# AliaksandrSiarohin/wc-gan

Hardware: AMD Instinct MI355X
Metric: images/sec G+D step, CIFAR-10 ResNet-SN+WC, batch 64 (higher is better)
Workload: dtype f32; 1 GPU; CIFAR-10 ResNet SN uncond + WC (scripts/cifar10_resnet_sn_uncond.sh), batch 64/GPU, training_ratio 5, generator_batch_multiple 2; parallelism=dp1, wc_statistics=per-replica, launch=hipgraph

## Files before the change

### include/wc_hip.h

```cpp
#ifndef WC_HIP_H
#define WC_HIP_H

#include <stddef.h>
#include <stdint.h>

#ifdef __cplusplus
extern "C" {
#endif

#define WC_ABI_VERSION 8

#define WC_OK                 0
#define WC_ERR_NULL          -1
#define WC_ERR_SHAPE         -2
#define WC_ERR_CHANNELS      -3
#define WC_ERR_WORKSPACE     -4
#define WC_ERR_ARG           -5

typedef void* wc_stream_t;

int         wc_abi_version(void);
const char* wc_error_string(int code);

#define WC_CORE_API "wc_stats_f32 wc_factor_f64 wc_color_f32 wc_group_bias_f32 wc_apply_f32 wc_apply_act_f32 " \
                    "wc_bwd_reduce_f32 wc_bwd_factor_f64 wc_bwd_apply_f32 " \
                    "wc_stats_workspace_bytes wc_factor_workspace_bytes wc_color_workspace_bytes wc_apply_workspace_bytes " \
                    "wc_bwd_reduce_workspace_bytes wc_bwd_factor_workspace_bytes wc_bwd_apply_workspace_bytes"

size_t wc_whiten_workspace_bytes(int64_t M, int C, int groups);
size_t wc_factor_error_offset(int C, int groups);
int    wc_factor_route(int C, int groups);
size_t wc_whiten_error_offset(int64_t M, int C, int groups);
int    wc_whiten_f32(const float* x, int64_t M, int C, int groups, double eps, double momentum, int ddof,
                     float* moving_mean , float* moving_cov ,
                     float* mu , float* chan_scale , double* L , double* W ,
                     void* ws, size_t ws_bytes, wc_stream_t stream);

size_t wc_stats_workspace_bytes(int64_t M, int C, int groups);
size_t wc_factor_workspace_bytes(int C, int groups);
size_t wc_color_workspace_bytes(int C, int Kc);
size_t wc_bwd_reduce_workspace_bytes(int64_t N, int64_t HW, int C, int Kc, int has_slot);
size_t wc_bwd_factor_workspace_bytes(int C, int Kc);
size_t wc_apply_workspace_bytes(int64_t N, int64_t HW, int C, int Kc);
size_t wc_apply_plan_bytes(int C, int Kc);
size_t wc_bwd_apply_workspace_bytes(int64_t N, int64_t HW, int C, int Kc);

int wc_stats_f32(const float* x, int64_t M, int C, int groups,
                 double* sum , double* xtx ,
                 void* ws, size_t ws_bytes, wc_stream_t stream);

int wc_factor_f64(const double* sum, const double* xtx, int64_t M , int C, int groups,
                  double eps, double momentum, int ddof, int training,
                  float* moving_mean , float* moving_cov ,
                  float* mu , float* chan_scale ,
                  double* L , double* W ,
                  void* ws, size_t ws_bytes, wc_stream_t stream);

int wc_color_f32(const double* W , const float* gamma ,
                 int Kc, int C, int groups, int per_group,
                 float* A , float* At ,
                 const float* chan_scale , void* plan ,
                 void* ws, size_t ws_bytes, wc_stream_t stream);

int wc_group_bias_f32(const float* mu , const float* A ,
                      const float* beta ,
                      int groups, int Kc, int C, int per_group, float* center , float* bias ,
                      wc_stream_t stream);

int wc_apply_f32(const float* x, const float* mu, const float* A, const float* bias,
                 const int32_t* slot, int64_t N, int64_t HW, int C, int Kc,
                 float* y, const void* plan ,
                 void* ws, size_t ws_bytes, wc_stream_t stream);

int wc_apply_act_f32(const float* x, const float* mu, const float* A, const float* bias,
                     const int32_t* slot, int64_t N, int64_t HW, int C, int Kc, int relu,
                     float* y, const void* plan ,
                     void* ws, size_t ws_bytes, wc_stream_t stream);

size_t wc_split_bytes(int64_t M, int C);
#define WC_SPLIT_FLAG_WORDS (64 + 2 * 1024)
int wc_split_scales_f32(const float* x, int64_t M, int C, float* center , float* scale ,
                        int* flag , wc_stream_t stream);
int wc_split_f32(const float* x, const float* center , const float* scale, int64_t M, int C, int relu,
                 void* xs , int* flag , wc_stream_t stream);
int wc_unsplit_f32(const void* xs, const float* center , const float* scale, int64_t M, int C, float* x ,
                   wc_stream_t stream);

int    wc_stats_split_supported(int64_t M, int C, int groups);
size_t wc_stats_split_workspace_bytes(int64_t M, int C, int groups);
int wc_stats_split_f16x2(const void* xs, const float* xs_center, const float* xs_scale, int64_t M, int C, int groups,
                         double* sum , double* xtx , void* ws, size_t ws_bytes, wc_stream_t stream);

int    wc_split_bias_f32(const float* A , const float* bias, const float* xs_center, const float* mu, int Kc, int C,
                         float* bias_eff , wc_stream_t stream);
int    wc_apply_split_supported(int64_t N, int64_t HW, int C);
size_t wc_apply_split_workspace_bytes(int C, int Kc);
int wc_apply_split_f16x2(const void* xs, const float* xs_center , const float* xs_scale,
                         const float* mu , const float* A, const float* bias ,
                         const int32_t* slot, int64_t N, int64_t HW, int C, int Kc, int relu,
                         float* y, const void* plan , void* ws, size_t ws_bytes, wc_stream_t stream);

int wc_resadd_split_supported(int64_t N, int64_t H, int64_t W, int C);
int wc_resadd_f32(const float* h, const float* s , int64_t N, int64_t H, int64_t W, int C, int up, float* out,
                  wc_stream_t stream);
int wc_resadd_split_f32(const float* h, const float* s , int64_t N, int64_t H, int64_t W, int C, int up,
                        void* xs , float* center , float* scale ,
                        int* flag , float* x32 ,
                        wc_stream_t stream);
int wc_patch_sum_f32(const float* g , int64_t N, int64_t Hs, int64_t Ws, int C, float* out ,
                     wc_stream_t stream);
int    wc_resadd_stats_supported(int64_t N, int64_t H, int64_t W, int C, int up, int groups);
size_t wc_resadd_stats_workspace_bytes(int64_t N, int64_t H, int64_t W, int C, int groups);
int    wc_resadd_stats_split_f32(const float* h, const float* s , int64_t N, int64_t H, int64_t W, int C, int up, int groups,
                                 void* xs , float* center , float* scale , int* flag ,
                                 float* x32 , void* ws , size_t ws_bytes, wc_stream_t stream);
size_t wc_whiten_presummed_error_offset(int64_t M, int C, int groups);
int    wc_whiten_presummed_f16x2(const float* xs_center, int64_t M, int C, int groups, double eps, double momentum, int ddof,
                                 float* moving_mean , float* moving_cov , float* mu ,
                                 double* L , double* W , void* ws ,
                                 size_t ws_bytes, wc_stream_t stream);
int    wc_stats_presummed_f16x2(const float* xs_center, int64_t M, int C, int groups, double* sum ,
                                double* xtx , void* ws , size_t ws_bytes, wc_stream_t stream);
int wc_fold_channel_scale_f32(const float* w, int64_t stride_o, int64_t stride_c, int Cout, int Cin, const float* bias ,
                              const float* scale, const float* center, float* wf , float* bf , wc_stream_t stream);
int wc_unfold_channel_scale_f32(const float* D, const float* db, int64_t stride_o, int64_t stride_c, int Cout, int Cin,
                                const float* scale, const float* center, float* dW , wc_stream_t stream);

size_t wc_whiten_split_workspace_bytes(int64_t M, int C, int groups);
size_t wc_whiten_split_error_offset(int64_t M, int C, int groups);
int    wc_whiten_split_f16x2(const void* xs, const float* xs_center, const float* xs_scale, int64_t M, int C, int groups,
                             double eps, double momentum, int ddof, float* moving_mean , float* moving_cov ,
                             float* mu , double* L , double* W ,
                             void* ws, size_t ws_bytes, wc_stream_t stream);

int wc_color_split_f32(const double* W , const float* gamma , int Kc, int C, float* A ,
                       float* At , const float* xs_scale, const float* xs_center, const float* mu ,
                       const float* beta , void* plan , float* bias_eff ,
                       void* ws, size_t ws_bytes, wc_stream_t stream);
int wc_group_bias_centered_f32(const float* mu , const float* A , const float* beta ,
                               const float* center , int groups, int Kc, int C, int per_group, float* bias ,
                               wc_stream_t stream);

int    wc_factor_mix_supported(int E, int C);
int    wc_factor_mix_f32(const float* dict, const float* alpha, const int32_t* idx , const float* base ,
                         int E, int C, int K, int Kc, float* out , wc_stream_t stream);
size_t wc_factor_mix_bwd_workspace_bytes(int E, int Kc);
int    wc_factor_mix_bwd_f32(const float* dict, const float* alpha, const int32_t* idx , const float* dout ,
                             int E, int C, int K, int Kc, float* ddict , float* dalpha , float* dbase ,
                             void* ws, size_t ws_bytes, wc_stream_t stream);

int wc_apply_split_ex_f16x2(const void* xs, const float* xs_center , const float* xs_scale,
                            const float* mu , const float* A, const float* bias ,
                            const int32_t* slot, int64_t N, int64_t HW, int C, int Kc, int relu,
                            float* y , void* relu_mask , void* planes , float* oscale,
                            const void* plan , void* ws, size_t ws_bytes, wc_stream_t stream);

size_t wc_relu_mask_bytes(int64_t M, int C);
int wc_relu_mask_apply_f32(const float* gy, const void* relu_mask, int64_t M, int C, float* out, wc_stream_t stream);
int wc_apply_mask_f32(const float* x, const float* mu, const float* A, const float* bias,
                      const int32_t* slot, int64_t N, int64_t HW, int C, int Kc,
                      float* y, void* relu_mask , const void* plan ,
                      void* ws, size_t ws_bytes, wc_stream_t stream);

int    wc_apply_planes_supported(int64_t N, int64_t HW, int C);
size_t wc_apply_planes_scale_floats(void);
int    wc_out_scale_f32(const float* gamma , const float* beta , int K, int C,
                        float* oscale, wc_stream_t stream);
int    wc_apply_planes_f32(const float* x, const float* mu, const float* A, const float* bias, const int32_t* slot,
                           int64_t N, int64_t HW, int C, int Kc, int relu, void* planes , float* oscale,
                           void* relu_mask , const void* plan, wc_stream_t stream);

int wc_bwd_reduce_f32(const float* x, const float* mu, const float* gy, const int32_t* slot,
                      int64_t N, int64_t HW, int C, int Kc,
                      double* R , double* gsum ,
                      void* ws, size_t ws_bytes, wc_stream_t stream);

int wc_bwd_reduce_scaled_f32(const float* x, const float* mu, const float* gy, const int32_t* slot,
                             int64_t N, int64_t HW, int C, int Kc,
                             double* R , double* gsum , float* scales_out ,
                             void* ws, size_t ws_bytes, wc_stream_t stream);
int wc_bwd_reduce_relu_f32(const float* x, const float* mu, const float* gy, const float* relu_y , const int32_t* slot,
                           int64_t N, int64_t HW, int C, int Kc,
                           double* R , double* gsum , float* gy_masked ,
                           float* scales_out , void* ws, size_t ws_bytes, wc_stream_t stream);
int wc_bwd_reduce_mask_f32(const float* x, const float* mu, const float* gy, const void* relu_mask, const int32_t* slot,
                           int64_t N, int64_t HW, int C, int Kc,
                           double* R , double* gsum , float* gy_masked ,
                           float* scales_out , void* ws, size_t ws_bytes, wc_stream_t stream);

int wc_bwd_bits_supported(int64_t N, int64_t HW, int C, int has_slot);
int wc_bwd_reduce_bits_f32(const float* x, const float* mu, const float* gy, const void* relu_mask, const int32_t* slot,
                           int64_t N, int64_t HW, int C, int Kc, double* R , double* gsum ,
                           float* scales_out , void* ws, size_t ws_bytes, wc_stream_t stream);
int wc_bwd_apply_bits_f32(const float* gy, const void* relu_mask, const float* x, const float* mu, const float* At, const float* S,
                          const float* gmean, const int32_t* slot, int64_t N, int64_t HW, int C, int Kc,
                          const float* scales , float* dx, void* ws, size_t ws_bytes, wc_stream_t stream);
int wc_bwd_apply_scaled_f32(const float* gy, const float* x, const float* mu, const float* At,
                            const float* S, const float* gmean, const int32_t* slot,
                            int64_t N, int64_t HW, int C, int Kc, const float* scales , float* dx,
                            void* ws, size_t ws_bytes, wc_stream_t stream);

int    wc_bwd_xsplit_supported(int64_t N, int64_t HW, int C, int has_slot);
int    wc_bwd_reduce_xsplit_f32(const void* xs, const float* xs_center, const float* xs_scale, const float* mu, const float* gy,
                                const void* relu_mask , const int32_t* slot, int64_t N, int64_t HW, int C, int Kc,
                                double* R , double* gsum , float* scales_out ,
                                void* ws , size_t ws_bytes, wc_stream_t stream);
size_t wc_bwd_apply_xsplit_workspace_bytes(int C, int Kc);
int    wc_bwd_apply_xsplit_f32(const float* gy, const void* relu_mask , const void* xs, const float* xs_center,
                               const float* xs_scale, const float* mu, const float* At, const float* S, const float* gmean,
                               const int32_t* slot, int64_t N, int64_t HW, int C, int Kc, const float* scales ,
                               float* dx, void* ws, size_t ws_bytes, wc_stream_t stream);

int wc_bwd_factor_f64(const double* R, const double* gsum, const double* W, const double* L,
                      const float* gamma, const float* A, int Kc, int C, int64_t M,
                      double eps, int ddof, int training,
                      float* dgamma , float* dbeta ,
                      float* S , float* gmean ,
                      void* ws, size_t ws_bytes, wc_stream_t stream);

int wc_bwd_apply_f32(const float* gy, const float* x, const float* mu, const float* At,
                     const float* S, const float* gmean, const int32_t* slot,
                     int64_t N, int64_t HW, int C, int Kc, float* dx,
                     void* ws, size_t ws_bytes, wc_stream_t stream);

size_t wc_spectral_norm_workspace_bytes(int rows, int cols);
size_t wc_spectral_norm_amax_offset(int rows, int cols);
size_t wc_spectral_norm_error_offset(int rows, int cols);
int wc_spectral_norm_f32(const float* W, int rows, int cols, float* u, float* v, int iterations, float eps,
                         float* w_sn , float* sigma ,
                         float* u_used , float* v_used ,
                         void* ws, size_t ws_bytes, wc_stream_t stream);

int wc_spectral_norm_bwd_f32(const float* g, const float* w_sn, const float* u, const float* v, const float* sigma,
                             int rows, int cols, int fully_diff, float* dW,
                             void* ws, size_t ws_bytes, wc_stream_t stream);

typedef struct {
    const float* W; float* u; float* v; float* w_sn; float* sigma; float* u_used; float* v_used; void* ws;
    int rows, cols;
} wc_sn_item;
typedef struct {
    const float* g; const float* w_sn; const float* u; const float* v; const float* sigma; float* dW; void* ws;
    int rows, cols;
} wc_sn_bwd_item;
int wc_spectral_norm_batched_f32(const wc_sn_item* items, int count, int iterations, float eps, wc_stream_t stream);
int wc_spectral_norm_bwd_batched_f32(const wc_sn_bwd_item* items, int count, int fully_diff, wc_stream_t stream);

typedef struct {
    int N, H, W;
    int Hin, Win, Cin;
    int Hout, Wout, Cout;
    int in_stride, out_stride;
    int ntaps, nphase;
    signed char dy[4][16], dx[4][16];
    signed char off_y[4], off_x[4];
    signed char nsrc[4][16];
    signed char wr[4][16][4], ws[4][16][4];
    float wcoef;
} wc_conv_geom;

#define WC_CONV_SCRATCH_BYTES 2048

int wc_conv_supported(const wc_conv_geom* g);

int wc_conv_split_f32(const float* x, int64_t n, int relu, void* hi, void* lo, float* scale, void* amax_scratch,
                      wc_stream_t stream);

#define WC_CONV_COLSUM_ROWS 512
int wc_conv_split_colsum_f32(const float* x, int64_t n, int relu, void* hi, void* lo, float* scale, void* amax_scratch,
                             float* colsum_partials, int C, wc_stream_t stream);

#define WC_CONV_HIST_FLOATS (4 * 512 + 16)
#define WC_CONV_HIST_REDO (4 * 512)
int wc_conv_split_hist_f32(const float* x, int64_t n, int relu, void* hi, void* lo, float* scale, float* colsum_partials , int C,
                           float* hist, int bootstrap, wc_stream_t stream);

int wc_conv_split_leaky_f32(const float* x, int64_t n, float negative_slope, void* hi, void* lo, float* scale, void* amax_scratch,
                            float* colsum_partials , int C, wc_stream_t stream);
int wc_conv_split_hist_leaky_f32(const float* x, int64_t n, float negative_slope, void* hi, void* lo, float* scale,
                                 float* colsum_partials , int C, float* hist, int bootstrap, wc_stream_t stream);
int wc_conv_leaky_bwd_f32(float* dx, const float* x, int64_t n, float negative_slope, wc_stream_t stream);

size_t wc_conv_weights_bytes(const wc_conv_geom* g);
int wc_conv_weights_f32(const float* w, int64_t stride_k, int64_t stride_n, int64_t stride_r, int64_t stride_s,
                        int64_t n_elems, const wc_conv_geom* g, void* image, float* scale, void* amax_scratch,
                        const float* known_amax, int known_count, wc_stream_t stream);

int wc_conv_weights_pair_f32(const float* w, int64_t stride_r, int64_t stride_s, int64_t n_elems,
                             int64_t a_stride_k, int64_t a_stride_n, const wc_conv_geom* ga, void* image_a,
                             int64_t b_stride_k, int64_t b_stride_n, const wc_conv_geom* gb, void* image_b,
                             float* scale, void* amax_scratch, const float* known_amax, int known_count,
                             wc_stream_t stream);

size_t wc_conv_workspace_bytes(const wc_conv_geom* g);
int wc_conv_f16x3(const void* xhi, const void* xlo, const float* xscale, const void* wimage, const float* wscale,
                  const float* bias, const void* zero_line, const wc_conv_geom* g, int relu, float* y,
                  void* ws, size_t ws_bytes, wc_stream_t stream);

size_t wc_conv_wrw_workspace_bytes(const wc_conv_geom* g);
int wc_conv_wrw_f16x3(const void* xhi, const void* xlo, const float* xscale, const void* ghi, const void* glo,
                      const float* gscale, const void* zero_line, const wc_conv_geom* g, float* dw, int64_t stride_k,
                      int64_t stride_n, int64_t stride_r, int64_t stride_s, void* ws, size_t ws_bytes,
                      wc_stream_t stream);

int    wc_conv_wrw_narrow_supported(int64_t N, int64_t H, int64_t W, int Cin, int Cout, int ksize);
size_t wc_conv_wrw_narrow_workspace_bytes(int64_t N, int64_t H, int64_t W, int Cin, int Cout, int ksize);
int    wc_conv_wrw_narrow_f32(const float* x, const float* gy, int64_t N, int64_t H, int64_t W, int Cin, int Cout, int ksize,
                              float* dw, int64_t stride_k, int64_t stride_n, int64_t stride_r, int64_t stride_s, float* db ,
                              void* ws, size_t ws_bytes, wc_stream_t stream);

int    wc_conv_narrow64_supported(int64_t N, int64_t H, int64_t W, int Cin, int Cout, int ksize);
size_t wc_conv_wrw_narrow64_workspace_bytes(int64_t N, int64_t H, int64_t W, int Cin, int Cout, int ksize);
int    wc_conv_wrw_narrow64_f32(const float* x, const float* gy, int64_t N, int64_t H, int64_t W, int Cin, int Cout, int ksize,
                                float* dw, int64_t stride_k, int64_t stride_n, int64_t stride_r, int64_t stride_s, float* db ,
                                void* ws, size_t ws_bytes, wc_stream_t stream);

int    wc_conv_fwd_narrow_f32(const float* x, const float* w, int64_t stride_k, int64_t stride_n, int64_t stride_r, int64_t stride_s,
                              const float* bias , int64_t N, int64_t H, int64_t W, int Cin, int Cout, int ksize, int relu,
                              float* y, wc_stream_t stream);

int wc_conv_wrw_bias_f16x3(const void* xhi, const void* xlo, const float* xscale, const void* ghi, const void* glo,
                           const float* gscale, const void* zero_line, const wc_conv_geom* g, float* dw, int64_t stride_k,
                           int64_t stride_n, int64_t stride_r, int64_t stride_s, const float* colsum_partials, float* db,
                           void* ws, size_t ws_bytes, wc_stream_t stream);

int    wc_conv_bwd_pair_supported(const wc_conv_geom* gd, const wc_conv_geom* gf);
size_t wc_conv_bwd_pair_workspace_bytes(const wc_conv_geom* gd, const wc_conv_geom* gf);
int    wc_conv_bwd_pair_f16x3(const void* ghi, const void* glo, const float* gscale, const void* wimage, const float* wscale,
                              const void* zero_line, const wc_conv_geom* gd, float* dx, void* ws_dx, size_t ws_dx_bytes,
                              const void* xhi, const void* xlo, const float* xscale, const wc_conv_geom* gf, float* dw,
                              int64_t stride_k, int64_t stride_n, int64_t stride_r, int64_t stride_s,
                              const float* colsum_partials, float* db, void* ws_dw, size_t ws_dw_bytes, wc_stream_t stream);

int wc_stream_copy_f32(const float* src, float* dst, int64_t n, wc_stream_t stream);


size_t wc_std_stats_workspace_bytes(int64_t M, int C, int groups);
int    wc_std_stats_f32(const float* x, int64_t M, int C, int groups, double* sum , double* sqsum ,
                        void* ws, size_t ws_bytes, wc_stream_t stream);

int    wc_std_factor_f64(const double* sum, const double* sqsum, int64_t M, int C, int groups, double eps, double momentum, int ddof,
                         int training, float* moving_mean , float* moving_variance ,
                         const float* gamma , const float* beta , int Kc,
                         float* mu , float* w , float* a , float* b ,
                         wc_stream_t stream);

int    wc_std_apply_f32(const float* x, const float* a, const float* b, const int32_t* slot , int64_t N, int64_t HW,
                        int C, int Kt, int relu, float* y, wc_stream_t stream);

size_t wc_std_bwd_reduce_workspace_bytes(int64_t N, int64_t HW, int C, int Kc);
int    wc_std_bwd_reduce_f32(const float* x, const float* gy, const float* a, const float* b, const int32_t* slot, int64_t N, int64_t HW,
                             int C, int Kc, int relu, double* gsum , double* gxsum ,
                             void* ws, size_t ws_bytes, wc_stream_t stream);

int    wc_std_bwd_factor_f64(const double* gsum, const double* gxsum, const float* mu , const float* w ,
                             const float* gamma , int64_t M, int C, int Kc, int training,
                             float* dgamma , float* dbeta , float* q , float* r , wc_stream_t stream);

int    wc_std_bwd_apply_f32(const float* x, const float* gy, const float* a, const float* b, const float* q, const float* r,
                            const int32_t* slot, int64_t N, int64_t HW, int C, int Kc, int relu, float* dx, wc_stream_t stream);


int    wc_zca_supported(int C);
size_t wc_zca_workspace_bytes(int C, int groups);
size_t wc_zca_status_offset(int C, int groups);
int    wc_zca_f64(const double* L , int C, int groups, double eps,
                  double* U , double* lam , double* W ,
                  void* ws, size_t ws_bytes, wc_stream_t stream);

size_t wc_bwd_factor_zca_workspace_bytes(int C, int Kc);
int    wc_bwd_factor_zca_f64(const double* R, const double* gsum, const double* W, const double* U, const double* lam,
                             const float* gamma, const float* A, int Kc, int C, int64_t M,
                             double eps, int ddof, int training,
                             float* dgamma , float* dbeta ,
                             float* S , float* gmean ,
                             void* ws, size_t ws_bytes, wc_stream_t stream);


int    wc_renorm_supported(int C);
size_t wc_renorm_workspace_bytes(int C);
int    wc_renorm_f64(const float* moving_cov , const double* L , int C, double eps,
                     double* Wm , double* C0 ,
                     void* ws, size_t ws_bytes, wc_stream_t stream);

size_t wc_bwd_factor_renorm_workspace_bytes(int C, int Kc);
int    wc_bwd_factor_renorm_f64(const double* R, const double* gsum, const double* W, const double* Wm, const double* C0,
                                const float* gamma, const float* A, int Kc, int C, int64_t M,
                                double eps, int ddof, int training,
                                float* dgamma , float* dbeta ,
                                float* S , float* gmean ,
                                void* ws, size_t ws_bytes, wc_stream_t stream);


int wc_conv_split_masked_f32(const float* t, const float* a, int64_t n, float slope, void* hi, void* lo, float* scale, void* amax_scratch,
                             wc_stream_t stream);
int wc_conv_split_hist_masked_f32(const float* t, const float* a, int64_t n, float slope, void* hi, void* lo, float* scale, float* hist,
                                  int bootstrap, wc_stream_t stream);

int wc_gp_interp_f32(const float* real, const float* fake, const float* eps, int64_t N, int64_t L, float* x_hat, wc_stream_t stream);

size_t wc_gp_rows_workspace_bytes(int64_t N);
int wc_gp_rows_f32(const float* g, int64_t N, int64_t L, double lambda, double inv_n, float* norms , float* v ,
                   float* penalty , void* ws, size_t ws_bytes, wc_stream_t stream);

#ifdef __cplusplus
}
#endif
#endif
```

### wc_gan_amd/_lib.py

```python
from __future__ import annotations

import ctypes
import os
from ctypes import c_float, c_char_p, c_double, c_int, c_int64, c_size_t, c_void_p

_HERE = os.path.dirname(os.path.abspath(__file__))
LIB_PATH = os.path.join(_HERE, "libwc_hip.so")

WC_OK = 0
ABI_VERSION = 8
ERRORS = {-1: "WC_ERR_NULL", -2: "WC_ERR_SHAPE", -3: "WC_ERR_CHANNELS", -4: "WC_ERR_WORKSPACE", -5: "WC_ERR_ARG"}

SIGNATURES = {
    "wc_abi_version": (c_int, []),
    "wc_error_string": (c_char_p, [c_int]),
    "wc_stats_workspace_bytes": (c_size_t, [c_int64, c_int, c_int]),
    "wc_factor_workspace_bytes": (c_size_t, [c_int, c_int]),
    "wc_color_workspace_bytes": (c_size_t, [c_int, c_int]),
    "wc_bwd_reduce_workspace_bytes": (c_size_t, [c_int64, c_int64, c_int, c_int, c_int]),
    "wc_bwd_factor_workspace_bytes": (c_size_t, [c_int, c_int]),
    "wc_apply_workspace_bytes": (c_size_t, [c_int64, c_int64, c_int, c_int]),
    "wc_apply_plan_bytes": (c_size_t, [c_int, c_int]),
    "wc_bwd_apply_workspace_bytes": (c_size_t, [c_int64, c_int64, c_int, c_int]),
    "wc_stats_f32": (c_int, [c_void_p, c_int64, c_int, c_int, c_void_p, c_void_p, c_void_p, c_size_t, c_void_p]),
    "wc_group_bias_f32": (c_int, [c_void_p, c_void_p, c_void_p, c_int, c_int, c_int, c_int, c_void_p, c_void_p, c_void_p]),
    "wc_factor_f64": (c_int, [c_void_p, c_void_p, c_int64, c_int, c_int, c_double, c_double, c_int, c_int,
                              c_void_p, c_void_p, c_void_p, c_void_p, c_void_p, c_void_p, c_void_p, c_size_t, c_void_p]),
    "wc_color_f32": (c_int, [c_void_p, c_void_p, c_int, c_int, c_int, c_int, c_void_p, c_void_p, c_void_p, c_void_p,
                             c_void_p, c_size_t, c_void_p]),
    "wc_apply_f32": (c_int, [c_void_p, c_void_p, c_void_p, c_void_p, c_void_p, c_int64, c_int64, c_int, c_int,
                             c_void_p, c_void_p, c_void_p, c_size_t, c_void_p]),
    "wc_apply_act_f32": (c_int, [c_void_p, c_void_p, c_void_p, c_void_p, c_void_p, c_int64, c_int64, c_int, c_int, c_int,
                                 c_void_p, c_void_p, c_void_p, c_size_t, c_void_p]),
    "wc_bwd_reduce_f32": (c_int, [c_void_p, c_void_p, c_void_p, c_void_p, c_int64, c_int64, c_int, c_int,
                                  c_void_p, c_void_p, c_void_p, c_size_t, c_void_p]),
    "wc_bwd_reduce_scaled_f32": (c_int, [c_void_p, c_void_p, c_void_p, c_void_p, c_int64, c_int64, c_int, c_int,
                                         c_void_p, c_void_p, c_void_p, c_void_p, c_size_t, c_void_p]),
    "wc_bwd_reduce_relu_f32": (c_int, [c_void_p, c_void_p, c_void_p, c_void_p, c_void_p, c_int64, c_int64, c_int, c_int,
                                       c_void_p, c_void_p, c_void_p, c_void_p, c_void_p, c_size_t, c_void_p]),
    "wc_relu_mask_bytes": (c_size_t, [c_int64, c_int]),
    "wc_relu_mask_apply_f32": (c_int, [c_void_p, c_void_p, c_int64, c_int, c_void_p, c_void_p]),
    "wc_apply_mask_f32": (c_int, [c_void_p, c_void_p, c_void_p, c_void_p, c_void_p, c_int64, c_int64, c_int, c_int,
                                  c_void_p, c_void_p, c_void_p, c_void_p, c_size_t, c_void_p]),
    "wc_whiten_workspace_bytes": (c_size_t, [c_int64, c_int, c_int]),
    "wc_factor_error_offset": (c_size_t, [c_int, c_int]),
    "wc_factor_route": (c_int, [c_int, c_int]),
    "wc_whiten_error_offset": (c_size_t, [c_int64, c_int, c_int]),
    "wc_whiten_f32": (c_int, [c_void_p, c_int64, c_int, c_int, c_double, c_double, c_int, c_void_p, c_void_p, c_void_p, c_void_p,
                              c_void_p, c_void_p, c_void_p, c_size_t, c_void_p]),
    "wc_apply_planes_supported": (c_int, [c_int64, c_int64, c_int]),
    "wc_apply_planes_scale_floats": (c_size_t, []),
    "wc_out_scale_f32": (c_int, [c_void_p, c_void_p, c_int, c_int, c_void_p, c_void_p]),
    "wc_apply_planes_f32": (c_int, [c_void_p, c_void_p, c_void_p, c_void_p, c_void_p, c_int64, c_int64, c_int, c_int, c_int,
                                    c_void_p, c_void_p, c_void_p, c_void_p, c_void_p]),
    "wc_bwd_reduce_mask_f32": (c_int, [c_void_p, c_void_p, c_void_p, c_void_p, c_void_p, c_int64, c_int64, c_int, c_int,
                                       c_void_p, c_void_p, c_void_p, c_void_p, c_void_p, c_size_t, c_void_p]),
    "wc_bwd_bits_supported": (c_int, [c_int64, c_int64, c_int, c_int]),
    "wc_bwd_reduce_bits_f32": (c_int, [c_void_p, c_void_p, c_void_p, c_void_p, c_void_p, c_int64, c_int64, c_int, c_int,
                                       c_void_p, c_void_p, c_void_p, c_void_p, c_size_t, c_void_p]),
    "wc_bwd_apply_bits_f32": (c_int, [c_void_p, c_void_p, c_void_p, c_void_p, c_void_p, c_void_p, c_void_p, c_void_p,
                                      c_int64, c_int64, c_int, c_int, c_void_p, c_void_p, c_void_p, c_size_t, c_void_p]),
    "wc_bwd_apply_scaled_f32": (c_int, [c_void_p, c_void_p, c_void_p, c_void_p, c_void_p, c_void_p, c_void_p,
                                        c_int64, c_int64, c_int, c_int, c_void_p, c_void_p, c_void_p, c_size_t, c_void_p]),
    "wc_bwd_factor_f64": (c_int, [c_void_p, c_void_p, c_void_p, c_void_p, c_void_p, c_void_p, c_int, c_int, c_int64,
                                  c_double, c_int, c_int, c_void_p, c_void_p, c_void_p, c_void_p,
                                  c_void_p, c_size_t, c_void_p]),
    "wc_bwd_apply_f32": (c_int, [c_void_p, c_void_p, c_void_p, c_void_p, c_void_p, c_void_p, c_void_p,
                                 c_int64, c_int64, c_int, c_int, c_void_p, c_void_p, c_size_t, c_void_p]),
    "wc_split_bytes": (c_size_t, [c_int64, c_int]),
    "wc_split_scales_f32": (c_int, [c_void_p, c_int64, c_int, c_void_p, c_void_p, c_void_p, c_void_p]),
    "wc_split_f32": (c_int, [c_void_p, c_void_p, c_void_p, c_int64, c_int, c_int, c_void_p, c_void_p, c_void_p]),
    "wc_unsplit_f32": (c_int, [c_void_p, c_void_p, c_void_p, c_int64, c_int, c_void_p, c_void_p]),
    "wc_stats_split_supported": (c_int, [c_int64, c_int, c_int]),
    "wc_stats_split_workspace_bytes": (c_size_t, [c_int64, c_int, c_int]),
    "wc_stats_split_f16x2": (c_int, [c_void_p, c_void_p, c_void_p, c_int64, c_int, c_int, c_void_p, c_void_p, c_void_p, c_size_t, c_void_p]),
    "wc_split_bias_f32": (c_int, [c_void_p, c_void_p, c_void_p, c_void_p, c_int, c_int, c_void_p, c_void_p]),
    "wc_apply_split_supported": (c_int, [c_int64, c_int64, c_int]),
    "wc_apply_split_workspace_bytes": (c_size_t, [c_int, c_int]),
    "wc_apply_split_f16x2": (c_int, [c_void_p, c_void_p, c_void_p, c_void_p, c_void_p, c_void_p, c_void_p, c_int64, c_int64,
                                     c_int, c_int, c_int, c_void_p, c_void_p, c_void_p, c_size_t, c_void_p]),
    "wc_apply_split_ex_f16x2": (c_int, [c_void_p, c_void_p, c_void_p, c_void_p, c_void_p, c_void_p, c_void_p, c_int64, c_int64,
                                        c_int, c_int, c_int, c_void_p, c_void_p, c_void_p, c_void_p, c_void_p, c_void_p, c_size_t, c_void_p]),
    "wc_whiten_split_workspace_bytes": (c_size_t, [c_int64, c_int, c_int]),
    "wc_whiten_split_error_offset": (c_size_t, [c_int64, c_int, c_int]),
    "wc_whiten_split_f16x2": (c_int, [c_void_p, c_void_p, c_void_p, c_int64, c_int, c_int, c_double, c_double, c_int, c_void_p, c_void_p,
                                      c_void_p, c_void_p, c_void_p, c_void_p, c_size_t, c_void_p]),
    "wc_resadd_split_supported": (c_int, [c_int64, c_int64, c_int64, c_int]),
    "wc_resadd_f32": (c_int, [c_void_p, c_void_p, c_int64, c_int64, c_int64, c_int, c_int, c_void_p, c_void_p]),
    "wc_resadd_stats_supported": (c_int, [c_int64, c_int64, c_int64, c_int, c_int, c_int]),
    "wc_resadd_stats_workspace_bytes": (c_size_t, [c_int64, c_int64, c_int64, c_int, c_int]),
    "wc_resadd_stats_split_f32": (c_int, [c_void_p, c_void_p, c_int64, c_int64, c_int64, c_int, c_int, c_int, c_void_p, c_void_p, c_void_p, c_void_p,
                                          c_void_p, c_void_p, c_size_t, c_void_p]),
    "wc_whiten_presummed_error_offset": (c_size_t, [c_int64, c_int, c_int]),
    "wc_whiten_presummed_f16x2": (c_int, [c_void_p, c_int64, c_int, c_int, c_double, c_double, c_int, c_void_p, c_void_p, c_void_p, c_void_p,
                                          c_void_p, c_void_p, c_size_t, c_void_p]),
    "wc_stats_presummed_f16x2": (c_int, [c_void_p, c_int64, c_int, c_int, c_void_p, c_void_p, c_void_p, c_size_t, c_void_p]),
    "wc_resadd_split_f32": (c_int, [c_void_p, c_void_p, c_int64, c_int64, c_int64, c_int, c_int, c_void_p, c_void_p, c_void_p, c_void_p,
                                    c_void_p, c_void_p]),
    "wc_patch_sum_f32": (c_int, [c_void_p, c_int64, c_int64, c_int64, c_int, c_void_p, c_void_p]),
    "wc_fold_channel_scale_f32": (c_int, [c_void_p, c_int64, c_int64, c_int, c_int, c_void_p, c_void_p, c_void_p, c_void_p, c_void_p, c_void_p]),
    "wc_unfold_channel_scale_f32": (c_int, [c_void_p, c_void_p, c_int64, c_int64, c_int, c_int, c_void_p, c_void_p, c_void_p, c_void_p]),
    "wc_color_split_f32": (c_int, [c_void_p, c_void_p, c_int, c_int, c_void_p, c_void_p, c_void_p, c_void_p, c_void_p, c_void_p, c_void_p,
                                   c_void_p, c_void_p, c_size_t, c_void_p]),
    "wc_factor_mix_supported": (c_int, [c_int, c_int]),
    "wc_factor_mix_f32": (c_int, [c_void_p, c_void_p, c_void_p, c_void_p, c_int, c_int, c_int, c_int, c_void_p, c_void_p]),
    "wc_factor_mix_bwd_workspace_bytes": (c_size_t, [c_int, c_int]),
    "wc_factor_mix_bwd_f32": (c_int, [c_void_p, c_void_p, c_void_p, c_void_p, c_int, c_int, c_int, c_int, c_void_p, c_void_p, c_void_p,
                                      c_void_p, c_size_t, c_void_p]),
    "wc_group_bias_centered_f32": (c_int, [c_void_p, c_void_p, c_void_p, c_void_p, c_int, c_int, c_int, c_int, c_void_p, c_void_p]),
    "wc_bwd_xsplit_supported": (c_int, [c_int64, c_int64, c_int, c_int]),
    "wc_bwd_reduce_xsplit_f32": (c_int, [c_void_p, c_void_p, c_void_p, c_void_p, c_void_p, c_void_p, c_void_p, c_int64, c_int64, c_int, c_int,
                                         c_void_p, c_void_p, c_void_p, c_void_p, c_size_t, c_void_p]),
    "wc_bwd_apply_xsplit_workspace_bytes": (c_size_t, [c_int, c_int]),
    "wc_bwd_apply_xsplit_f32": (c_int, [c_void_p, c_void_p, c_void_p, c_void_p, c_void_p, c_void_p, c_void_p, c_void_p, c_void_p, c_void_p,
                                        c_int64, c_int64, c_int, c_int, c_void_p, c_void_p, c_void_p, c_size_t, c_void_p]),
    "wc_stream_copy_f32": (c_int, [c_void_p, c_void_p, c_int64, c_void_p]),
    "wc_spectral_norm_workspace_bytes": (c_size_t, [c_int, c_int]),
    "wc_spectral_norm_batched_f32": (c_int, [c_void_p, c_int, c_int, c_float, c_void_p]),
    "wc_spectral_norm_bwd_batched_f32": (c_int, [c_void_p, c_int, c_int, c_void_p]),
    "wc_spectral_norm_f32": (c_int, [c_void_p, c_int, c_int, c_void_p, c_void_p, c_int, c_float, c_void_p, c_void_p,
                                     c_void_p, c_void_p, c_void_p, c_size_t, c_void_p]),
    "wc_spectral_norm_bwd_f32": (c_int, [c_void_p, c_void_p, c_void_p, c_void_p, c_void_p, c_int, c_int, c_int, c_void_p,
                                         c_void_p, c_size_t, c_void_p]),
    "wc_conv_supported": (c_int, [c_void_p]),
    "wc_conv_split_f32": (c_int, [c_void_p, c_int64, c_int, c_void_p, c_void_p, c_void_p, c_void_p, c_void_p]),
    "wc_conv_weights_bytes": (c_size_t, [c_void_p]),
    "wc_conv_weights_f32": (c_int, [c_void_p, c_int64, c_int64, c_int64, c_int64, c_int64, c_void_p, c_void_p, c_void_p,
                                    c_void_p, c_void_p, c_int, c_void_p]),
    "wc_spectral_norm_amax_offset": (c_size_t, [c_int, c_int]),
    "wc_spectral_norm_error_offset": (c_size_t, [c_int, c_int]),
    "wc_conv_split_hist_f32": (c_int, [c_void_p, c_int64, c_int, c_void_p, c_void_p, c_void_p, c_void_p, c_int, c_void_p, c_int, c_void_p]),
    "wc_conv_split_leaky_f32": (c_int, [c_void_p, c_int64, c_float, c_void_p, c_void_p, c_void_p, c_void_p, c_void_p, c_int, c_void_p]),
    "wc_conv_split_hist_leaky_f32": (c_int, [c_void_p, c_int64, c_float, c_void_p, c_void_p, c_void_p, c_void_p, c_int, c_void_p, c_int, c_void_p]),
    "wc_conv_leaky_bwd_f32": (c_int, [c_void_p, c_void_p, c_int64, c_float, c_void_p]),
    "wc_conv_narrow64_supported": (c_int, [c_int64, c_int64, c_int64, c_int, c_int, c_int]),
    "wc_conv_wrw_narrow64_workspace_bytes": (c_size_t, [c_int64, c_int64, c_int64, c_int, c_int, c_int]),
    "wc_conv_wrw_narrow64_f32": (c_int, [c_void_p, c_void_p, c_int64, c_int64, c_int64, c_int, c_int, c_int, c_void_p, c_int64, c_int64, c_int64,
                                         c_int64, c_void_p, c_void_p, c_size_t, c_void_p]),
    "wc_conv_fwd_narrow_f32": (c_int, [c_void_p, c_void_p, c_int64, c_int64, c_int64, c_int64, c_void_p, c_int64, c_int64, c_int64, c_int, c_int, c_int,
                                       c_int, c_void_p, c_void_p]),
    "wc_conv_wrw_narrow_supported": (c_int, [c_int64, c_int64, c_int64, c_int, c_int, c_int]),
    "wc_conv_wrw_narrow_workspace_bytes": (c_size_t, [c_int64, c_int64, c_int64, c_int, c_int, c_int]),
    "wc_conv_wrw_narrow_f32": (c_int, [c_void_p, c_void_p, c_int64, c_int64, c_int64, c_int, c_int, c_int, c_void_p, c_int64, c_int64, c_int64,
                                       c_int64, c_void_p, c_void_p, c_size_t, c_void_p]),
    "wc_conv_split_colsum_f32": (c_int, [c_void_p, c_int64, c_int, c_void_p, c_void_p, c_void_p, c_void_p, c_void_p, c_int, c_void_p]),
    "wc_conv_wrw_bias_f16x3": (c_int, [c_void_p, c_void_p, c_void_p, c_void_p, c_void_p, c_void_p, c_void_p, c_void_p, c_void_p,
                                       c_int64, c_int64, c_int64, c_int64, c_void_p, c_void_p, c_void_p, c_size_t, c_void_p]),
    "wc_conv_weights_pair_f32": (c_int, [c_void_p, c_int64, c_int64, c_int64, c_int64, c_int64, c_void_p, c_void_p,
                                         c_int64, c_int64, c_void_p, c_void_p, c_void_p, c_void_p, c_void_p, c_int, c_void_p]),
    "wc_conv_wrw_workspace_bytes": (c_size_t, [c_void_p]),
    "wc_conv_wrw_f16x3": (c_int, [c_void_p, c_void_p, c_void_p, c_void_p, c_void_p, c_void_p, c_void_p, c_void_p, c_void_p,
                                  c_int64, c_int64, c_int64, c_int64, c_void_p, c_size_t, c_void_p]),
    "wc_conv_workspace_bytes": (c_size_t, [c_void_p]),
    "wc_conv_f16x3": (c_int, [c_void_p, c_void_p, c_void_p, c_void_p, c_void_p, c_void_p, c_void_p, c_void_p, c_int,
                              c_void_p, c_void_p, c_size_t, c_void_p]),
    "wc_conv_bwd_pair_supported": (c_int, [c_void_p, c_void_p]),
    "wc_conv_bwd_pair_workspace_bytes": (c_size_t, [c_void_p, c_void_p]),
    "wc_conv_bwd_pair_f16x3": (c_int, [c_void_p, c_void_p, c_void_p, c_void_p, c_void_p, c_void_p, c_void_p, c_void_p, c_void_p, c_size_t,
                                       c_void_p, c_void_p, c_void_p, c_void_p, c_void_p, c_int64, c_int64, c_int64, c_int64,
                                       c_void_p, c_void_p, c_void_p, c_size_t, c_void_p]),
    "wc_std_stats_workspace_bytes": (c_size_t, [c_int64, c_int, c_int]),
    "wc_std_stats_f32": (c_int, [c_void_p, c_int64, c_int, c_int, c_void_p, c_void_p, c_void_p, c_size_t, c_void_p]),
    "wc_std_factor_f64": (c_int, [c_void_p, c_void_p, c_int64, c_int, c_int, c_double, c_double, c_int, c_int, c_void_p, c_void_p,
                                  c_void_p, c_void_p, c_int, c_void_p, c_void_p, c_void_p, c_void_p, c_void_p]),
    "wc_std_apply_f32": (c_int, [c_void_p, c_void_p, c_void_p, c_void_p, c_int64, c_int64, c_int, c_int, c_int, c_void_p, c_void_p]),
    "wc_std_bwd_reduce_workspace_bytes": (c_size_t, [c_int64, c_int64, c_int, c_int]),
    "wc_std_bwd_reduce_f32": (c_int, [c_void_p, c_void_p, c_void_p, c_void_p, c_void_p, c_int64, c_int64, c_int, c_int, c_int,
                                      c_void_p, c_void_p, c_void_p, c_size_t, c_void_p]),
    "wc_std_bwd_factor_f64": (c_int, [c_void_p, c_void_p, c_void_p, c_void_p, c_void_p, c_int64, c_int, c_int, c_int,
                                      c_void_p, c_void_p, c_void_p, c_void_p, c_void_p]),
    "wc_std_bwd_apply_f32": (c_int, [c_void_p, c_void_p, c_void_p, c_void_p, c_void_p, c_void_p, c_void_p, c_int64, c_int64, c_int, c_int,
                                     c_int, c_void_p, c_void_p]),
    "wc_zca_supported": (c_int, [c_int]),
    "wc_zca_workspace_bytes": (c_size_t, [c_int, c_int]),
    "wc_zca_status_offset": (c_size_t, [c_int, c_int]),
    "wc_zca_f64": (c_int, [c_void_p, c_int, c_int, c_double, c_void_p, c_void_p, c_void_p, c_void_p, c_size_t, c_void_p]),
    "wc_bwd_factor_zca_workspace_bytes": (c_size_t, [c_int, c_int]),
    "wc_bwd_factor_zca_f64": (c_int, [c_void_p, c_void_p, c_void_p, c_void_p, c_void_p, c_void_p, c_void_p, c_int, c_int, c_int64,
                                      c_double, c_int, c_int, c_void_p, c_void_p, c_void_p, c_void_p,
                                      c_void_p, c_size_t, c_void_p]),
    "wc_renorm_supported": (c_int, [c_int]),
    "wc_renorm_workspace_bytes": (c_size_t, [c_int]),
    "wc_renorm_f64": (c_int, [c_void_p, c_void_p, c_int, c_double, c_void_p, c_void_p, c_void_p, c_size_t, c_void_p]),
    "wc_bwd_factor_renorm_workspace_bytes": (c_size_t, [c_int, c_int]),
    "wc_bwd_factor_renorm_f64": (c_int, [c_void_p, c_void_p, c_void_p, c_void_p, c_void_p, c_void_p, c_void_p, c_int, c_int, c_int64,
                                         c_double, c_int, c_int, c_void_p, c_void_p, c_void_p, c_void_p,
                                         c_void_p, c_size_t, c_void_p]),
    "wc_conv_split_masked_f32": (c_int, [c_void_p, c_void_p, c_int64, c_float, c_void_p, c_void_p, c_void_p, c_void_p, c_void_p]),
    "wc_conv_split_hist_masked_f32": (c_int, [c_void_p, c_void_p, c_int64, c_float, c_void_p, c_void_p, c_void_p, c_void_p, c_int, c_void_p]),
    "wc_gp_interp_f32": (c_int, [c_void_p, c_void_p, c_void_p, c_int64, c_int64, c_void_p, c_void_p]),
    "wc_gp_rows_workspace_bytes": (c_size_t, [c_int64]),
    "wc_gp_rows_f32": (c_int, [c_void_p, c_int64, c_int64, c_double, c_double, c_void_p, c_void_p, c_void_p, c_void_p, c_size_t, c_void_p]),
}


class SnItem(ctypes.Structure):
    _fields_ = [("W", c_void_p), ("u", c_void_p), ("v", c_void_p), ("w_sn", c_void_p), ("sigma", c_void_p),
                ("u_used", c_void_p), ("v_used", c_void_p), ("ws", c_void_p), ("rows", c_int), ("cols", c_int)]


class SnBwdItem(ctypes.Structure):
    _fields_ = [("g", c_void_p), ("w_sn", c_void_p), ("u", c_void_p), ("v", c_void_p), ("sigma", c_void_p),
                ("dW", c_void_p), ("ws", c_void_p), ("rows", c_int), ("cols", c_int)]


class ConvGeom(ctypes.Structure):
    _fields_ = [("N", c_int), ("H", c_int), ("W", c_int), ("Hin", c_int), ("Win", c_int), ("Cin", c_int),
                ("Hout", c_int), ("Wout", c_int), ("Cout", c_int), ("in_stride", c_int), ("out_stride", c_int),
                ("ntaps", c_int), ("nphase", c_int),
                ("dy", (ctypes.c_byte * 16) * 4), ("dx", (ctypes.c_byte * 16) * 4),
                ("off_y", ctypes.c_byte * 4), ("off_x", ctypes.c_byte * 4),
                ("nsrc", (ctypes.c_byte * 16) * 4),
                ("wr", ((ctypes.c_byte * 4) * 16) * 4), ("ws", ((ctypes.c_byte * 4) * 16) * 4),
                ("wcoef", c_float)]


_lib = None


class WcHipError(RuntimeError):
    pass


def shared_gpu_guard(device_count=None) -> bool:
    if "WC_K2_TWO_LAUNCH" in os.environ:
        if os.environ["WC_K2_TWO_LAUNCH"] == "0":
            del os.environ["WC_K2_TWO_LAUNCH"]
        return False
    try:
        ranks = int(os.environ.get("LOCAL_WORLD_SIZE", "1") or 1)
    except ValueError:
        ranks = 1
    if ranks <= 1:
        return False
    if any(os.environ.get(k) for k in ("HIP_VISIBLE_DEVICES", "CUDA_VISIBLE_DEVICES", "ROCR_VISIBLE_DEVICES")):
        return False
    if device_count is None:
        try:
            import torch
            device_count = torch.cuda.device_count()
        except Exception:
            device_count = 0
    if device_count and ranks > device_count:
        os.environ["WC_K2_TWO_LAUNCH"] = "1"
        return True
    return False


def load() -> ctypes.CDLL:
    global _lib
    if _lib is not None:
        return _lib
    import torch
    shared_gpu_guard()
    if not os.path.exists(LIB_PATH):
        raise WcHipError(
            f"{LIB_PATH} is missing: build it with `python -m wc_gan_amd.build` "
            "(or __graft_entry__.build()); the WC path has no non-HIP fallback")
    lib = ctypes.CDLL(LIB_PATH)
    for name, (res, args) in SIGNATURES.items():
        fn = getattr(lib, name)
        fn.restype = res
        fn.argtypes = args
    if lib.wc_abi_version() != ABI_VERSION:
        raise WcHipError(f"libwc_hip.so ABI version {lib.wc_abi_version()} != {ABI_VERSION}: rebuild it "
                         "(python -m wc_gan_amd.build)")
    _lib = lib
    return lib


def check(code: int, what: str) -> None:
    if code == WC_OK:
        return
    lib = load()
    msg = lib.wc_error_string(code)
    raise WcHipError(f"{what} failed: {ERRORS.get(code, code)} ({msg.decode() if msg else '?'})")
```

### wc_gan_amd/conv.py

```python
from __future__ import annotations

import ctypes
import os

import torch
import torch.nn.functional as F

from . import _lib, _state
from .ops import _ptr, _stream

_zero_lines = {}


def _zero_line(device):
    z = _zero_lines.get(device)
    if z is None:
        z = _zero_lines[device] = torch.zeros(64, dtype=torch.uint8, device=device)
    return z


def _plain(r, s):
    return [(r, s)], 1.0


def _pooled3(r, s):
    return [(r - a, s - b) for a in (0, 1) for b in (0, 1) if 0 <= r - a <= 2 and 0 <= s - b <= 2], 0.25


_UP_ROWS = ((2,), (1, 2), (0, 1), (0,))


def _upsampled3(r, s):
    return [(r3, s3) for r3 in _UP_ROWS[r] for s3 in _UP_ROWS[s]], 1.0


def _set_sources(g, p, t, r, s, source):
    taps, coef = source(r, s)
    g.nsrc[p][t] = len(taps)
    for m, (r3, s3) in enumerate(taps):
        g.wr[p][t][m], g.ws[p][t][m] = r3, s3
    g.wcoef = coef


def _dense_geom(N, Hin, Win, Cin, Cout, k, stride, source=_plain):
    pad = k // 2 if stride == 1 else 1
    g = _lib.ConvGeom()
    g.N, g.Hin, g.Win, g.Cin, g.Cout = N, Hin, Win, Cin, Cout
    g.H, g.W = Hin // stride, Win // stride
    g.Hout, g.Wout = g.H, g.W
    g.in_stride, g.out_stride, g.ntaps, g.nphase = stride, 1, k * k, 1
    for r in range(k):
        for s in range(k):
            t = r * k + s
            g.dy[0][t], g.dx[0][t] = r - pad, s - pad
            _set_sources(g, 0, t, r, s, source)
    return g


def _phase_geom(N, Hin, Win, Cin, Cout, source=_plain):
    g = _lib.ConvGeom()
    g.N, g.Hin, g.Win, g.Cin, g.Cout = N, Hin, Win, Cin, Cout
    g.H, g.W, g.Hout, g.Wout = Hin, Win, 2 * Hin, 2 * Win
    g.in_stride, g.out_stride, g.ntaps, g.nphase = 1, 2, 4, 4
    for py in range(2):
        for px in range(2):
            p = py * 2 + px
            g.off_y[p], g.off_x[p] = py, px
            t = 0
            for dy in ((-1, 0) if py == 0 else (0, 1)):
                for dx in ((-1, 0) if px == 0 else (0, 1)):
                    g.dy[p][t], g.dx[p][t] = dy, dx
                    _set_sources(g, p, t, py + 1 - 2 * dy, px + 1 - 2 * dx, source)
                    t += 1
    return g


def _supported(g):
    return bool(_lib.load().wc_conv_supported(ctypes.addressof(g)))


def supported(x, w, kind):
    handed = getattr(x, '_wc_planes', None) is not None
    if not (x.is_cuda and x.dtype == torch.float32 and x.dim() == 4 and (handed or x.is_contiguous()) and w.dtype == torch.float32):
        return False
    p = _plan(kind, x, w)
    return bool(p) and p.ok


class _Plan:
    __slots__ = ('ok', 'fwd', 'bwd', 'fwd_ws', 'bwd_ws', 'wrw_ws', 'fwd_ptr', 'bwd_ptr', 'pair')

    def __init__(self, kind, N, H, W, wshape):
        class _W:
            shape = wshape
        lib = _lib.load()
        (gf, kf, nf), (gb, kb, nb) = _geoms(kind, N, H, W, _W)
        self.fwd, self.bwd = (gf, kf, nf), (gb, kb, nb)
        self.fwd_ptr, self.bwd_ptr = ctypes.addressof(gf), ctypes.addressof(gb)
        self.ok = bool(lib.wc_conv_supported(self.fwd_ptr)) and bool(lib.wc_conv_supported(self.bwd_ptr))
        self.fwd_ws = lib.wc_conv_workspace_bytes(self.fwd_ptr) if self.ok else 0
        self.bwd_ws = lib.wc_conv_workspace_bytes(self.bwd_ptr) if self.ok else 0
        self.wrw_ws = lib.wc_conv_wrw_workspace_bytes(self.fwd_ptr) if self.ok else 0
        self.pair = self.ok and bool(lib.wc_conv_bwd_pair_supported(self.bwd_ptr, self.fwd_ptr))


_plans = {}


def _plan(kind, x, w):
    key = (kind, tuple(x.shape), tuple(w.shape))
    p = _plans.get(key)
    if p is None:
        N, H, W, C = x.shape
        good = (kind == 'same' and w.shape[1] == C and w.shape[2] == w.shape[3] and w.shape[2] in (1, 3)) or \
               (kind == 'down' and w.shape[1] == C and tuple(w.shape[2:]) == (4, 4) and H % 2 == 0 and W % 2 == 0) or \
               (kind == 'down3' and w.shape[1] == C and tuple(w.shape[2:]) == (3, 3) and H % 2 == 0 and W % 2 == 0) or \
               (kind == 'up3' and w.shape[1] == C and tuple(w.shape[2:]) == (3, 3)) or \
               (kind == 'up' and w.shape[0] == C and tuple(w.shape[2:]) == (4, 4))
        if kind not in ('same', 'down', 'up', 'down3', 'up3'):
            raise ValueError(kind)
        if good and kind != 'down' and (C % 128 or w.shape[0] % 128 or w.shape[1] % 128):
            good = False
        p = _plans[key] = _Plan(kind, N, H, W, tuple(w.shape)) if good else False
    return p


def _colsum_ok(C):
    return C % 4 == 0 and 256 % (C // 4) == 0


SPLIT_HIST = os.environ.get('WC_SPLIT_HIST', '1') != '0'
HIST_FLOATS = 4 * 512 + 16
HIST_REDO = 4 * 512


_REDO_MODE = os.environ.get('WC_SPLIT_HIST_REDO', '1')


def _guarded(role):
    return _REDO_MODE == '2' or (_REDO_MODE != '0' and role in ('g', 't', 'd'))


def _site_hist(site, role, device):
    if not getattr(site, 'training', True):
        return None
    book = site.__dict__.setdefault('_wc_split_hist', {})
    h = book.get(role)
    if h is not None and h[0].device != device:
        h = None
    if h is None:
        if torch.cuda.is_current_stream_capturing():
            return None
        h = book[role] = [torch.zeros(HIST_FLOATS, dtype=torch.float32, device=device), False]
    return h


def split_planes(x, relu=False, colsum=False, site=None, role='x', leaky=None):
    lib = _lib.load()
    if leaky is not None:
        if relu:
            raise ValueError("relu and leaky are two activations")
        return _split_planes_leaky(lib, x, float(leaky), colsum, site, role)
    both = torch.empty((2,) + tuple(x.shape), dtype=torch.float16, device=x.device)
    hi, lo = both[0], both[1]
    scale = torch.empty(1 + 512, dtype=torch.float32, device=x.device)
    h = _site_hist(site, role, x.device) if (SPLIT_HIST and site is not None) else None
    if h is not None:
        C = x.shape[-1]
        part = torch.empty((512, C), dtype=torch.float32, device=x.device) if colsum else None
        _lib.check(lib.wc_conv_split_hist_f32(_ptr(x), x.numel(), 1 if relu else 0, _ptr(hi), _ptr(lo), _ptr(scale), _ptr(part), C if colsum else 0,
                                              _ptr(h[0]), (0 if h[1] else 1) | (0 if _guarded(role) else 2), _stream()), "wc_conv_split_hist_f32")
        h[1] = True
        return (hi, lo, scale, part) if colsum else (hi, lo, scale)
    if not colsum:
        _lib.check(lib.wc_conv_split_f32(_ptr(x), x.numel(), 1 if relu else 0, _ptr(hi), _ptr(lo), _ptr(scale),
                                         scale.data_ptr() + 4, _stream()), "wc_conv_split_f32")
        return hi, lo, scale
    C = x.shape[-1]
    part = torch.empty((512, C), dtype=torch.float32, device=x.device)
    _lib.check(lib.wc_conv_split_colsum_f32(_ptr(x), x.numel(), 1 if relu else 0, _ptr(hi), _ptr(lo), _ptr(scale),
                                            scale.data_ptr() + 4, _ptr(part), C, _stream()), "wc_conv_split_colsum_f32")
    return hi, lo, scale, part


def _split_planes_leaky(lib, x, slope, colsum, site, role):
    both = torch.empty((2,) + tuple(x.shape), dtype=torch.float16, device=x.device)
    hi, lo = both[0], both[1]
    scale = torch.empty(1 + 512, dtype=torch.float32, device=x.device)
    C = x.shape[-1]
    part = torch.empty((512, C), dtype=torch.float32, device=x.device) if colsum else None
    h = _site_hist(site, role, x.device) if (SPLIT_HIST and site is not None) else None
    if h is not None:
        _lib.check(lib.wc_conv_split_hist_leaky_f32(_ptr(x), x.numel(), slope, _ptr(hi), _ptr(lo), _ptr(scale), _ptr(part), C if colsum else 0,
                                                    _ptr(h[0]), (0 if h[1] else 1) | (0 if _guarded(role) else 2), _stream()),
                   "wc_conv_split_hist_leaky_f32")
        h[1] = True
    else:
        _lib.check(lib.wc_conv_split_leaky_f32(_ptr(x), x.numel(), slope, _ptr(hi), _ptr(lo), _ptr(scale), scale.data_ptr() + 4,
                                               _ptr(part), C if colsum else 0, _stream()), "wc_conv_split_leaky_f32")
    return (hi, lo, scale, part) if colsum else (hi, lo, scale)


def split_planes_masked(t, a, slope=0.0, site=None, role='t'):
    if not (t.is_contiguous() and a.is_contiguous() and t.shape == a.shape and t.dtype == a.dtype == torch.float32):
        raise ValueError("split_planes_masked: dense fp32 tensors of one shape")
    lib = _lib.load()
    both = torch.empty((2,) + tuple(t.shape), dtype=torch.float16, device=t.device)
    hi, lo = both[0], both[1]
    scale = torch.empty(1 + 512, dtype=torch.float32, device=t.device)
    h = _site_hist(site, role, t.device) if (SPLIT_HIST and site is not None) else None
    if h is not None:
        _lib.check(lib.wc_conv_split_hist_masked_f32(_ptr(t), _ptr(a), t.numel(), float(slope), _ptr(hi), _ptr(lo), _ptr(scale), _ptr(h[0]),
                                                     (0 if h[1] else 1) | (0 if _guarded(role) else 2), _stream()),
                   "wc_conv_split_hist_masked_f32")
        h[1] = True
    else:
        _lib.check(lib.wc_conv_split_masked_f32(_ptr(t), _ptr(a), t.numel(), float(slope), _ptr(hi), _ptr(lo), _ptr(scale),
                                                scale.data_ptr() + 4, _stream()), "wc_conv_split_masked_f32")
    return hi, lo, scale


def leaky_backward_(dx, x, slope):
    if not (dx.is_contiguous() and x.is_contiguous() and dx.shape == x.shape and dx.dtype == x.dtype == torch.float32):
        raise ValueError("leaky_backward_: dense fp32 tensors of one shape")
    _lib.check(_lib.load().wc_conv_leaky_bwd_f32(_ptr(dx), _ptr(x), dx.numel(), float(slope), _stream()), "wc_conv_leaky_bwd_f32")
    return dx


def _storage_extent(w):
    return 1 + sum((n - 1) * s for n, s in zip(w.shape, w.stride()))


def weight_image(w, geom, k_axis, n_axis):
    lib = _lib.load()
    nbytes = lib.wc_conv_weights_bytes(ctypes.addressof(geom))
    img = torch.empty(nbytes, dtype=torch.uint8, device=w.device)
    scale = torch.empty(1 + 512, dtype=torch.float32, device=w.device)
    ext = _storage_extent(w)
    if ext != w.numel():
        raise ValueError("weight must be dense")
    known = getattr(w, '_wc_amax', None)
    _lib.check(lib.wc_conv_weights_f32(_ptr(w), w.stride(k_axis), w.stride(n_axis), w.stride(2), w.stride(3), ext,
                                       ctypes.addressof(geom), _ptr(img), _ptr(scale), scale.data_ptr() + 4,
                                       _ptr(known), 0 if known is None else known.numel(), _stream()),
               "wc_conv_weights_f32")
    return img, scale


def weight_image_pair(w, fwd, bwd):
    lib = _lib.load()
    (ga, ka, na), (gb, kb, nb) = fwd, bwd
    img_a = torch.empty(lib.wc_conv_weights_bytes(ctypes.addressof(ga)), dtype=torch.uint8, device=w.device)
    img_b = torch.empty(lib.wc_conv_weights_bytes(ctypes.addressof(gb)), dtype=torch.uint8, device=w.device)
    scale = torch.empty(2 + 512, dtype=torch.float32, device=w.device)
    ext = _storage_extent(w)
    if ext != w.numel():
        raise ValueError("weight must be dense")
    known = getattr(w, '_wc_amax', None)
    _lib.check(lib.wc_conv_weights_pair_f32(_ptr(w), w.stride(2), w.stride(3), ext,
                                            w.stride(ka), w.stride(na), ctypes.addressof(ga), _ptr(img_a),
                                            w.stride(kb), w.stride(nb), ctypes.addressof(gb), _ptr(img_b),
                                            _ptr(scale), scale.data_ptr() + 8, _ptr(known), 0 if known is None else known.numel(),
                                            _stream()), "wc_conv_weights_pair_f32")
    return (img_a, scale[0:1]), (img_b, scale[1:2])


def _cached_image(w, key, geom, k_axis, n_axis):
    return weight_image(w, geom, k_axis, n_axis)


def run(planes, image, geom, bias=None, relu=False, nbytes=None):
    hi, lo, xs = planes
    img, ws = image
    lib = _lib.load()
    y = torch.empty((geom.N, geom.Hout, geom.Wout, geom.Cout), dtype=torch.float32, device=hi.device)
    if nbytes is None:
        nbytes = lib.wc_conv_workspace_bytes(ctypes.addressof(geom))
    work = torch.empty(nbytes, dtype=torch.uint8, device=hi.device) if nbytes else None
    _lib.check(lib.wc_conv_f16x3(_ptr(hi), _ptr(lo), _ptr(xs), _ptr(img), _ptr(ws), _ptr(bias) if bias is not None else None,
                                 _ptr(_zero_line(hi.device)), ctypes.addressof(geom), 1 if relu else 0, _ptr(y),
                                 _ptr(work), nbytes, _stream()), "wc_conv_f16x3")
    return y


def _geoms(kind, N, H, W, w):
    if kind == 'same':
        co, ci, k = w.shape[0], w.shape[1], w.shape[2]
        fwd = _dense_geom(N, H, W, ci, co, k, 1)
        bwd = _dense_geom(N, H, W, co, ci, k, 1)
        for t in range(k * k):
            bwd.dy[0][t], bwd.dx[0][t] = -bwd.dy[0][t], -bwd.dx[0][t]
        return (fwd, 1, 0), (bwd, 0, 1)
    if kind in ('down', 'down3'):
        co, ci = w.shape[0], w.shape[1]
        src = _pooled3 if kind == 'down3' else _plain
        return (_dense_geom(N, H, W, ci, co, 4, 2, src), 1, 0), (_phase_geom(N, H // 2, W // 2, co, ci, src), 0, 1)
    if kind == 'up3':
        co, ci = w.shape[0], w.shape[1]
        return (_phase_geom(N, H, W, ci, co, _upsampled3), 1, 0), (_dense_geom(N, 2 * H, 2 * W, co, ci, 4, 2, _upsampled3), 0, 1)
    ci, co = w.shape[0], w.shape[1]
    return (_phase_geom(N, H, W, ci, co), 0, 1), (_dense_geom(N, 2 * H, 2 * W, co, ci, 4, 2), 1, 0)


def weight_gradient(x_planes, g_planes, geom, w, k_axis, n_axis, nbytes=None, colsum=None):
    lib = _lib.load()
    xh, xl, xs = x_planes
    gh, gl, gs = g_planes[:3]
    dw = torch.empty_like(w)
    if dw.stride() != w.stride():
        raise ValueError("weight must be dense")
    if nbytes is None:
        nbytes = lib.wc_conv_wrw_workspace_bytes(ctypes.addressof(geom))
    ws = torch.empty(nbytes, dtype=torch.uint8, device=w.device)
    if colsum is not None:
        db = torch.empty(geom.Cout, dtype=torch.float32, device=w.device)
        _lib.check(lib.wc_conv_wrw_bias_f16x3(_ptr(xh), _ptr(xl), _ptr(xs), _ptr(gh), _ptr(gl), _ptr(gs), _ptr(_zero_line(w.device)),
                                              ctypes.addressof(geom), _ptr(dw), w.stride(k_axis), w.stride(n_axis), w.stride(2),
                                              w.stride(3), _ptr(colsum), _ptr(db), _ptr(ws), nbytes, _stream()),
                   "wc_conv_wrw_bias_f16x3")
        return dw, db
    _lib.check(lib.wc_conv_wrw_f16x3(_ptr(xh), _ptr(xl), _ptr(xs), _ptr(gh), _ptr(gl), _ptr(gs), _ptr(_zero_line(w.device)),
                                     ctypes.addressof(geom), _ptr(dw), w.stride(k_axis), w.stride(n_axis), w.stride(2),
                                     w.stride(3), _ptr(ws), nbytes, _stream()), "wc_conv_wrw_f16x3")
    return dw


def backward_pair(g_planes, image, x_planes, plan, w, colsum=None):
    lib = _lib.load()
    gh, gl, gs = g_planes[:3]
    xh, xl, xs = x_planes
    img, ws = image
    gf, kf, nf = plan.fwd
    gb = plan.bwd[0]
    dx = torch.empty((gb.N, gb.Hout, gb.Wout, gb.Cout), dtype=torch.float32, device=gh.device)
    dw = torch.empty_like(w)
    if dw.stride() != w.stride():
        raise ValueError("weight must be dense")
    work_dx = torch.empty(plan.bwd_ws, dtype=torch.uint8, device=gh.device) if plan.bwd_ws else None
    work_dw = torch.empty(plan.wrw_ws, dtype=torch.uint8, device=gh.device)
    db = torch.empty(gf.Cout, dtype=torch.float32, device=w.device) if colsum is not None else None
    zero = _zero_line(gh.device)
    _lib.check(lib.wc_conv_bwd_pair_f16x3(_ptr(gh), _ptr(gl), _ptr(gs), _ptr(img), _ptr(ws), _ptr(zero), plan.bwd_ptr, _ptr(dx),
                                          _ptr(work_dx), plan.bwd_ws,
                                          _ptr(xh), _ptr(xl), _ptr(xs), plan.fwd_ptr, _ptr(dw), w.stride(kf), w.stride(nf), w.stride(2),
                                          w.stride(3), _ptr(colsum), _ptr(db), _ptr(work_dw), plan.wrw_ws, _stream()),
               "wc_conv_bwd_pair_f16x3")
    return dx, dw, db


def takes_planes(shape, wshape, kind):
    class _S:
        pass
    xs, ws = _S(), _S()
    xs.shape, ws.shape = tuple(shape), tuple(wshape)
    p = _plan(kind, xs, ws)
    return bool(p) and p.ok


class _FastConv(torch.autograd.Function):
    @staticmethod
    def forward(ctx, x, w, bias, kind, plan, relu_input=False, handed=None, site=None, leaky=None):
        gf, kf, nf = plan.fwd
        planes = handed if handed is not None else split_planes(x, relu=relu_input, site=site, role='x', leaky=leaky)
        ctx.site, ctx.leaky = site, leaky
        if ctx.needs_input_grad[0]:
            img, ctx.bwd_image = weight_image_pair(w, plan.fwd, plan.bwd)
        else:
            img, ctx.bwd_image = weight_image(w, gf, kf, nf), None
        y = run(planes, img, gf, bias, nbytes=plan.fwd_ws)
        ctx.save_for_backward(w, *planes, *((x,) if (relu_input or leaky is not None) else ()))
        ctx.kind, ctx.has_bias, ctx.plan, ctx.relu_input = kind, bias is not None, plan, relu_input
        return y

    @staticmethod
    def backward(ctx, gy):
        w, xh, xl, xs = ctx.saved_tensors[:4]
        kind, plan = ctx.kind, ctx.plan
        gy = gy.contiguous()
        want_db = ctx.has_bias and ctx.needs_input_grad[2]
        fused_db = want_db and ctx.needs_input_grad[1] and _colsum_ok(gy.shape[-1])
        g_planes = split_planes(gy, colsum=fused_db, site=ctx.site, role='g')
        dx = dw = db = None
        paired = ctx.needs_input_grad[0] and ctx.needs_input_grad[1] and ctx.bwd_image is not None and plan.pair
        if paired:
            dx, dw, pdb = backward_pair(g_planes, ctx.bwd_image, (xh, xl, xs), plan, w, colsum=g_planes[3] if fused_db else None)
            if fused_db:
                db = pdb
        if ctx.needs_input_grad[0]:
            if not paired:
                gb, kb, nb = plan.bwd
                image = ctx.bwd_image if ctx.bwd_image is not None else weight_image(w, gb, kb, nb)
                dx = run(g_planes[:3], image, gb, nbytes=plan.bwd_ws)
            if ctx.relu_input:
                dx = torch.ops.aten.threshold_backward(dx, ctx.saved_tensors[4], 0)
            elif ctx.leaky is not None:
                dx = leaky_backward_(dx, ctx.saved_tensors[4], ctx.leaky)
        if ctx.needs_input_grad[1] and not paired:
            gf, kf, nf = plan.fwd
            if fused_db:
                dw, db = weight_gradient((xh, xl, xs), g_planes, gf, w, kf, nf, nbytes=plan.wrw_ws, colsum=g_planes[3])
            else:
                dw = weight_gradient((xh, xl, xs), g_planes, gf, w, kf, nf, nbytes=plan.wrw_ws)
        if want_db and not fused_db:
            db = gy.sum((0, 1, 2))
        return dx, dw, db, None, None, None, None, None, None


_ones = {}


def _one(device):
    t = _ones.get(device)
    if t is None:
        t = torch.ones(1, dtype=torch.float32, device=device)
        if not torch.cuda.is_current_stream_capturing():
            _ones[device] = t
    return t


class _SplitConv(torch.autograd.Function):

    @staticmethod
    def forward(ctx, x, w, bias, plan, st, site=None):
        from . import ops
        ctx.site = site
        gf, kf, nf = plan.fwd
        wf, bf = ops.fold_channel_scale(w, bias, st.scale, st.center)
        img = weight_image(wf, gf, kf, nf)
        ctx.bwd_image = None
        if ctx.needs_input_grad[0]:
            gb, kb, nb = plan.bwd
            ctx.bwd_image = weight_image(w, gb, kb, nb)
        hi, lo = st.planes[0].view(st.shape), st.planes[1].view(st.shape)
        one = _one(hi.device)
        y = run((hi, lo, one), img, gf, bf, nbytes=plan.fwd_ws)
        ctx.save_for_backward(w, hi, lo, one, st.scale, st.center)
        ctx.plan, ctx.has_bias = plan, bias is not None
        return y

    @staticmethod
    def backward(ctx, gy):
        from . import ops
        w, xh, xl, one, scale, center = ctx.saved_tensors
        plan = ctx.plan
        gy = gy.contiguous()
        need_w = ctx.needs_input_grad[1]
        need_b = ctx.has_bias and ctx.needs_input_grad[2]
        fused_db = need_w and _colsum_ok(gy.shape[-1])
        g_planes = split_planes(gy, colsum=fused_db, site=ctx.site, role='g')
        dx = dw = db = None
        paired = ctx.needs_input_grad[0] and need_w and ctx.bwd_image is not None and plan.pair
        if paired:
            dx, D, db = backward_pair(g_planes, ctx.bwd_image, (xh, xl, one), plan, w, colsum=g_planes[3] if fused_db else None)
            if not fused_db:
                db = gy.sum((0, 1, 2))
            dw = ops.unfold_channel_scale(D, db, scale, center)
        elif ctx.needs_input_grad[0]:
            gb, kb, nb = plan.bwd
            image = ctx.bwd_image if ctx.bwd_image is not None else weight_image(w, gb, kb, nb)
            dx = run(g_planes[:3], image, gb, nbytes=plan.bwd_ws)
        if need_w:
            if not paired:
                gf, kf, nf = plan.fwd
                if fused_db:
                    D, db = weight_gradient((xh, xl, one), g_planes, gf, w, kf, nf, nbytes=plan.wrw_ws, colsum=g_planes[3])
                else:
                    D = weight_gradient((xh, xl, one), g_planes, gf, w, kf, nf, nbytes=plan.wrw_ws)
                    db = gy.sum((0, 1, 2))
                dw = ops.unfold_channel_scale(D, db, scale, center)
        elif need_b:
            db = gy.sum((0, 1, 2))
        return dx, dw, (db if need_b else None), None, None, None


def split_conv(x, st, w, bias=None, site=None):
    p = _plan('same', x, w)
    if not (p and p.ok and tuple(w.shape[2:]) == (1, 1) and w.dtype == torch.float32):
        raise _lib.WcHipError(f"split_conv: a pre-split handle reached a convolution without a planes path {tuple(x.shape)} x {tuple(w.shape)}")
    return _SplitConv.apply(x, w, bias, p, st, site)


def fast_conv_or_none(x, w, bias=None, kind='same', relu_input=False, site=None, leaky_input=None):
    if leaky_input is not None and relu_input:
        raise ValueError("relu_input and leaky_input are two activations")
    handed = getattr(x, '_wc_planes', None)
    if not supported(x, w, kind):
        if handed is not None:
            raise _lib.WcHipError(f"fast_conv: a K3 handle reached a convolution that cannot take planes {tuple(x.shape)} x {tuple(w.shape)} ({kind})")
        return None
    if handed is not None:
        if relu_input or leaky_input is not None:
            raise ValueError("a K3 handle is already ReLU'd")
        return _FastConv.apply(x, w, bias, kind, _plan(kind, x, w), False, handed, site)
    return _FastConv.apply(x, w, bias, kind, _plan(kind, x, w), relu_input, None, site,
                           None if leaky_input is None else float(leaky_input))


NARROW_WRW = os.environ.get('WC_NARROW_WRW', '1') != '0'


def narrow_wrw_supported(x, w):
    if not (NARROW_WRW and x.is_cuda and x.dtype == torch.float32 and w.dtype == torch.float32 and x.dim() == 4 and w.dim() == 4):
        return False
    k = w.shape[2]
    if w.shape[3] != k or k not in (1, 3) or w.shape[1] != x.shape[3]:
        return False
    N, H, W, C = x.shape
    return bool(_lib.load().wc_conv_narrow64_supported(N, H, W, C, w.shape[0], k))


def narrow_forward(x, w, bias=None, relu=False, mirrored=False):
    lib = _lib.load()
    N, H, W, C = x.shape
    k = w.shape[2]
    if mirrored:
        O = w.shape[1]
        ptr = ctypes.c_void_p(w.data_ptr() + 4 * ((k - 1) * w.stride(2) + (k - 1) * w.stride(3)))
        strides = (w.stride(0), w.stride(1), -w.stride(2), -w.stride(3))
    else:
        O = w.shape[0]
        ptr = _ptr(w)
        strides = (w.stride(1), w.stride(0), w.stride(2), w.stride(3))
    y = torch.empty((N, H, W, O), dtype=torch.float32, device=x.device)
    xc = x if x.is_contiguous() else x.contiguous()
    _lib.check(lib.wc_conv_fwd_narrow_f32(_ptr(xc), ptr, *strides, _ptr(bias), N, H, W, C, O, k, 1 if relu else 0, _ptr(y), _stream()),
               "wc_conv_fwd_narrow_f32")
    return y


class _NarrowInConv(torch.autograd.Function):

    @staticmethod
    def forward(ctx, x, w, bias):
        ctx.save_for_backward(x, w)
        ctx.has_bias = bias is not None
        return narrow_forward(x, w, bias)

    @staticmethod
    def backward(ctx, gy):
        x, w = ctx.saved_tensors
        N, H, W, C = x.shape
        O, k = w.shape[0], w.shape[2]
        lib = _lib.load()
        dx = dw = db = None
        g = gy if gy.is_contiguous() else gy.contiguous()
        if ctx.needs_input_grad[0]:
            dx = torch.ops.aten.convolution_backward(g.permute(0, 3, 1, 2), x.permute(0, 3, 1, 2), w, None, [1, 1], [k // 2, k // 2], [1, 1],
                                                     False, [0, 0], 1, [True, False, False])[0].permute(0, 2, 3, 1)
        if ctx.needs_input_grad[1] or (ctx.has_bias and ctx.needs_input_grad[2]):
            dw = torch.empty_strided(w.shape, w.stride(), dtype=torch.float32, device=w.device)
            if _storage_extent(dw) != dw.numel():
                raise ValueError("weight must be dense")
            db = torch.empty(O, dtype=torch.float32, device=w.device) if ctx.has_bias else None
            nb = lib.wc_conv_wrw_narrow64_workspace_bytes(N, H, W, C, O, k)
            ws = torch.empty(nb, dtype=torch.uint8, device=x.device)
            xc = x if x.is_contiguous() else x.contiguous()
            _lib.check(lib.wc_conv_wrw_narrow64_f32(_ptr(xc), _ptr(g), N, H, W, C, O, k, _ptr(dw), dw.stride(1), dw.stride(0), dw.stride(2),
                                                    dw.stride(3), _ptr(db), _ptr(ws), nb, _stream()), "wc_conv_wrw_narrow64_f32")
        return dx, dw, db


def narrow_weight_gradient(x, gy, w):
    N, H, W, C = x.shape
    O, k = w.shape[0], w.shape[2]
    lib = _lib.load()
    dw = torch.empty_strided(w.shape, w.stride(), dtype=torch.float32, device=w.device)
    if _storage_extent(dw) != dw.numel():
        raise ValueError("weight must be dense")
    nb = lib.wc_conv_wrw_narrow64_workspace_bytes(N, H, W, C, O, k)
    ws = torch.empty(nb, dtype=torch.uint8, device=x.device)
    xc = x if x.is_contiguous() else x.contiguous()
    g = gy if gy.is_contiguous() else gy.contiguous()
    _lib.check(lib.wc_conv_wrw_narrow64_f32(_ptr(xc), _ptr(g), N, H, W, C, O, k, _ptr(dw), dw.stride(1), dw.stride(0), dw.stride(2),
                                            dw.stride(3), None, _ptr(ws), nb, _stream()), "wc_conv_wrw_narrow64_f32")
    return dw


def narrow_in_conv(x, w, bias=None):
    if _storage_extent(w) != w.numel():
        w = w.contiguous()
    return _NarrowInConv.apply(x, w, bias)


def narrow_out_weight_gradient(x, gy, w):
    lib = _lib.load()
    N, H, W, C = x.shape
    O, k = w.shape[0], w.shape[2]
    dw = torch.empty_strided(w.shape, w.stride(), dtype=torch.float32, device=w.device)
    if _storage_extent(dw) != dw.numel():
        raise ValueError("weight must be dense")
    nb = lib.wc_conv_wrw_narrow_workspace_bytes(N, H, W, O, C, k)
    ws = torch.empty(nb, dtype=torch.uint8, device=x.device)
    last = dw.data_ptr() + 4 * ((k - 1) * dw.stride(2) + (k - 1) * dw.stride(3))
    _lib.check(lib.wc_conv_wrw_narrow_f32(_ptr(gy), _ptr(x), N, H, W, O, C, k, ctypes.c_void_p(last), dw.stride(0), dw.stride(1), -dw.stride(2),
                                          -dw.stride(3), None, _ptr(ws), nb, _stream()), "wc_conv_wrw_narrow_f32")
    return dw


def narrow_out_wrw_supported(x, w):
    if not (NARROW_WRW and x.is_cuda and x.dtype == torch.float32 and w.dtype == torch.float32 and x.dim() == 4 and w.dim() == 4):
        return False
    k = w.shape[2]
    if w.shape[3] != k or k not in (1, 3) or w.shape[1] != x.shape[3]:
        return False
    N, H, W, C = x.shape
    return bool(_lib.load().wc_conv_wrw_narrow_supported(N, H, W, w.shape[0], C, k))


def fast_conv(x, w, bias=None, kind='same'):
    if not supported(x, w, kind):
        raise _lib.WcHipError(f"fast_conv: unsupported call {tuple(x.shape)} x {tuple(w.shape)} ({kind})")
    return _FastConv.apply(x, w, bias, kind, _plan(kind, x, w))
```

### wc_gan_amd/csrc/wc_conv.hip

```cpp
#include "wc_common.h"
#include "../../include/wc_hip.h"
#include <stdlib.h>


namespace {

constexpr int kMaxTaps = 16, kMaxPhase = 4;

struct ConvArgs {
    const _Float16* xhi; const _Float16* xlo;
    const _Float16* zero;
    const char* wimg;
    const float* xscale; const float* wscale;
    const float* bias;
    float* y;
    int N, H, W, Hin, Win, Cin, Cout, in_stride, ntaps, nphase, Hout, Wout, out_stride, relu;
    unsigned magHW, shHW, magW, shW;
    int ksplit; float* partial;
    signed char dy[kMaxPhase][kMaxTaps], dx[kMaxPhase][kMaxTaps];
    signed char offy[kMaxPhase], offx[kMaxPhase];
};

__device__ __forceinline__ void lds_dma16(const void* g, unsigned lds)
{
    unsigned keep;
    asm volatile("s_mov_b32 %0, m0\n\ts_mov_b32 m0, %2\n\ts_nop 0\n\tglobal_load_lds_dwordx4 %1, off\n\ts_mov_b32 m0, %0"
                 : "=&s"(keep) : "v"(g), "s"(lds) : "memory");
}

template <int MB, int NB, bool KS>
__device__ __forceinline__ void conv_f16x3_body(const ConvArgs& a, const unsigned bx, const unsigned by, const unsigned bz)
{
    extern __shared__ __attribute__((aligned(16))) char smem[];
    constexpr int TM = 64 * MB, TN = 64 * NB;
    constexpr int A_BYTES = 2 * MB * 4 * 1024, B_BYTES = 2 * NB * 4 * 1024, STAGE = A_BYTES + B_BYTES;
    constexpr int AQ = (2 * MB) / 4;
    static_assert(AQ >= 1, "MB >= 2");

    const int tid = threadIdx.x, lane = tid & 63;
    const int wave = __builtin_amdgcn_readfirstlane(tid >> 6);
    const int wm = wave >> 1, wn = wave & 1;
    const int ntn = a.Cout / TN;
    const int phase = by / ntn, nt = by - phase * ntn;
    const unsigned m0 = bx * TM;
    const unsigned HW = a.H * a.W;
    const int koff = (lane >> 5) * 8;

    int gy[AQ], gx[AQ];
    unsigned gpix[AQ];
    #pragma unroll
    for (int q = 0; q < AQ; ++q) {
        const unsigned m = m0 + (wave * AQ + q) * 32 + (lane & 31);
        const unsigned n = __umulhi(m, a.magHW) >> a.shHW, rem = m - n * HW;
        const unsigned yy = __umulhi(rem, a.magW) >> a.shW, xx = rem - yy * a.W;
        gy[q] = yy * a.in_stride; gx[q] = xx * a.in_stride; gpix[q] = n * (a.Hin * a.Win);
    }
    const unsigned lds0 = (unsigned)(size_t)((__attribute__((address_space(3))) char*)smem);
    const int nchunk = a.Cin >> 5;
    const int iters = a.ntaps * nchunk;
    const int nblk_all = a.Cout >> 5;

    auto issue = [&](int it, int stage) {
        const int tap = it / nchunk, ch = it - tap * nchunk;
        const int dy = a.dy[phase][tap], dx = a.dx[phase][tap];
        const unsigned sbase = __builtin_amdgcn_readfirstlane(lds0 + stage * STAGE);
        #pragma unroll
        for (int q = 0; q < AQ; ++q) {
            const int iy = gy[q] + dy, ix = gx[q] + dx;
            const bool ok = (unsigned)iy < (unsigned)a.Hin && (unsigned)ix < (unsigned)a.Win;
            const int64_t e = ((int64_t)(gpix[q] + iy * a.Win + ix)) * a.Cin + ch * 32 + koff;
            #pragma unroll
            for (int s = 0; s < 2; ++s) {
                const _Float16* ph = ok ? a.xhi + e + s * 16 : a.zero + koff;
                const _Float16* pl = ok ? a.xlo + e + s * 16 : a.zero + koff;
                const unsigned l = sbase + (((wave * AQ + q) * 2 + s) * 2) * 1024;
                lds_dma16(ph, l);
                lds_dma16(pl, l + 1024);
            }
        }
        const char* wsrc = a.wimg + ((((int64_t)(phase * a.ntaps + tap) * nchunk + ch) * nblk_all + nt * 2 * NB) << 12);
        #pragma unroll
        for (int c = 0; c < 2 * NB; ++c) {
            const int idx = wave * 2 * NB + c;
            lds_dma16(wsrc + idx * 1024 + lane * 16, sbase + A_BYTES + idx * 1024);
        }
    };

    f32x16 acc[MB][NB];
    #pragma unroll
    for (int i = 0; i < MB; ++i)
        #pragma unroll
        for (int j = 0; j < NB; ++j)
            #pragma unroll
            for (int r = 0; r < 16; ++r) acc[i][j][r] = 0.f;

    const int it0 = KS ? (int)bz * iters / a.ksplit : 0, it1 = KS ? ((int)bz + 1) * iters / a.ksplit : iters;
    constexpr int NA = AQ * 4, ND = NA + 2 * NB, HALF = ND / 2, PER = 3 * MB * NB, GAP = PER / HALF;
    static_assert(PER % HALF == 0, "DMAs spread evenly");
    int tabv = 0;
    if (lane < a.ntaps) tabv = (a.dy[phase][lane] & 0xff) | ((a.dx[phase][lane] & 0xff) << 8);
    const char* pa[AQ][2];
    int pstep[AQ];
    const char* pw;
    unsigned sb_next = 0;
    auto prep = [&](int it, int stage) {
        const int tap = it / nchunk, ch = it - tap * nchunk;
        const int p = __builtin_amdgcn_readlane(tabv, tap);
        const int dy = (signed char)(p & 0xff), dx = (signed char)((p >> 8) & 0xff);
        #pragma unroll
        for (int q = 0; q < AQ; ++q) {
            const int iy = gy[q] + dy, ix = gx[q] + dx;
            const bool ok = (unsigned)iy < (unsigned)a.Hin && (unsigned)ix < (unsigned)a.Win;
            const int64_t e = ((int64_t)(gpix[q] + iy * a.Win + ix)) * a.Cin + ch * 32 + koff;
            pa[q][0] = reinterpret_cast<const char*>(ok ? a.xhi + e : a.zero + koff);
            pa[q][1] = reinterpret_cast<const char*>(ok ? a.xlo + e : a.zero + koff);
            pstep[q] = ok ? 32 : 0;
        }
        pw = a.wimg + ((((int64_t)(phase * a.ntaps + tap) * nchunk + ch) * nblk_all + nt * 2 * NB) << 12) + wave * (2 * NB * 1024) + lane * 16;
        sb_next = __builtin_amdgcn_readfirstlane(lds0 + stage * STAGE);
    };
    auto dma = [&](int d) {
        if (d < NA) {
            const int q = d >> 2, ks = (d >> 1) & 1, pl = d & 1;
            lds_dma16(pa[q][pl] + ks * pstep[q], sb_next + (((wave * AQ + q) * 2 + ks) * 2 + pl) * 1024);
        } else {
            const int c = d - NA;
            lds_dma16(pw + c * 1024, sb_next + A_BYTES + (wave * 2 * NB + c) * 1024);
        }
    };
    f16x8 fa[2][MB][2], fb[2][NB][2];
    auto frags = [&](int stage, int ks) {
        const char* sa = smem + stage * STAGE;
        const char* sb = sa + A_BYTES;
        #pragma unroll
        for (int i = 0; i < MB; ++i) {
            const char* p = sa + (((wm * MB + i) * 2 + ks) * 2) * 1024 + lane * 16;
            fa[ks][i][0] = *reinterpret_cast<const f16x8*>(p);
            fa[ks][i][1] = *reinterpret_cast<const f16x8*>(p + 1024);
        }
        #pragma unroll
        for (int j = 0; j < NB; ++j) {
            const char* p = sb + (((wn * NB + j) * 2 + ks) * 2) * 1024 + lane * 16;
            fb[ks][j][0] = *reinterpret_cast<const f16x8*>(p);
            fb[ks][j][1] = *reinterpret_cast<const f16x8*>(p + 1024);
        }
    };
    prep(it0, 0);
    #pragma unroll
    for (int d = 0; d < ND; ++d) dma(d);
    for (int it = it0; it < it1; ++it) {
        const int stage = (it - it0) & 1;
        __builtin_amdgcn_s_waitcnt(0x0F70);
        __syncthreads();
        frags(stage, 0);
        prep(it + 1 < it1 ? it + 1 : it, stage ^ 1);
        __builtin_amdgcn_sched_barrier(0);
        #pragma unroll
        for (int ks = 0; ks < 2; ++ks) {
            #pragma unroll
            for (int g = 0; g < PER; ++g) {
                const int prod = g / (MB * NB), i = (g / NB) % MB, j = g % NB;
                acc[i][j] = __builtin_amdgcn_mfma_f32_32x32x16_f16(fa[ks][i][prod == 0 ? 1 : 0], fb[ks][j][prod == 1 ? 1 : 0], acc[i][j], 0, 0, 0);
                if ((g + 1) % GAP == 0) {
                    dma(ks * HALF + g / GAP);
                    __builtin_amdgcn_sched_barrier(0);
                }
                if (ks == 0 && g == PER / 2) {
                    frags(stage, 1);
                    __builtin_amdgcn_sched_barrier(0);
                }
            }
        }
    }
    __builtin_amdgcn_s_waitcnt(0x0F70);
    const float inv = 1.0f / (a.xscale[0] * a.wscale[0]);
    const int oy0 = a.offy[phase], ox0 = a.offx[phase];
    float bj[NB];
    #pragma unroll
    for (int j = 0; j < NB; ++j) bj[j] = a.bias ? a.bias[nt * TN + (wn * NB + j) * 32 + (lane & 31)] : 0.f;
    #pragma unroll
    for (int i = 0; i < MB; ++i) {
        #pragma unroll
        for (int r = 0; r < 16; ++r) {
            const unsigned row = (r & 3) + 8 * (r >> 2) + 4 * (lane >> 5);
            const unsigned m = m0 + (wm * MB + i) * 32 + row;
            const unsigned n = __umulhi(m, a.magHW) >> a.shHW, rem = m - n * HW;
            const unsigned yy = __umulhi(rem, a.magW) >> a.shW, xx = rem - yy * a.W;
            const int64_t opix = ((int64_t)n * a.Hout + (yy * a.out_stride + oy0)) * a.Wout + (xx * a.out_stride + ox0);
            const int64_t oe = opix * a.Cout + nt * TN + wn * NB * 32 + (lane & 31);
            if (KS) {
                float* o = a.partial + (int64_t)bz * ((int64_t)a.N * a.Hout * a.Wout * a.Cout) + oe;
                #pragma unroll
                for (int j = 0; j < NB; ++j) o[j * 32] = acc[i][j][r];
            } else {
                float* o = a.y + oe;
                #pragma unroll
                for (int j = 0; j < NB; ++j) {
                    float v = acc[i][j][r] * inv + bj[j];
                    if (a.relu) v = fmaxf(v, 0.f);
                    o[j * 32] = v;
                }
            }
        }
    }
}

template <int MB, int NB, bool KS>
__global__ __launch_bounds__(256) void conv_f16x3_kernel(ConvArgs a) { conv_f16x3_body<MB, NB, KS>(a, blockIdx.x, blockIdx.y, blockIdx.z); }

struct KsplitReduceArgs {
    const float* partial; int ksplit; int64_t n4; int cout;
    const float* xscale; const float* wscale; const float* bias; int relu; float* y;
};

__device__ __forceinline__ void conv_ksplit_reduce_body(const float* __restrict__ partial, int ksplit, int64_t n4, int cout,
                                                        const float* __restrict__ xscale, const float* __restrict__ wscale,
                                                        const float* __restrict__ bias, int relu, float* __restrict__ y,
                                                        const unsigned bid, const unsigned nblocks)
{
    const float inv = 1.0f / (xscale[0] * wscale[0]);
    for (int64_t i = (int64_t)bid * 256 + threadIdx.x; i < n4; i += (int64_t)nblocks * 256) {
        f32x4 v = *reinterpret_cast<const f32x4*>(partial + 4 * i);
        int z = 1;
        for (; z + 3 < ksplit; z += 4) {
            f32x4 t[4];
            #pragma unroll
            for (int u = 0; u < 4; ++u) t[u] = *reinterpret_cast<const f32x4*>(partial + 4 * ((z + u) * n4 + i));
            #pragma unroll
            for (int u = 0; u < 4; ++u) v += t[u];
        }
        for (; z < ksplit; ++z) v += *reinterpret_cast<const f32x4*>(partial + 4 * (z * n4 + i));
        v = v * inv;
        if (bias) v += *reinterpret_cast<const f32x4*>(bias + (4 * i) % cout);
        if (relu) { v[0] = fmaxf(v[0], 0.f); v[1] = fmaxf(v[1], 0.f); v[2] = fmaxf(v[2], 0.f); v[3] = fmaxf(v[3], 0.f); }
        *reinterpret_cast<f32x4*>(y + 4 * i) = v;
    }
}

__global__ __launch_bounds__(256) void conv_ksplit_reduce_kernel(const float* __restrict__ partial, int ksplit, int64_t n4, int cout,
                                                                 const float* __restrict__ xscale, const float* __restrict__ wscale,
                                                                 const float* __restrict__ bias, int relu, float* __restrict__ y)
{
    conv_ksplit_reduce_body(partial, ksplit, n4, cout, xscale, wscale, bias, relu, y, blockIdx.x, gridDim.x);
}

__device__ __forceinline__ f32x4 split_act(f32x4 v, int relu, float slope)
{
    if (relu == 1) { v[0] = fmaxf(v[0], 0.f); v[1] = fmaxf(v[1], 0.f); v[2] = fmaxf(v[2], 0.f); v[3] = fmaxf(v[3], 0.f); }
    else if (relu == 2) {
        #pragma unroll
        for (int j = 0; j < 4; ++j) v[j] = v[j] > 0.f ? v[j] : slope * v[j];
    }
    return v;
}

constexpr int kAmaxBlocks = 512;

__global__ __launch_bounds__(256) void conv_absmax_kernel(const float* __restrict__ x, int64_t n4, int64_t n, float* __restrict__ partial,
                                                          float* __restrict__ colsum = nullptr, int c4n = 0, float leaky = -1.f)
{
    __shared__ float red[4];
    __shared__ f32x4 red4[256];
    float m = 0.f;
    f32x4 cs = {0.f, 0.f, 0.f, 0.f};
    for (int64_t i = blockIdx.x * 256 + threadIdx.x; i < n4; i += (int64_t)gridDim.x * 256) {
        const f32x4 v = *reinterpret_cast<const f32x4*>(x + 4 * i);
        const f32x4 u = leaky >= 0.f ? split_act(v, 2, leaky) : v;
        m = fmaxf(fmaxf(m, fabsf(u[0])), fmaxf(fabsf(u[1]), fmaxf(fabsf(u[2]), fabsf(u[3]))));
        cs += v;
    }
    if (blockIdx.x == 0 && threadIdx.x == 0) for (int64_t i = 4 * n4; i < n; ++i) m = fmaxf(m, fabsf(x[i]));
    #pragma unroll
    for (int o = 32; o > 0; o >>= 1) m = fmaxf(m, __shfl_xor(m, o));
    if ((threadIdx.x & 63) == 0) red[threadIdx.x >> 6] = m;
    if (colsum) red4[threadIdx.x] = cs;
    __syncthreads();
    if (threadIdx.x == 0) partial[blockIdx.x] = fmaxf(fmaxf(red[0], red[1]), fmaxf(red[2], red[3]));
    if (colsum && (int)threadIdx.x < c4n) {
        f32x4 t = red4[threadIdx.x];
        for (int p = threadIdx.x + c4n; p < 256; p += c4n) t += red4[p];
        *reinterpret_cast<f32x4*>(colsum + (int64_t)blockIdx.x * 4 * c4n + 4 * threadIdx.x) = t;
    }
}

__device__ __forceinline__ float scale_of(const float* __restrict__ partial, float mul = 1.0f, int count = kAmaxBlocks)
{
    float amax = 0.f;
    for (int i = threadIdx.x & 63; i < count; i += 64) amax = fmaxf(amax, partial[i]);
    #pragma unroll
    for (int o = 32; o > 0; o >>= 1) amax = fmaxf(amax, __shfl_xor(amax, o));
    amax *= mul;
    if (!(amax > 0.f) || !(amax < 3.0e38f)) return 1.0f;
    int e;
    (void)frexpf(amax, &e);
    return ldexpf(1.0f, 14 - e);
}

__global__ __launch_bounds__(256) void conv_leaky_bwd_kernel(float* __restrict__ dx, const float* __restrict__ x, int64_t n4, float slope)
{
    for (int64_t i = blockIdx.x * 256 + threadIdx.x; i < n4; i += (int64_t)gridDim.x * 256) {
        f32x4 g = *reinterpret_cast<const f32x4*>(dx + 4 * i);
        const f32x4 v = *reinterpret_cast<const f32x4*>(x + 4 * i);
        #pragma unroll
        for (int j = 0; j < 4; ++j) g[j] = v[j] > 0.f ? g[j] : slope * g[j];
        *reinterpret_cast<f32x4*>(dx + 4 * i) = g;
    }
}

__global__ __launch_bounds__(256) void conv_split_kernel(const float* __restrict__ x, int64_t n4, const float* __restrict__ amax,
                                                         int relu, _Float16* __restrict__ hi, _Float16* __restrict__ lo,
                                                         float* __restrict__ scale_out, float slope = 0.f)
{
    const float s = scale_of(amax);
    if (blockIdx.x == 0 && threadIdx.x == 0) scale_out[0] = s;
    for (int64_t i = blockIdx.x * 256 + threadIdx.x; i < n4; i += (int64_t)gridDim.x * 256) {
        f32x4 v = *reinterpret_cast<const f32x4*>(x + 4 * i);
        v = split_act(v, relu, slope);
        v = v * s;
        f16x4 h, l;
        #pragma unroll
        for (int j = 0; j < 4; ++j) { h[j] = (_Float16)v[j]; l[j] = (_Float16)(v[j] - (float)h[j]); }
        *reinterpret_cast<f16x4*>(hi + 4 * i) = h;
        *reinterpret_cast<f16x4*>(lo + 4 * i) = l;
    }
}

constexpr float kHistMargin = 64.0f;
constexpr int kHistArray = 2 * kAmaxBlocks;

__device__ __forceinline__ float scale_for(float amax)
{
    if (!(amax > 0.f) || !(amax < 3.0e38f)) return 1.0f;
    int e;
    (void)frexpf(amax, &e);
    return ldexpf(1.0f, 14 - e);
}

__global__ __launch_bounds__(kAmaxBlocks) void conv_hist_seed_kernel(float* __restrict__ hist)
{
    const float m = hist[threadIdx.x];
    __syncthreads();
    typedef float f32x2h __attribute__((ext_vector_type(2)));
    f32x2h a = {m, __builtin_bit_cast(float, 1u)}, b = {0.f, __builtin_bit_cast(float, 0u)};
    *reinterpret_cast<f32x2h*>(hist + 2 * threadIdx.x) = a;
    *reinterpret_cast<f32x2h*>(hist + kHistArray + 2 * threadIdx.x) = b;
    __shared__ float red[kAmaxBlocks / 64];
    float mm = m;
    #pragma unroll
    for (int o = 32; o > 0; o >>= 1) mm = fmaxf(mm, __shfl_xor(mm, o));
    if ((threadIdx.x & 63) == 0) red[threadIdx.x >> 6] = mm;
    __syncthreads();
    if (threadIdx.x == 0) {
        float t = 0.f;
        for (int i = 0; i < kAmaxBlocks / 64; ++i) t = fmaxf(t, red[i]);
        hist[2 * kHistArray + 2] = t; hist[2 * kHistArray + 3] = t;
    }
}

__global__ __launch_bounds__(256) void conv_split_hist_kernel(const float* __restrict__ x, int64_t n4, int relu, _Float16* __restrict__ hi,
                                                              _Float16* __restrict__ lo, float* __restrict__ scale_out,
                                                              float* __restrict__ hist, float* __restrict__ colsum, int c4n,
                                                              float slope = 0.f)
{
    __shared__ float red[4];
    __shared__ f32x4 red4[256];
    typedef float f32x2h __attribute__((ext_vector_type(2)));
    typedef int i32x2h __attribute__((ext_vector_type(2)));
    float mx[2] = {0.f, 0.f};
    int tlo[2] = {0x7fffffff, 0x7fffffff}, thi[2] = {0, 0};
    #pragma unroll
    for (int arr = 0; arr < 2; ++arr)
        #pragma unroll
        for (int i = 0; i < kAmaxBlocks / 64; ++i) {
            const i32x2h p = *reinterpret_cast<const i32x2h*>(hist + arr * kHistArray + 2 * ((threadIdx.x & 63) + 64 * i));
            mx[arr] = fmaxf(mx[arr], __builtin_bit_cast(float, p[0]));
            tlo[arr] = min(tlo[arr], p[1]);
            thi[arr] = max(thi[arr], p[1]);
        }
    #pragma unroll
    for (int o = 32; o > 0; o >>= 1)
        #pragma unroll
        for (int arr = 0; arr < 2; ++arr) {
            mx[arr] = fmaxf(mx[arr], __shfl_xor(mx[arr], o));
            tlo[arr] = min(tlo[arr], __shfl_xor(tlo[arr], o));
            thi[arr] = max(thi[arr], __shfl_xor(thi[arr], o));
        }
    const bool ok0 = tlo[0] == thi[0], ok1 = tlo[1] == thi[1];
    const int src = (ok1 && (!ok0 || thi[1] > thi[0])) ? 1 : 0;
    const int tag = (src ? thi[1] : thi[0]) + 1;
    const float prev = src ? mx[1] : mx[0];
    const float assumed = prev > 0.f ? prev : hist[2 * kHistArray + 2 + src];
    const float s = scale_for(assumed * kHistMargin);
    if (blockIdx.x == 0 && threadIdx.x == 0) { scale_out[0] = s; hist[2 * kHistArray + 2 + (1 - src)] = assumed; }
    float m = 0.f;
    f32x4 cs = {0.f, 0.f, 0.f, 0.f};
    for (int64_t i = blockIdx.x * 256 + threadIdx.x; i < n4; i += (int64_t)gridDim.x * 256) {
        f32x4 v = *reinterpret_cast<const f32x4*>(x + 4 * i);
        cs += v;
        v = split_act(v, relu, slope);
        m = fmaxf(fmaxf(m, fabsf(v[0])), fmaxf(fabsf(v[1]), fmaxf(fabsf(v[2]), fabsf(v[3]))));
        v = v * s;
        f16x4 h, l;
        #pragma unroll
        for (int j = 0; j < 4; ++j) { h[j] = (_Float16)v[j]; l[j] = (_Float16)(v[j] - (float)h[j]); }
        *reinterpret_cast<f16x4*>(hi + 4 * i) = h;
        *reinterpret_cast<f16x4*>(lo + 4 * i) = l;
    }
    #pragma unroll
    for (int o = 32; o > 0; o >>= 1) m = fmaxf(m, __shfl_xor(m, o));
    if ((threadIdx.x & 63) == 0) red[threadIdx.x >> 6] = m;
    if (colsum) red4[threadIdx.x] = cs;
    __syncthreads();
    if (threadIdx.x == 0) {
        const f32x2h p = {fmaxf(fmaxf(red[0], red[1]), fmaxf(red[2], red[3])), __builtin_bit_cast(float, tag)};
        *reinterpret_cast<f32x2h*>(hist + (1 - src) * kHistArray + 2 * blockIdx.x) = p;
    }
    if (colsum && (int)threadIdx.x < c4n) {
        f32x4 t = red4[threadIdx.x];
        for (int p = threadIdx.x + c4n; p < 256; p += c4n) t += red4[p];
        *reinterpret_cast<f32x4*>(colsum + (int64_t)blockIdx.x * 4 * c4n + 4 * threadIdx.x) = t;
    }
}

constexpr int kHistRedoWord = 2 * kHistArray;
__global__ __launch_bounds__(256) void conv_split_redo_kernel(const float* __restrict__ x, int64_t n4, int relu, _Float16* __restrict__ hi,
                                                              _Float16* __restrict__ lo, float* __restrict__ scale_out,
                                                              float* __restrict__ hist, float slope = 0.f)
{
    typedef int i32x2h __attribute__((ext_vector_type(2)));
    float mx[2] = {0.f, 0.f};
    int tg[2] = {0, 0};
    #pragma unroll
    for (int arr = 0; arr < 2; ++arr)
        #pragma unroll
        for (int i = 0; i < kAmaxBlocks / 64; ++i) {
            const i32x2h p = *reinterpret_cast<const i32x2h*>(hist + arr * kHistArray + 2 * ((threadIdx.x & 63) + 64 * i));
            mx[arr] = fmaxf(mx[arr], __builtin_bit_cast(float, p[0]));
            tg[arr] = max(tg[arr], p[1]);
        }
    #pragma unroll
    for (int o = 32; o > 0; o >>= 1)
        #pragma unroll
        for (int arr = 0; arr < 2; ++arr) {
            mx[arr] = fmaxf(mx[arr], __shfl_xor(mx[arr], o));
            tg[arr] = max(tg[arr], __shfl_xor(tg[arr], o));
        }
    const int now = tg[1] > tg[0] ? 1 : 0;
    const float own = mx[now], assumed = hist[2 * kHistArray + 2 + now];
    const float s_used = scale_for(assumed * kHistMargin);
    const float top = own * s_used;
    const bool fine = !(own > 0.f) || !(own < 3.0e38f) || (top >= 0.03125f && top < 65504.0f);
    if (fine) return;
    const float s = scale_for(own);
    if (blockIdx.x == 0 && threadIdx.x == 0) {
        scale_out[0] = s;
        reinterpret_cast<unsigned*>(hist)[kHistRedoWord] += 1u;
    }
    for (int64_t i = blockIdx.x * 256 + threadIdx.x; i < n4; i += (int64_t)gridDim.x * 256) {
        f32x4 v = *reinterpret_cast<const f32x4*>(x + 4 * i);
        v = split_act(v, relu, slope);
        v = v * s;
        f16x4 h, l;
        #pragma unroll
        for (int j = 0; j < 4; ++j) { h[j] = (_Float16)v[j]; l[j] = (_Float16)(v[j] - (float)h[j]); }
        *reinterpret_cast<f16x4*>(hi + 4 * i) = h;
        *reinterpret_cast<f16x4*>(lo + 4 * i) = l;
    }
}

struct WeightArgs {
    const float* w; int64_t sk, sn, sr, ss;
    const float* amax; float* scale_out; char* img;
    int K, Nn, ntaps, nphase;
    int64_t n4;
    float coef, bound_mul;
    int amax_count;
    signed char nsrc[kMaxPhase][kMaxTaps];
    signed char r[kMaxPhase][kMaxTaps][4], s[kMaxPhase][kMaxTaps][4];
};

__device__ __forceinline__ void conv_weights_body(const WeightArgs& a, const int bid, const int nblocks)
{
    float sc;
    if (a.amax) sc = scale_of(a.amax, a.bound_mul, a.amax_count);
    else {
        __shared__ float red[4];
        float m = 0.f;
        for (int64_t i = threadIdx.x; i < a.n4; i += 256) {
            const f32x4 v = *reinterpret_cast<const f32x4*>(a.w + 4 * i);
            m = fmaxf(fmaxf(m, fabsf(v[0])), fmaxf(fabsf(v[1]), fmaxf(fabsf(v[2]), fabsf(v[3]))));
        }
        #pragma unroll
        for (int o = 32; o > 0; o >>= 1) m = fmaxf(m, __shfl_xor(m, o));
        if ((threadIdx.x & 63) == 0) red[threadIdx.x >> 6] = m;
        __syncthreads();
        m = fmaxf(fmaxf(red[0], red[1]), fmaxf(red[2], red[3])) * a.bound_mul;
        sc = 1.0f;
        if (m > 0.f && m < 3.0e38f) { int e; (void)frexpf(m, &e); sc = ldexpf(1.0f, 14 - e); }
    }
    if (bid == 0 && threadIdx.x == 0) a.scale_out[0] = sc;
    const int nchunk = a.K >> 5, nblk = a.Nn >> 5;
    const int64_t groups = (int64_t)a.nphase * a.ntaps * nchunk * nblk * 2 * 64;
    for (int64_t g = (int64_t)bid * 256 + threadIdx.x; g < groups; g += (int64_t)nblocks * 256) {
        const int lane = g & 63;
        int64_t t = g >> 6;
        const int ks = t & 1; t >>= 1;
        const int nb = t % nblk; t /= nblk;
        const int ch = t % nchunk; t /= nchunk;
        const int tap = t % a.ntaps; const int ph = t / a.ntaps;
        const int n = nb * 32 + (lane & 31);
        const int k0 = ch * 32 + ks * 16 + (lane >> 5) * 8;
        const float* base = a.w + n * a.sn;
        const int ns = a.nsrc[ph][tap];
        float acc8[8] = {0.f, 0.f, 0.f, 0.f, 0.f, 0.f, 0.f, 0.f};
        for (int m = 0; m < ns; ++m) {
            const float* src = base + a.r[ph][tap][m] * a.sr + a.s[ph][tap][m] * a.ss;
            #pragma unroll
            for (int j = 0; j < 8; ++j) acc8[j] += src[(k0 + j) * a.sk];
        }
        const float cs = a.coef * sc;
        f16x8 h, l;
        #pragma unroll
        for (int j = 0; j < 8; ++j) {
            const float v = acc8[j] * cs;
            h[j] = (_Float16)v; l[j] = (_Float16)(v - (float)h[j]);
        }
        char* dst = a.img + (((((int64_t)(ph * a.ntaps + tap) * nchunk + ch) * nblk + nb) * 2 + ks) * 2) * 1024 + lane * 16;
        *reinterpret_cast<f16x8*>(dst) = h;
        *reinterpret_cast<f16x8*>(dst + 1024) = l;
    }
}

__global__ __launch_bounds__(256) void conv_weights_kernel(WeightArgs a) { conv_weights_body(a, blockIdx.x, gridDim.x); }

__global__ __launch_bounds__(256) void conv_weights_pair_kernel(WeightArgs a, WeightArgs b, int blocks_a)
{
    if ((int)blockIdx.x < blocks_a) conv_weights_body(a, blockIdx.x, blocks_a);
    else conv_weights_body(b, blockIdx.x - blocks_a, gridDim.x - blocks_a);
}

struct WrwOperand {
    const _Float16* hi; const _Float16* lo;
    int Hp, Wp, C, stride;
    signed char dy[kMaxPhase][kMaxTaps], dx[kMaxPhase][kMaxTaps];
};

struct WrwArgs {
    WrwOperand A, B;
    const _Float16* zero;
    float* partial;
    int N, H, W, ntaps, nphase;
    unsigned magHW, shHW, magW, shW;
    int nchunks, cps;
};

typedef short s16x4v __attribute__((__vector_size__(4 * sizeof(short))));

__device__ __forceinline__ f16x8 tr_read8(const char* block, int lane_off)
{
    auto p = (__attribute__((address_space(3))) s16x4v*)((__attribute__((address_space(3))) char*)(block + lane_off));
    auto q = (__attribute__((address_space(3))) s16x4v*)((__attribute__((address_space(3))) char*)(block + lane_off + 256));
    const s16x4v a = __builtin_amdgcn_ds_read_tr16_b64_v4i16(p);
    const s16x4v b = __builtin_amdgcn_ds_read_tr16_b64_v4i16(q);
    typedef short s16x8v __attribute__((__vector_size__(8 * sizeof(short))));
    const s16x8v ab = __builtin_shufflevector(a, b, 0, 1, 2, 3, 4, 5, 6, 7);
    return __builtin_bit_cast(f16x8, ab);
}

template <int MB, int NB>
__device__ __forceinline__ void conv_wrw_body(const WrwArgs& a, const unsigned bx, const unsigned by)
{
    extern __shared__ __attribute__((aligned(16))) char smem[];
    constexpr int TA = 64 * MB, TB = 64 * NB;
    constexpr int A_BYTES = 2 * MB * 4 * 1024, B_BYTES = 2 * NB * 4 * 1024, STAGE = A_BYTES + B_BYTES;
    constexpr int AQ = (2 * MB) / 4, BQ = (2 * NB) / 4;
    constexpr bool ONE = MB == 1 && NB == 1;
    static_assert(ONE || (MB >= 2 && NB >= 2), "a wave stages whole blocks of both operands, or one block of one");

    const int tid = threadIdx.x, lane = tid & 63;
    const int wave = __builtin_amdgcn_readfirstlane(tid >> 6);
    const int wm = wave >> 1, wn = wave & 1;
    const int nta = a.A.C / TA, ntb = a.B.C / TB;
    int idx = by;
    const int tb = idx % ntb; idx /= ntb;
    const int ta = idx % nta; idx /= nta;
    const int tap = idx % a.ntaps, phase = idx / a.ntaps;
    const int c0 = bx * a.cps, c1 = min(c0 + a.cps, a.nchunks);
    const int dya = a.A.dy[phase][tap], dxa = a.A.dx[phase][tap], dyb = a.B.dy[phase][tap], dxb = a.B.dx[phase][tap];
    const unsigned HW = a.H * a.W;
    const unsigned lds0 = (unsigned)(size_t)((__attribute__((address_space(3))) char*)smem);
    const int c8 = (lane & 3) * 8;

    auto issue = [&](int c, int stage) {
        const unsigned sbase = __builtin_amdgcn_readfirstlane(lds0 + stage * STAGE);
        #pragma unroll
        for (int s = 0; s < 2; ++s) {
            const unsigned m = c * 32 + s * 16 + (lane >> 2);
            const unsigned n = __umulhi(m, a.magHW) >> a.shHW, rem = m - n * HW;
            const unsigned yy = __umulhi(rem, a.magW) >> a.shW, xx = rem - yy * a.W;
            const int ay = yy * a.A.stride + dya, ax = xx * a.A.stride + dxa;
            const int by = yy * a.B.stride + dyb, bx = xx * a.B.stride + dxb;
            const bool oka = (unsigned)ay < (unsigned)a.A.Hp && (unsigned)ax < (unsigned)a.A.Wp;
            const bool okb = (unsigned)by < (unsigned)a.B.Hp && (unsigned)bx < (unsigned)a.B.Wp;
            const int64_t ea = ((int64_t)((n * a.A.Hp + ay) * a.A.Wp + ax)) * a.A.C + ta * TA + c8;
            const int64_t eb = ((int64_t)((n * a.B.Hp + by) * a.B.Wp + bx)) * a.B.C + tb * TB + c8;
            #pragma unroll
            for (int q = 0; q < AQ; ++q) {
                const int b = wave * AQ + q;
// ... 370 lines not shown
        const unsigned yy = __umulhi(rem, a.magW) >> a.shW, xx = rem - yy * a.W;
        const int pb = (int)pc * a.Cin;
#pragma unroll
        for (int s = 0; s < KS; ++s) {
            const int dy = (signed char)(dyx[s] & 0xff), dx = (signed char)((dyx[s] >> 8) & 0xff), kind = dyx[s] >> 16;
            const bool inb = kind == 0 && (unsigned)((int)yy + dy) < (unsigned)a.H && (unsigned)((int)xx + dx) < (unsigned)a.W;
            const float xv = a.x[inb ? pb + off[s] : 0];
            av[s] = inb ? xv : (kind == 1 ? 1.f : 0.f);
        }
    };
    float av[KS], an[KS];
    if (t0 < t1) gather(t0, av);
    for (int t = t0; t < t1; ++t) {
        if (t + 1 < t1) gather(t + 1, an);
        f32x16 acc[kNarrowNQ];
#pragma unroll
        for (int q = 0; q < kNarrowNQ; ++q)
#pragma unroll
            for (int r = 0; r < 16; ++r) acc[q][r] = 0.f;
#pragma unroll
        for (int s = 0; s < KS; ++s)
#pragma unroll
            for (int q = 0; q < kNarrowNQ; ++q) acc[q] = __builtin_amdgcn_mfma_f32_32x32x2f32(av[s], bw[s][q], acc[q], 0, 0, 0);
        float* tl = nf_tile + wave * (32 * kNarrowLd);
#pragma unroll
        for (int r = 0; r < 16; ++r) {
            const int row = (r & 3) + 8 * (r >> 2) + 4 * k;
#pragma unroll
            for (int q = 0; q < kNarrowNQ; ++q) {
                float v = acc[q][r];
                if (a.relu) v = fmaxf(v, 0.f);
                tl[row * kNarrowLd + q * 32 + i] = v;
            }
        }
        __builtin_amdgcn_s_waitcnt(0xc07f);
#pragma unroll
        for (int j = 0; j < 8; ++j) {
            const int row = 4 * j + (lane >> 4);
            const int64_t pr = (int64_t)t * 32 + row;
            const f32x4 v = *reinterpret_cast<const f32x4*>(tl + row * kNarrowLd + 4 * (lane & 15));
            if (pr < a.M) *reinterpret_cast<f32x4*>(a.y + pr * a.Cout + grp * (32 * kNarrowNQ) + 4 * (lane & 15)) = v;
        }
#pragma unroll
        for (int s = 0; s < KS; ++s) av[s] = an[s];
    }
}

void magic_u31(unsigned d, unsigned* mag, unsigned* sh)
{
    unsigned s = 0;
    while ((1u << s) < d) ++s;
    const unsigned long long num = 1ull << (31 + s);
    *mag = (unsigned)((num + d - 1) / d);
    *sh = s - 1;
}

int grid_for(int64_t work_items)
{
    int64_t g = (work_items + 255) / 256;
    return (int)(g < 1 ? 1 : (g > 2048 ? 2048 : g));
}

template <int MB, int NB, bool KS = false>
hipError_t launch_conv(const ConvArgs& a, hipStream_t st)
{
    constexpr int LDS = 2 * (2 * MB * 4 * 1024 + 2 * NB * 4 * 1024);
    hipError_t e = wc_set_max_lds(reinterpret_cast<const void*>(conv_f16x3_kernel<MB, NB, KS>), LDS);
    if (e != hipSuccess) return e;
    const int64_t M = (int64_t)a.N * a.H * a.W;
    dim3 grid((unsigned)(M / (64 * MB)), (unsigned)(a.nphase * (a.Cout / (64 * NB))), (unsigned)a.ksplit);
    hipLaunchKernelGGL((conv_f16x3_kernel<MB, NB, KS>), grid, dim3(256), LDS, st, a);
    return hipGetLastError();
}

}

extern "C" {

static int split_measured(const float* x, int64_t n, int relu, float slope, void* hi, void* lo, float* scale, void* amax_scratch,
                          float* colsum_partials, int C, hipStream_t st)
{
    if (!x || !hi || !lo || !scale || !amax_scratch || n <= 0 || (n & 3)) return WC_ERR_ARG;
    if (colsum_partials && (C <= 0 || (C & 3) || 256 % (C >> 2) != 0 || n % C != 0)) return WC_ERR_SHAPE;
    hipLaunchKernelGGL(conv_absmax_kernel, dim3(kAmaxBlocks), dim3(256), 0, st, x, n / 4, n, (float*)amax_scratch,
                       colsum_partials, colsum_partials ? C >> 2 : 0, relu == 2 ? slope : -1.f);
    hipLaunchKernelGGL(conv_split_kernel, dim3(grid_for(n / 4)), dim3(256), 0, st, x, n / 4, (const float*)amax_scratch, relu,
                       (_Float16*)hi, (_Float16*)lo, scale, slope);
    return (int)hipGetLastError();
}

static int split_hist(const float* x, int64_t n, int relu, float slope, void* hi, void* lo, float* scale, float* colsum_partials, int C,
                      float* hist, int bootstrap, hipStream_t st)
{
    if (!x || !hi || !lo || !scale || !hist || n <= 0 || (n & 3)) return WC_ERR_ARG;
    if (colsum_partials && (C <= 0 || (C & 3) || 256 % (C >> 2) != 0 || n % C != 0)) return WC_ERR_SHAPE;
    if (bootstrap & 1) {
        hipLaunchKernelGGL(conv_absmax_kernel, dim3(kAmaxBlocks), dim3(256), 0, st, x, n / 4, n, hist, colsum_partials, colsum_partials ? C >> 2 : 0,
                           relu == 2 ? slope : -1.f);
        hipLaunchKernelGGL(conv_split_kernel, dim3(grid_for(n / 4)), dim3(256), 0, st, x, n / 4, (const float*)hist, relu, (_Float16*)hi,
                           (_Float16*)lo, scale, slope);
        hipLaunchKernelGGL(conv_hist_seed_kernel, dim3(1), dim3(kAmaxBlocks), 0, st, hist);
        return (int)hipGetLastError();
    }
    hipLaunchKernelGGL(conv_split_hist_kernel, dim3(kAmaxBlocks), dim3(256), 0, st, x, n / 4, relu, (_Float16*)hi, (_Float16*)lo, scale,
                       hist, colsum_partials, colsum_partials ? C >> 2 : 0, slope);
    if (!(bootstrap & 2)) {
        const unsigned g2 = grid_for(n / 4) < 64u ? grid_for(n / 4) : 64u;
        hipLaunchKernelGGL(conv_split_redo_kernel, dim3(g2), dim3(256), 0, st, x, n / 4, relu, (_Float16*)hi, (_Float16*)lo, scale, hist, slope);
    }
    return (int)hipGetLastError();
}

int wc_conv_split_f32(const float* x, int64_t n, int relu, void* hi, void* lo, float* scale, void* amax_scratch, wc_stream_t stream)
{
    return wc_conv_split_colsum_f32(x, n, relu, hi, lo, scale, amax_scratch, nullptr, 0, stream);
}

int wc_conv_split_colsum_f32(const float* x, int64_t n, int relu, void* hi, void* lo, float* scale, void* amax_scratch,
                             float* colsum_partials, int C, wc_stream_t stream)
{
    return split_measured(x, n, relu ? 1 : 0, 0.f, hi, lo, scale, amax_scratch, colsum_partials, C, (hipStream_t)stream);
}

int wc_conv_split_hist_f32(const float* x, int64_t n, int relu, void* hi, void* lo, float* scale, float* colsum_partials, int C,
                           float* hist, int bootstrap, wc_stream_t stream)
{
    return split_hist(x, n, relu ? 1 : 0, 0.f, hi, lo, scale, colsum_partials, C, hist, bootstrap, (hipStream_t)stream);
}

int wc_conv_split_leaky_f32(const float* x, int64_t n, float negative_slope, void* hi, void* lo, float* scale, void* amax_scratch,
                            float* colsum_partials, int C, wc_stream_t stream)
{
    if (!(negative_slope >= 0.f && negative_slope <= 1.f)) return WC_ERR_ARG;
    return split_measured(x, n, negative_slope == 0.f ? 1 : 2, negative_slope, hi, lo, scale, amax_scratch, colsum_partials, C, (hipStream_t)stream);
}

int wc_conv_split_hist_leaky_f32(const float* x, int64_t n, float negative_slope, void* hi, void* lo, float* scale, float* colsum_partials, int C,
                                 float* hist, int bootstrap, wc_stream_t stream)
{
    if (!(negative_slope >= 0.f && negative_slope <= 1.f)) return WC_ERR_ARG;
    return split_hist(x, n, negative_slope == 0.f ? 1 : 2, negative_slope, hi, lo, scale, colsum_partials, C, hist, bootstrap, (hipStream_t)stream);
}

int wc_conv_leaky_bwd_f32(float* dx, const float* x, int64_t n, float negative_slope, wc_stream_t stream)
{
    if (!dx || !x || n <= 0 || (n & 3)) return WC_ERR_ARG;
    hipLaunchKernelGGL(conv_leaky_bwd_kernel, dim3(grid_for(n / 4)), dim3(256), 0, (hipStream_t)stream, dx, x, n / 4, negative_slope);
    return (int)hipGetLastError();
}

size_t wc_conv_weights_bytes(const wc_conv_geom* g)
{
    if (!g) return 0;
    return (size_t)g->nphase * g->ntaps * g->Cin * g->Cout * 4;
}

static int fill_weight_args(WeightArgs& a, const float* w, int64_t stride_k, int64_t stride_n, int64_t stride_r, int64_t stride_s,
                            int64_t n_elems, const wc_conv_geom* g, void* image, float* scale, const float* amax, int amax_count)
{
    if (g->ntaps < 1 || g->ntaps > kMaxTaps || g->nphase < 1 || g->nphase > kMaxPhase || (g->Cin & 31) || (g->Cout & 31)) return WC_ERR_ARG;
    a.w = w; a.sk = stride_k; a.sn = stride_n; a.sr = stride_r; a.ss = stride_s;
    a.amax = amax; a.amax_count = amax_count; a.scale_out = scale; a.img = (char*)image;
    a.n4 = n_elems / 4;
    a.K = g->Cin; a.Nn = g->Cout; a.ntaps = g->ntaps; a.nphase = g->nphase;
    int most = 1;
    for (int p = 0; p < kMaxPhase; ++p)
        for (int t = 0; t < kMaxTaps; ++t) {
            a.nsrc[p][t] = g->nsrc[p][t];
            if (p < g->nphase && t < g->ntaps) {
                if (g->nsrc[p][t] < 1 || g->nsrc[p][t] > 4) return WC_ERR_ARG;
                if (g->nsrc[p][t] > most) most = g->nsrc[p][t];
            }
            for (int m = 0; m < 4; ++m) { a.r[p][t][m] = g->wr[p][t][m]; a.s[p][t][m] = g->ws[p][t][m]; }
        }
    a.coef = g->wcoef; a.bound_mul = fabsf(g->wcoef) * most;
    return WC_OK;
}

int wc_conv_weights_f32(const float* w, int64_t stride_k, int64_t stride_n, int64_t stride_r, int64_t stride_s, int64_t n_elems,
                        const wc_conv_geom* g, void* image, float* scale, void* amax_scratch,
                        const float* known_amax, int known_count, wc_stream_t stream)
{
    hipStream_t st = (hipStream_t)stream;
    if (!w || !g || !image || !scale || (!amax_scratch && !known_amax) || n_elems <= 0) return WC_ERR_ARG;
    if (known_amax && (known_count < 1 || known_count > 4096)) return WC_ERR_ARG;
    const bool inline_max = !known_amax && n_elems <= 32768 && (n_elems & 3) == 0 && ((uintptr_t)w & 15) == 0;
    if (!inline_max && !known_amax) hipLaunchKernelGGL(conv_absmax_kernel, dim3(kAmaxBlocks), dim3(256), 0, st, w, n_elems / 4, n_elems, (float*)amax_scratch);
    WeightArgs a;
    const int rc = fill_weight_args(a, w, stride_k, stride_n, stride_r, stride_s, n_elems, g, image, scale,
                                    inline_max ? nullptr : (known_amax ? known_amax : (const float*)amax_scratch), known_amax ? known_count : kAmaxBlocks);
    if (rc != WC_OK) return rc;
    const int64_t groups = (int64_t)g->nphase * g->ntaps * (g->Cin >> 5) * (g->Cout >> 5) * 128;
    hipLaunchKernelGGL(conv_weights_kernel, dim3(grid_for(groups)), dim3(256), 0, st, a);
    return (int)hipGetLastError();
}

int wc_conv_weights_pair_f32(const float* w, int64_t stride_r, int64_t stride_s, int64_t n_elems,
                             int64_t a_stride_k, int64_t a_stride_n, const wc_conv_geom* ga, void* image_a,
                             int64_t b_stride_k, int64_t b_stride_n, const wc_conv_geom* gb, void* image_b,
                             float* scale, void* amax_scratch, const float* known_amax, int known_count, wc_stream_t stream)
{
    hipStream_t st = (hipStream_t)stream;
    if (!w || !ga || !gb || !image_a || !image_b || !scale || (!amax_scratch && !known_amax) || n_elems <= 0) return WC_ERR_ARG;
    if (known_amax && (known_count < 1 || known_count > 4096)) return WC_ERR_ARG;
    if (!known_amax) hipLaunchKernelGGL(conv_absmax_kernel, dim3(kAmaxBlocks), dim3(256), 0, st, w, n_elems / 4, n_elems, (float*)amax_scratch);
    const float* amax = known_amax ? known_amax : (const float*)amax_scratch;
    const int cnt = known_amax ? known_count : kAmaxBlocks;
    WeightArgs a, b;
    int rc = fill_weight_args(a, w, a_stride_k, a_stride_n, stride_r, stride_s, n_elems, ga, image_a, scale, amax, cnt);
    if (rc != WC_OK) return rc;
    rc = fill_weight_args(b, w, b_stride_k, b_stride_n, stride_r, stride_s, n_elems, gb, image_b, scale + 1, amax, cnt);
    if (rc != WC_OK) return rc;
    if (a.bound_mul != b.bound_mul) return WC_ERR_ARG;
    const int blocks_a = grid_for((int64_t)ga->nphase * ga->ntaps * (ga->Cin >> 5) * (ga->Cout >> 5) * 128);
    const int blocks_b = grid_for((int64_t)gb->nphase * gb->ntaps * (gb->Cin >> 5) * (gb->Cout >> 5) * 128);
    hipLaunchKernelGGL(conv_weights_pair_kernel, dim3(blocks_a + blocks_b), dim3(256), 0, st, a, b, blocks_a);
    return (int)hipGetLastError();
}

int wc_conv_supported(const wc_conv_geom* g)
{
    if (!g) return 0;
    if (g->ntaps < 1 || g->ntaps > kMaxTaps || g->nphase < 1 || g->nphase > kMaxPhase) return 0;
    if ((g->Cin & 31) || (g->Cout & 63)) return 0;
    const int64_t M = (int64_t)g->N * g->H * g->W;
    if (M <= 0 || (M & 127) || M > (int64_t)1 << 31) return 0;
    if ((int64_t)g->N * g->Hin * g->Win > (int64_t)1 << 31) return 0;
    if (g->W < 2 || g->H < 1) return 0;
    return 1;
}

constexpr int kKsplitMaxWgs = 96;
constexpr int kKsplitTargetWgs = 256;
constexpr int kWrwTargetWgs = 512;

static int conv_ksplit(const wc_conv_geom* g)
{
    const int64_t M = (int64_t)g->N * g->H * g->W;
    const bool wide = (g->Cout % 256) == 0;
    const int64_t wgs = (M / 128) * g->nphase * (g->Cout / (wide ? 256 : (g->Cout % 128) ? 64 : 128));
    const int iters = g->ntaps * (g->Cin / 32);
    if (wgs > kKsplitMaxWgs || iters < 8) return 1;
    int k = (int)((kKsplitTargetWgs + wgs - 1) / wgs);
    if (k > iters / 4) k = iters / 4;
    return k < 1 ? 1 : (k > 8 ? 8 : k);
}

size_t wc_conv_workspace_bytes(const wc_conv_geom* g)
{
    if (!g) return 0;
    const int k = conv_ksplit(g);
    return k > 1 ? (size_t)k * g->N * g->Hout * g->Wout * g->Cout * 4 : 0;
}

static bool conv_big_tile(const wc_conv_geom* g, int ksplit)
{
    const int64_t M = (int64_t)g->N * g->H * g->W;
    const bool wide = (g->Cout % 256) == 0;
    const int64_t wgs_big = (M / 256) * g->nphase * (g->Cout / (wide ? 256 : 128));
    return ksplit == 1 && (M % 256) == 0 && wgs_big >= 256;
}

static int conv_prepare(ConvArgs& a, const void* xhi, const void* xlo, const float* xscale, const void* wimage, const float* wscale,
                        const float* bias, const void* zero_line, const wc_conv_geom* g, int relu, float* y, void* ws, size_t ws_bytes)
{
    if (!xhi || !xlo || !xscale || !wimage || !wscale || !zero_line || !g || !y) return WC_ERR_ARG;
    if (!wc_conv_supported(g)) return WC_ERR_SHAPE;
    a.xhi = (const _Float16*)xhi; a.xlo = (const _Float16*)xlo; a.zero = (const _Float16*)zero_line;
    a.wimg = (const char*)wimage; a.xscale = xscale; a.wscale = wscale; a.bias = bias; a.y = y;
    a.N = g->N; a.H = g->H; a.W = g->W; a.Hin = g->Hin; a.Win = g->Win; a.Cin = g->Cin; a.Cout = g->Cout;
    a.in_stride = g->in_stride; a.ntaps = g->ntaps; a.nphase = g->nphase; a.Hout = g->Hout; a.Wout = g->Wout;
    a.out_stride = g->out_stride; a.relu = relu;
    a.ksplit = conv_ksplit(g); a.partial = (float*)ws;
    magic_u31((unsigned)(g->H * g->W), &a.magHW, &a.shHW);
    magic_u31((unsigned)g->W, &a.magW, &a.shW);
    if (a.ksplit > 1 && (!ws || ws_bytes < wc_conv_workspace_bytes(g))) return WC_ERR_WORKSPACE;
    for (int p = 0; p < kMaxPhase; ++p) {
        a.offy[p] = g->off_y[p]; a.offx[p] = g->off_x[p];
        for (int t = 0; t < kMaxTaps; ++t) { a.dy[p][t] = g->dy[p][t]; a.dx[p][t] = g->dx[p][t]; }
    }
    return WC_OK;
}

int wc_conv_f16x3(const void* xhi, const void* xlo, const float* xscale, const void* wimage, const float* wscale,
                  const float* bias, const void* zero_line, const wc_conv_geom* g, int relu, float* y,
                  void* ws, size_t ws_bytes, wc_stream_t stream)
{
    hipStream_t st = (hipStream_t)stream;
    ConvArgs a;
    const int rc = conv_prepare(a, xhi, xlo, xscale, wimage, wscale, bias, zero_line, g, relu, y, ws, ws_bytes);
    if (rc != WC_OK) return rc;
    const bool wide = (g->Cout % 256) == 0;
    hipError_t e;
    if (g->Cout % 128)                                      e = a.ksplit > 1 ? launch_conv<2, 1, true>(a, st) : launch_conv<2, 1>(a, st);
    else if (conv_big_tile(g, a.ksplit))                    e = wide ? launch_conv<4, 4>(a, st) : launch_conv<4, 2>(a, st);
    else if (a.ksplit > 1)                                  e = wide ? launch_conv<2, 4, true>(a, st) : launch_conv<2, 2, true>(a, st);
    else                                                    e = wide ? launch_conv<2, 4>(a, st) : launch_conv<2, 2>(a, st);
    if (e != hipSuccess) return (int)e;
    if (a.ksplit > 1) {
        const int64_t n4 = (int64_t)g->N * g->Hout * g->Wout * g->Cout / 4;
        hipLaunchKernelGGL(conv_ksplit_reduce_kernel, dim3(grid_for(n4)), dim3(256), 0, st, (const float*)ws, a.ksplit, n4, g->Cout,
                           xscale, wscale, bias, relu, y);
    }
    return (int)hipGetLastError();
}

static int wrw_splits(const wc_conv_geom* g, int* tile)
{
    const bool wide = (g->Cin % 256 == 0) && (g->Cout % 256 == 0) && g->nphase * g->ntaps * (g->Cin / 256) * (g->Cout / 256) >= 4;
    *tile = wide ? 256 : ((g->Cin % 128) || (g->Cout % 128)) ? 64 : 128;
    const int tiles = g->nphase * g->ntaps * (g->Cin / *tile) * (g->Cout / *tile);
    const int64_t nchunks = (int64_t)g->N * g->H * g->W / 32;
    int splits = kWrwTargetWgs / tiles / 8 * 8;
    if (splits < 8) splits = 8;
    if (splits > 64) splits = 64;
    if (splits > nchunks) splits = (int)nchunks;
    return splits < 1 ? 1 : splits;
}

int wc_conv_wrw_narrow_supported(int64_t N, int64_t H, int64_t W, int Cin, int Cout, int ksize);
int wc_conv_narrow64_supported(int64_t N, int64_t H, int64_t W, int Cin, int Cout, int ksize);

int wc_conv_fwd_narrow_f32(const float* x, const float* w, int64_t stride_k, int64_t stride_n, int64_t stride_r, int64_t stride_s,
                           const float* bias, int64_t N, int64_t H, int64_t W, int Cin, int Cout, int ksize, int relu, float* y, wc_stream_t stream)
{
    if (!x || !w || !y) return WC_ERR_ARG;
    if (!wc_conv_narrow64_supported(N, H, W, Cin, Cout, ksize) || N * H * W * Cin >= ((int64_t)1 << 31)) return WC_ERR_SHAPE;
    hipStream_t st = (hipStream_t)stream;
    NarrowFwdArgs a = {};
    a.x = x; a.w = w; a.bias = bias; a.y = y;
    a.N = (int)N; a.H = (int)H; a.W = (int)W; a.Cin = Cin; a.Cout = Cout; a.ks = ksize; a.nrow = ksize * ksize * Cin; a.relu = relu;
    a.sk = stride_k; a.sn = stride_n; a.sr = stride_r; a.ss = stride_s;
    magic_u31((unsigned)(H * W), &a.magHW, &a.shHW);
    magic_u31((unsigned)W, &a.magW, &a.shW);
    for (int m = 0; m < 32; ++m) {
        const int tap = m < a.nrow ? m / Cin : 0, c = m < a.nrow ? m % Cin : 0;
        a.tr[m] = (signed char)(tap / ksize); a.ts[m] = (signed char)(tap % ksize); a.tch[m] = (signed char)c;
        a.tdy[m] = (signed char)(tap / ksize - ksize / 2); a.tdx[m] = (signed char)(tap % ksize - ksize / 2);
    }
    a.M = N * H * W;
    a.ntiles = (int)((a.M + 31) / 32);
    a.tiles_per_wave = (a.ntiles + 1023) / 1024;
    if (a.tiles_per_wave < 1) a.tiles_per_wave = 1;
    const int nwg = (a.ntiles + 4 * a.tiles_per_wave - 1) / (4 * a.tiles_per_wave);
    const int ks2 = (a.nrow + 2) / 2;
    dim3 grid(nwg, Cout / (32 * kNarrowNQ));
    if (ks2 <= 2) hipLaunchKernelGGL(conv_fwd_narrow_kernel<2>, grid, dim3(256), 0, st, a);
    else if (ks2 <= 5) hipLaunchKernelGGL(conv_fwd_narrow_kernel<5>, grid, dim3(256), 0, st, a);
    else if (ks2 <= 10) hipLaunchKernelGGL(conv_fwd_narrow_kernel<10>, grid, dim3(256), 0, st, a);
    else if (ks2 <= 14) hipLaunchKernelGGL(conv_fwd_narrow_kernel<14>, grid, dim3(256), 0, st, a);
    else hipLaunchKernelGGL(conv_fwd_narrow_kernel<16>, grid, dim3(256), 0, st, a);
    return (int)hipGetLastError();
}

static int64_t narrow_wrw_parts(int64_t M, int64_t* pix_per_wave)
{
    int64_t ppw = (M + 256 * 8 - 1) / (256 * 8);
    if (ppw < 16) ppw = 16;
    ppw = (ppw + 1) & ~(int64_t)1;
    *pix_per_wave = ppw;
    return (M + 8 * ppw - 1) / (8 * ppw);
}

int wc_conv_narrow64_supported(int64_t N, int64_t H, int64_t W, int Cin, int Cout, int ksize)
{
    if (N <= 0 || H <= 0 || W <= 0 || Cin <= 0 || Cout <= 0 || (ksize != 1 && ksize != 3)) return 0;
    if (ksize * ksize * Cin >= 32 || (Cout & 63)) return 0;
    return N * H * W < ((int64_t)1 << 31) ? 1 : 0;
}

int wc_conv_wrw_narrow_supported(int64_t N, int64_t H, int64_t W, int Cin, int Cout, int ksize)
{
    return ((Cout & 127) == 0 && wc_conv_narrow64_supported(N, H, W, Cin, Cout, ksize)) ? 1 : 0;
}

size_t wc_conv_wrw_narrow64_workspace_bytes(int64_t N, int64_t H, int64_t W, int Cin, int Cout, int ksize)
{
    if (!wc_conv_narrow64_supported(N, H, W, Cin, Cout, ksize)) return 0;
    int64_t ppw;
    return (size_t)narrow_wrw_parts(N * H * W, &ppw) * ((Cout + 127) / 128) * 4096 * sizeof(float);
}

size_t wc_conv_wrw_narrow_workspace_bytes(int64_t N, int64_t H, int64_t W, int Cin, int Cout, int ksize)
{
    return wc_conv_wrw_narrow_supported(N, H, W, Cin, Cout, ksize) ? wc_conv_wrw_narrow64_workspace_bytes(N, H, W, Cin, Cout, ksize) : 0;
}

int wc_conv_wrw_narrow64_f32(const float* x, const float* gy, int64_t N, int64_t H, int64_t W, int Cin, int Cout, int ksize,
                             float* dw, int64_t stride_k, int64_t stride_n, int64_t stride_r, int64_t stride_s, float* db,
                             void* ws, size_t ws_bytes, wc_stream_t stream)
{
    if (!x || !gy || !dw || !ws) return WC_ERR_ARG;
    if (!wc_conv_narrow64_supported(N, H, W, Cin, Cout, ksize)) return WC_ERR_SHAPE;
    if (ws_bytes < wc_conv_wrw_narrow64_workspace_bytes(N, H, W, Cin, Cout, ksize)) return WC_ERR_WORKSPACE;
    hipStream_t st = (hipStream_t)stream;
    NarrowWrwArgs a = {};
    a.x = x; a.gy = gy; a.partial = (float*)ws;
    a.N = (int)N; a.H = (int)H; a.W = (int)W; a.Cin = Cin; a.Cout = Cout; a.ks = ksize; a.nrow = ksize * ksize * Cin;
    magic_u31((unsigned)(H * W), &a.magHW, &a.shHW);
    magic_u31((unsigned)W, &a.magW, &a.shW);
    a.M = N * H * W;
    const int nparts = (int)narrow_wrw_parts(a.M, &a.pix_per_wave);
    const int ngrp = (Cout + 127) / 128;
    constexpr int lds = 8 * 4096 * 4;
    hipError_t e = wc_set_max_lds(reinterpret_cast<const void*>(conv_wrw_narrow_kernel), lds);
    if (e != hipSuccess) return (int)e;
    hipLaunchKernelGGL(conv_wrw_narrow_kernel, dim3(nparts, ngrp), dim3(512), lds, st, a);
    hipLaunchKernelGGL(conv_wrw_narrow_reduce_kernel, dim3(128, ngrp), dim3(256), 0, st, (const float*)ws, nparts, Cin, ksize, a.nrow,
                       dw, stride_k, stride_n, stride_r, stride_s, db, Cout);
    return (int)hipGetLastError();
}

int wc_conv_wrw_narrow_f32(const float* x, const float* gy, int64_t N, int64_t H, int64_t W, int Cin, int Cout, int ksize,
                           float* dw, int64_t stride_k, int64_t stride_n, int64_t stride_r, int64_t stride_s, float* db,
                           void* ws, size_t ws_bytes, wc_stream_t stream)
{
    if (!x || !gy || !dw || !ws) return WC_ERR_ARG;
    if (!wc_conv_wrw_narrow_supported(N, H, W, Cin, Cout, ksize)) return WC_ERR_SHAPE;
    return wc_conv_wrw_narrow64_f32(x, gy, N, H, W, Cin, Cout, ksize, dw, stride_k, stride_n, stride_r, stride_s, db, ws, ws_bytes, stream);
}

size_t wc_conv_wrw_workspace_bytes(const wc_conv_geom* g)
{
    if (!g) return 0;
    int tile;
    return (size_t)wrw_splits(g, &tile) * g->nphase * g->ntaps * g->Cin * g->Cout * 4;
}

int wc_conv_wrw_f16x3(const void* xhi, const void* xlo, const float* xscale, const void* ghi, const void* glo, const float* gscale,
                      const void* zero_line, const wc_conv_geom* g, float* dw, int64_t stride_k, int64_t stride_n,
                      int64_t stride_r, int64_t stride_s, void* ws, size_t ws_bytes, wc_stream_t stream)
{
    return wc_conv_wrw_bias_f16x3(xhi, xlo, xscale, ghi, glo, gscale, zero_line, g, dw, stride_k, stride_n, stride_r, stride_s,
                                  nullptr, nullptr, ws, ws_bytes, stream);
}

struct WrwPlan { WrwArgs a; WrwReduceArgs r; int T, splits, tiles, extra; };

static int wrw_prepare(WrwPlan& p, const void* xhi, const void* xlo, const float* xscale, const void* ghi, const void* glo, const float* gscale,
                       const void* zero_line, const wc_conv_geom* g, float* dw, int64_t stride_k, int64_t stride_n,
                       int64_t stride_r, int64_t stride_s, const float* colsum_partials, float* db, void* ws, size_t ws_bytes)
{
    if (!xhi || !xlo || !xscale || !ghi || !glo || !gscale || !zero_line || !g || !dw || !ws) return WC_ERR_NULL;
    if (!wc_conv_supported(g) || (g->Cin & 63) || g->W < 2 || g->H * g->W < 2) return WC_ERR_SHAPE;
    if (ws_bytes < wc_conv_wrw_workspace_bytes(g)) return WC_ERR_WORKSPACE;
    if ((colsum_partials == nullptr) != (db == nullptr)) return WC_ERR_NULL;
    if (db && ((g->Cout & 3) || 256 % (g->Cout >> 2) != 0)) return WC_ERR_SHAPE;
    WrwArgs& a = p.a;
    WrwReduceArgs& r = p.r;
    int T;
    int splits = wrw_splits(g, &T);
    const int64_t M = (int64_t)g->N * g->H * g->W;
    const int nslice = g->nphase * g->ntaps;
    const int tiles = nslice * (g->Cin / T) * (g->Cout / T);
    const int nchunks = (int)(M / 32);
    WrwOperand X, G;
    X.hi = (const _Float16*)xhi; X.lo = (const _Float16*)xlo; X.Hp = g->Hin; X.Wp = g->Win; X.C = g->Cin; X.stride = g->in_stride;
    G.hi = (const _Float16*)ghi; G.lo = (const _Float16*)glo; G.Hp = g->Hout; G.Wp = g->Wout; G.C = g->Cout; G.stride = g->out_stride;
    r.nout = 0; r.coef = g->wcoef;
    for (int ph = 0; ph < kMaxPhase; ++ph)
        for (int t = 0; t < kMaxTaps; ++t) {
            X.dy[ph][t] = g->dy[ph][t]; X.dx[ph][t] = g->dx[ph][t];
            G.dy[ph][t] = g->off_y[ph]; G.dx[ph][t] = g->off_x[ph];
            if (ph >= g->nphase || t >= g->ntaps) continue;
            if (g->nsrc[ph][t] < 1 || g->nsrc[ph][t] > 4) return WC_ERR_ARG;
            for (int m = 0; m < g->nsrc[ph][t]; ++m) {
                int o = 0;
                while (o < r.nout && (r.r[o] != g->wr[ph][t][m] || r.s[o] != g->ws[ph][t][m])) ++o;
                if (o == r.nout) {
                    if (r.nout == kMaxTaps) return WC_ERR_ARG;
                    r.r[o] = g->wr[ph][t][m]; r.s[o] = g->ws[ph][t][m]; r.cnt[o] = 0; ++r.nout;
                }
                if (r.cnt[o] == 4) return WC_ERR_ARG;
                r.slice[o][r.cnt[o]++] = (signed char)(ph * g->ntaps + t);
            }
        }
    const bool x_cols = stride_k == 1;
    a.A = x_cols ? G : X; a.B = x_cols ? X : G;
    a.zero = (const _Float16*)zero_line; a.partial = (float*)ws;
    a.N = g->N; a.H = g->H; a.W = g->W; a.ntaps = g->ntaps; a.nphase = g->nphase;
    magic_u31((unsigned)(g->H * g->W), &a.magHW, &a.shHW);
    magic_u31((unsigned)g->W, &a.magW, &a.shW);
    a.nchunks = nchunks; a.cps = (nchunks + splits - 1) / splits;
    splits = (nchunks + a.cps - 1) / a.cps;
    r.partial = (const float*)ws; r.splits = splits; r.nslice = nslice; r.Ca = a.A.C; r.Cb = a.B.C;
    r.xscale = xscale; r.gscale = gscale; r.dw = dw;
    r.sa = x_cols ? stride_n : stride_k; r.sb = x_cols ? stride_k : stride_n; r.sr = stride_r; r.ss = stride_s;
    r.colsum = colsum_partials; r.db = db; r.c4n = db ? g->Cout >> 2 : 0;
    r.main_blocks = grid_for((int64_t)r.nout * g->Cin * g->Cout);
    p.T = T; p.splits = splits; p.tiles = tiles; p.extra = db ? (r.c4n * 64 + 255) / 256 : 0;
    return WC_OK;
}

int wc_conv_wrw_bias_f16x3(const void* xhi, const void* xlo, const float* xscale, const void* ghi, const void* glo, const float* gscale,
                           const void* zero_line, const wc_conv_geom* g, float* dw, int64_t stride_k, int64_t stride_n,
                           int64_t stride_r, int64_t stride_s, const float* colsum_partials, float* db,
                           void* ws, size_t ws_bytes, wc_stream_t stream)
{
    hipStream_t st = (hipStream_t)stream;
    WrwPlan p;
    const int rc = wrw_prepare(p, xhi, xlo, xscale, ghi, glo, gscale, zero_line, g, dw, stride_k, stride_n, stride_r, stride_s,
                               colsum_partials, db, ws, ws_bytes);
    if (rc != WC_OK) return rc;
    const WrwArgs& a = p.a;
    const WrwReduceArgs& r = p.r;
    const int T = p.T;
    dim3 grid((unsigned)p.splits, (unsigned)p.tiles);
    hipError_t e = hipSuccess;
    if (T == 256) {
        constexpr int LDS = 2 * (2 * 4 * 4 * 1024 + 2 * 4 * 4 * 1024);
        e = wc_set_max_lds(reinterpret_cast<const void*>(conv_wrw_kernel<4, 4>), LDS);
        if (e != hipSuccess) return (int)e;
        hipLaunchKernelGGL((conv_wrw_kernel<4, 4>), grid, dim3(256), LDS, st, a);
    } else if (T == 64) {
        constexpr int LDS = 2 * (2 * 1 * 4 * 1024 + 2 * 1 * 4 * 1024);
        e = wc_set_max_lds(reinterpret_cast<const void*>(conv_wrw_kernel<1, 1>), LDS);
        if (e != hipSuccess) return (int)e;
        hipLaunchKernelGGL((conv_wrw_kernel<1, 1>), grid, dim3(256), LDS, st, a);
    } else {
        constexpr int LDS = 2 * (2 * 2 * 4 * 1024 + 2 * 2 * 4 * 1024);
        e = wc_set_max_lds(reinterpret_cast<const void*>(conv_wrw_kernel<2, 2>), LDS);
        if (e != hipSuccess) return (int)e;
        hipLaunchKernelGGL((conv_wrw_kernel<2, 2>), grid, dim3(256), LDS, st, a);
    }
    hipLaunchKernelGGL(conv_wrw_reduce_kernel, dim3(r.main_blocks + p.extra), dim3(256), 0, st, r);
    return (int)hipGetLastError();
}

int wc_conv_bwd_pair_supported(const wc_conv_geom* gd, const wc_conv_geom* gf)
{
    if (!gd || !gf || !wc_conv_supported(gd) || !wc_conv_supported(gf) || (gf->Cin & 63) || gf->H * gf->W < 2) return 0;
    if (gd->N != gf->N || gd->Cin != gf->Cout || gd->Cout != gf->Cin) return 0;
    if (gd->Hin != gf->Hout || gd->Win != gf->Wout || gd->Hout != gf->Hin || gd->Wout != gf->Win) return 0;
    if (gf->nphase != 1 || gd->in_stride != 1) return 0;
    if ((gd->Cout % 128) != 0 || (gd->Cout % 256) == 0 || conv_big_tile(gd, conv_ksplit(gd))) return 0;
    int tile;
    (void)wrw_splits(gf, &tile);
    return tile == 128 ? 1 : 0;
}

size_t wc_conv_bwd_pair_workspace_bytes(const wc_conv_geom* gd, const wc_conv_geom* gf)
{
    if (!gd || !gf) return 0;
    return wc_conv_workspace_bytes(gd) + wc_conv_wrw_workspace_bytes(gf);
}

int wc_conv_bwd_pair_f16x3(const void* ghi, const void* glo, const float* gscale, const void* wimage, const float* wscale,
                           const void* zero_line, const wc_conv_geom* gd, float* dx, void* ws_dx, size_t ws_dx_bytes,
                           const void* xhi, const void* xlo, const float* xscale, const wc_conv_geom* gf, float* dw,
                           int64_t stride_k, int64_t stride_n, int64_t stride_r, int64_t stride_s,
                           const float* colsum_partials, float* db, void* ws_dw, size_t ws_dw_bytes, wc_stream_t stream)
{
    hipStream_t st = (hipStream_t)stream;
    ConvArgs d;
    int rc = conv_prepare(d, ghi, glo, gscale, wimage, wscale, nullptr, zero_line, gd, 0, dx, ws_dx, ws_dx_bytes);
    if (rc != WC_OK) return rc;
    WrwPlan p;
    rc = wrw_prepare(p, xhi, xlo, xscale, ghi, glo, gscale, zero_line, gf, dw, stride_k, stride_n, stride_r, stride_s,
                     colsum_partials, db, ws_dw, ws_dw_bytes);
    if (rc != WC_OK) return rc;
    if (!wc_conv_bwd_pair_supported(gd, gf) || p.T != 128) return WC_ERR_SHAPE;
    constexpr int LDS = 2 * (2 * 2 * 4 * 1024 + 2 * 2 * 4 * 1024);
    const int64_t M = (int64_t)gd->N * gd->H * gd->W;
    const int gx = (int)(M / 128), gy = gd->nphase * (gd->Cout / 128);
    const int64_t conv_blocks = (int64_t)gx * gy * d.ksplit, wrw_off = (conv_blocks + 7) & ~(int64_t)7;
    const int64_t blocks = wrw_off + (int64_t)p.splits * p.tiles;
    if (blocks > 0x7fffffff) return WC_ERR_SHAPE;
    hipError_t e;
    if (d.ksplit > 1) {
        e = wc_set_max_lds(reinterpret_cast<const void*>(conv_bwd_pair_kernel<true>), LDS);
        if (e != hipSuccess) return (int)e;
        hipLaunchKernelGGL((conv_bwd_pair_kernel<true>), dim3((unsigned)blocks), dim3(256), LDS, st, d, p.a,
                           (int)conv_blocks, (int)wrw_off, p.splits, gx, gy);
    } else {
        e = wc_set_max_lds(reinterpret_cast<const void*>(conv_bwd_pair_kernel<false>), LDS);
        if (e != hipSuccess) return (int)e;
        hipLaunchKernelGGL((conv_bwd_pair_kernel<false>), dim3((unsigned)blocks), dim3(256), LDS, st, d, p.a,
                           (int)conv_blocks, (int)wrw_off, p.splits, gx, gy);
    }
    e = hipGetLastError();
    if (e != hipSuccess) return (int)e;
    const int reduce_blocks = p.r.main_blocks + p.extra;
    if (d.ksplit > 1) {
        KsplitReduceArgs k;
        k.n4 = (int64_t)gd->N * gd->Hout * gd->Wout * gd->Cout / 4;
        k.partial = (const float*)ws_dx; k.ksplit = d.ksplit; k.cout = gd->Cout;
        k.xscale = gscale; k.wscale = wscale; k.bias = nullptr; k.relu = 0; k.y = dx;
        hipLaunchKernelGGL(conv_pair_reduce_kernel, dim3(reduce_blocks + grid_for(k.n4)), dim3(256), 0, st, p.r, k, reduce_blocks);
    } else {
        hipLaunchKernelGGL(conv_wrw_reduce_kernel, dim3(reduce_blocks), dim3(256), 0, st, p.r);
    }
    return (int)hipGetLastError();
}

}
```

### wc_gan_amd/csrc/wc_gp.hip

```cpp
#include "wc_common.h"
#include "../../include/wc_hip.h"

namespace {

constexpr int kAmaxBlocks = 512;
constexpr float kHistMargin = 64.0f;
constexpr int kHistArray = 2 * kAmaxBlocks;
constexpr int kHistRedoWord = 2 * kHistArray;

__device__ __forceinline__ f32x4 masked_load(const float* __restrict__ t, const float* __restrict__ a, int64_t i, float slope)
{
    f32x4 v = *reinterpret_cast<const f32x4*>(t + 4 * i);
    const f32x4 p = *reinterpret_cast<const f32x4*>(a + 4 * i);
    #pragma unroll
    for (int j = 0; j < 4; ++j) v[j] = v[j] * (p[j] > 0.f ? 1.0f : slope);
    return v;
}

__device__ __forceinline__ float absmax4(float m, f32x4 v)
{
    return fmaxf(fmaxf(m, fabsf(v[0])), fmaxf(fabsf(v[1]), fmaxf(fabsf(v[2]), fabsf(v[3]))));
}

__device__ __forceinline__ void store_split(f32x4 v, float s, _Float16* __restrict__ hi, _Float16* __restrict__ lo, int64_t i)
{
    v = v * s;
    f16x4 h, l;
    #pragma unroll
    for (int j = 0; j < 4; ++j) { h[j] = (_Float16)v[j]; l[j] = (_Float16)(v[j] - (float)h[j]); }
    *reinterpret_cast<f16x4*>(hi + 4 * i) = h;
    *reinterpret_cast<f16x4*>(lo + 4 * i) = l;
}

__device__ __forceinline__ float scale_for(float amax)
{
    if (!(amax > 0.f) || !(amax < 3.0e38f)) return 1.0f;
    int e;
    (void)frexpf(amax, &e);
    return ldexpf(1.0f, 14 - e);
}

__device__ __forceinline__ float wave_max(float m)
{
    #pragma unroll
    for (int o = 32; o > 0; o >>= 1) m = fmaxf(m, __shfl_xor(m, o));
    return m;
}

__global__ __launch_bounds__(256) void gp_absmax_kernel(const float* __restrict__ t, const float* __restrict__ a, int64_t n4, float slope,
                                                        float* __restrict__ partial)
{
    __shared__ float red[4];
    float m = 0.f;
    for (int64_t i = blockIdx.x * 256 + threadIdx.x; i < n4; i += (int64_t)gridDim.x * 256) m = absmax4(m, masked_load(t, a, i, slope));
    m = wave_max(m);
    if ((threadIdx.x & 63) == 0) red[threadIdx.x >> 6] = m;
    __syncthreads();
    if (threadIdx.x == 0) partial[blockIdx.x] = fmaxf(fmaxf(red[0], red[1]), fmaxf(red[2], red[3]));
}

__global__ __launch_bounds__(256) void gp_split_kernel(const float* __restrict__ t, const float* __restrict__ a, int64_t n4, float slope,
                                                       const float* __restrict__ amax, _Float16* __restrict__ hi, _Float16* __restrict__ lo,
                                                       float* __restrict__ scale_out)
{
    float m = 0.f;
    for (int i = threadIdx.x & 63; i < kAmaxBlocks; i += 64) m = fmaxf(m, amax[i]);
    const float s = scale_for(wave_max(m));
    if (blockIdx.x == 0 && threadIdx.x == 0) scale_out[0] = s;
    for (int64_t i = blockIdx.x * 256 + threadIdx.x; i < n4; i += (int64_t)gridDim.x * 256) store_split(masked_load(t, a, i, slope), s, hi, lo, i);
}

typedef float f32x2h __attribute__((ext_vector_type(2)));
typedef int i32x2h __attribute__((ext_vector_type(2)));

__global__ __launch_bounds__(kAmaxBlocks) void gp_hist_seed_kernel(float* __restrict__ hist)
{
    const float m = hist[threadIdx.x];
    __syncthreads();
    const f32x2h a = {m, __builtin_bit_cast(float, 1u)}, b = {0.f, __builtin_bit_cast(float, 0u)};
    *reinterpret_cast<f32x2h*>(hist + 2 * threadIdx.x) = a;
    *reinterpret_cast<f32x2h*>(hist + kHistArray + 2 * threadIdx.x) = b;
    __shared__ float red[kAmaxBlocks / 64];
    const float mm = wave_max(m);
    if ((threadIdx.x & 63) == 0) red[threadIdx.x >> 6] = mm;
    __syncthreads();
    if (threadIdx.x == 0) {
        float top = 0.f;
        for (int i = 0; i < kAmaxBlocks / 64; ++i) top = fmaxf(top, red[i]);
        hist[2 * kHistArray + 2] = top; hist[2 * kHistArray + 3] = top;
    }
}

__global__ __launch_bounds__(256) void gp_split_hist_kernel(const float* __restrict__ t, const float* __restrict__ a, int64_t n4, float slope,
                                                            _Float16* __restrict__ hi, _Float16* __restrict__ lo, float* __restrict__ scale_out,
                                                            float* __restrict__ hist)
{
    __shared__ float red[4];
    float mx[2] = {0.f, 0.f};
    int tlo[2] = {0x7fffffff, 0x7fffffff}, thi[2] = {0, 0};
    #pragma unroll
    for (int arr = 0; arr < 2; ++arr)
        #pragma unroll
        for (int i = 0; i < kAmaxBlocks / 64; ++i) {
            const i32x2h p = *reinterpret_cast<const i32x2h*>(hist + arr * kHistArray + 2 * ((threadIdx.x & 63) + 64 * i));
            mx[arr] = fmaxf(mx[arr], __builtin_bit_cast(float, p[0]));
            tlo[arr] = min(tlo[arr], p[1]);
            thi[arr] = max(thi[arr], p[1]);
        }
    #pragma unroll
    for (int o = 32; o > 0; o >>= 1)
        #pragma unroll
        for (int arr = 0; arr < 2; ++arr) {
            mx[arr] = fmaxf(mx[arr], __shfl_xor(mx[arr], o));
            tlo[arr] = min(tlo[arr], __shfl_xor(tlo[arr], o));
            thi[arr] = max(thi[arr], __shfl_xor(thi[arr], o));
        }
    const bool ok0 = tlo[0] == thi[0], ok1 = tlo[1] == thi[1];
    const int src = (ok1 && (!ok0 || thi[1] > thi[0])) ? 1 : 0;
    const int tag = (src ? thi[1] : thi[0]) + 1;
    const float prev = src ? mx[1] : mx[0];
    const float assumed = prev > 0.f ? prev : hist[2 * kHistArray + 2 + src];
    const float s = scale_for(assumed * kHistMargin);
    if (blockIdx.x == 0 && threadIdx.x == 0) { scale_out[0] = s; hist[2 * kHistArray + 2 + (1 - src)] = assumed; }
    float m = 0.f;
    for (int64_t i = blockIdx.x * 256 + threadIdx.x; i < n4; i += (int64_t)gridDim.x * 256) {
        const f32x4 v = masked_load(t, a, i, slope);
        m = absmax4(m, v);
        store_split(v, s, hi, lo, i);
    }
    m = wave_max(m);
    if ((threadIdx.x & 63) == 0) red[threadIdx.x >> 6] = m;
    __syncthreads();
    if (threadIdx.x == 0) {
        const f32x2h p = {fmaxf(fmaxf(red[0], red[1]), fmaxf(red[2], red[3])), __builtin_bit_cast(float, tag)};
        *reinterpret_cast<f32x2h*>(hist + (1 - src) * kHistArray + 2 * blockIdx.x) = p;
    }
}

__global__ __launch_bounds__(256) void gp_split_redo_kernel(const float* __restrict__ t, const float* __restrict__ a, int64_t n4, float slope,
                                                            _Float16* __restrict__ hi, _Float16* __restrict__ lo, float* __restrict__ scale_out,
                                                            float* __restrict__ hist)
{
    float mx[2] = {0.f, 0.f};
    int tg[2] = {0, 0};
    #pragma unroll
    for (int arr = 0; arr < 2; ++arr)
        #pragma unroll
        for (int i = 0; i < kAmaxBlocks / 64; ++i) {
            const i32x2h p = *reinterpret_cast<const i32x2h*>(hist + arr * kHistArray + 2 * ((threadIdx.x & 63) + 64 * i));
            mx[arr] = fmaxf(mx[arr], __builtin_bit_cast(float, p[0]));
            tg[arr] = max(tg[arr], p[1]);
        }
    #pragma unroll
    for (int o = 32; o > 0; o >>= 1)
        #pragma unroll
        for (int arr = 0; arr < 2; ++arr) {
            mx[arr] = fmaxf(mx[arr], __shfl_xor(mx[arr], o));
            tg[arr] = max(tg[arr], __shfl_xor(tg[arr], o));
        }
    const int now = tg[1] > tg[0] ? 1 : 0;
    const float own = mx[now], assumed = hist[2 * kHistArray + 2 + now];
    const float top = own * scale_for(assumed * kHistMargin);
    const bool fine = !(own > 0.f) || !(own < 3.0e38f) || (top >= 0.03125f && top < 65504.0f);
    if (fine) return;
    const float s = scale_for(own);
    if (blockIdx.x == 0 && threadIdx.x == 0) {
        scale_out[0] = s;
        reinterpret_cast<unsigned*>(hist)[kHistRedoWord] += 1u;
    }
    for (int64_t i = blockIdx.x * 256 + threadIdx.x; i < n4; i += (int64_t)gridDim.x * 256) store_split(masked_load(t, a, i, slope), s, hi, lo, i);
}

int grid_for(int64_t work_items)
{
    const int64_t g = (work_items + 255) / 256;
    return (int)(g < 1 ? 1 : (g > 2048 ? 2048 : g));
}

__global__ __launch_bounds__(256) void gp_interp_kernel(const float* __restrict__ real, const float* __restrict__ fake, const float* __restrict__ eps,
                                                        int64_t total, int64_t L, float* __restrict__ out)
{
    for (int64_t i = (int64_t)blockIdx.x * 256 + threadIdx.x; i < total; i += (int64_t)gridDim.x * 256) {
        const double e = (double)eps[i / L];
        out[i] = (float)(e * (double)real[i] + (1.0 - e) * (double)fake[i]);
    }
}

__global__ __launch_bounds__(256) void gp_rows_kernel(const float* __restrict__ g, int64_t L, double two_lambda_over_n, float* __restrict__ norms,
                                                      float* __restrict__ v, double* __restrict__ terms)
{
    __shared__ double red[4];
    const float* row = g + (int64_t)blockIdx.x * L;
    float* out = v + (int64_t)blockIdx.x * L;
    double ss = 0.0;
    for (int64_t i = threadIdx.x; i < L; i += 256) { const double x = (double)row[i]; ss += x * x; }
    #pragma unroll
    for (int o = 32; o > 0; o >>= 1) ss += __shfl_xor(ss, o);
    if ((threadIdx.x & 63) == 0) red[threadIdx.x >> 6] = ss;
    __syncthreads();
    const double norm = sqrt((red[0] + red[1]) + (red[2] + red[3]));
    const double coef = norm > 0.0 ? two_lambda_over_n * (1.0 - 1.0 / norm) : 0.0;
    if (threadIdx.x == 0) { norms[blockIdx.x] = (float)norm; terms[blockIdx.x] = (norm - 1.0) * (norm - 1.0); }
    for (int64_t i = threadIdx.x; i < L; i += 256) out[i] = (float)(coef * (double)row[i]);
}

__global__ __launch_bounds__(64) void gp_finish_kernel(const double* __restrict__ terms, int64_t N, double lambda_over_n, float* __restrict__ penalty)
{
    double s = 0.0;
    for (int64_t i = threadIdx.x; i < N; i += 64) s += terms[i];
    #pragma unroll
    for (int o = 32; o > 0; o >>= 1) s += __shfl_xor(s, o);
    if (threadIdx.x == 0) penalty[0] = (float)(lambda_over_n * s);
}

}

extern "C" {

int wc_conv_split_masked_f32(const float* t, const float* a, int64_t n, float slope, void* hi, void* lo, float* scale, void* amax_scratch,
                             wc_stream_t stream)
{
    if (!t || !a || !hi || !lo || !scale || !amax_scratch || n <= 0 || (n & 3)) return WC_ERR_ARG;
    if (!(slope >= 0.f && slope <= 1.f)) return WC_ERR_ARG;
    hipStream_t st = (hipStream_t)stream;
    hipLaunchKernelGGL(gp_absmax_kernel, dim3(kAmaxBlocks), dim3(256), 0, st, t, a, n / 4, slope, (float*)amax_scratch);
    hipLaunchKernelGGL(gp_split_kernel, dim3(grid_for(n / 4)), dim3(256), 0, st, t, a, n / 4, slope, (const float*)amax_scratch,
                       (_Float16*)hi, (_Float16*)lo, scale);
    return (int)hipGetLastError();
}

int wc_conv_split_hist_masked_f32(const float* t, const float* a, int64_t n, float slope, void* hi, void* lo, float* scale, float* hist,
                                  int bootstrap, wc_stream_t stream)
{
    if (!t || !a || !hi || !lo || !scale || !hist || n <= 0 || (n & 3)) return WC_ERR_ARG;
    if (!(slope >= 0.f && slope <= 1.f)) return WC_ERR_ARG;
    hipStream_t st = (hipStream_t)stream;
    if (bootstrap & 1) {
        hipLaunchKernelGGL(gp_absmax_kernel, dim3(kAmaxBlocks), dim3(256), 0, st, t, a, n / 4, slope, hist);
        hipLaunchKernelGGL(gp_split_kernel, dim3(grid_for(n / 4)), dim3(256), 0, st, t, a, n / 4, slope, (const float*)hist, (_Float16*)hi,
                           (_Float16*)lo, scale);
        hipLaunchKernelGGL(gp_hist_seed_kernel, dim3(1), dim3(kAmaxBlocks), 0, st, hist);
        return (int)hipGetLastError();
    }
    hipLaunchKernelGGL(gp_split_hist_kernel, dim3(kAmaxBlocks), dim3(256), 0, st, t, a, n / 4, slope, (_Float16*)hi, (_Float16*)lo, scale, hist);
    if (!(bootstrap & 2)) {
        const unsigned g2 = grid_for(n / 4) < 64 ? grid_for(n / 4) : 64u;
        hipLaunchKernelGGL(gp_split_redo_kernel, dim3(g2), dim3(256), 0, st, t, a, n / 4, slope, (_Float16*)hi, (_Float16*)lo, scale, hist);
    }
    return (int)hipGetLastError();
}

int wc_gp_interp_f32(const float* real, const float* fake, const float* eps, int64_t N, int64_t L, float* x_hat, wc_stream_t stream)
{
    if (!real || !fake || !eps || !x_hat) return WC_ERR_NULL;
    if (N <= 0 || L <= 0) return WC_ERR_SHAPE;
    hipLaunchKernelGGL(gp_interp_kernel, dim3(grid_for(N * L)), dim3(256), 0, (hipStream_t)stream, real, fake, eps, N * L, L, x_hat);
    return (int)hipGetLastError();
}

size_t wc_gp_rows_workspace_bytes(int64_t N) { return N > 0 ? (size_t)N * sizeof(double) : 0; }

int wc_gp_rows_f32(const float* g, int64_t N, int64_t L, double lambda, double inv_n, float* norms, float* v, float* penalty,
                   void* ws, size_t ws_bytes, wc_stream_t stream)
{
    if (!g || !norms || !v || !penalty || !ws) return WC_ERR_NULL;
    if (N <= 0 || L <= 0 || N >= ((int64_t)1 << 31)) return WC_ERR_SHAPE;
    if (ws_bytes < wc_gp_rows_workspace_bytes(N)) return WC_ERR_WORKSPACE;
    hipStream_t st = (hipStream_t)stream;
    hipLaunchKernelGGL(gp_rows_kernel, dim3((unsigned)N), dim3(256), 0, st, g, L, 2.0 * lambda * inv_n, norms, v, (double*)ws);
    hipLaunchKernelGGL(gp_finish_kernel, dim3(1), dim3(64), 0, st, (const double*)ws, N, lambda * inv_n, penalty);
    return (int)hipGetLastError();
}

}
```

### wc_gan_amd/discriminator.py

```python
from __future__ import annotations

from functools import partial

import torch
import torch.nn as nn
import torch.nn.functional as F

from .generator import Conv2D, create_norm, to_nchw_view, to_nhwc


def downsample2x(x):
    return to_nhwc(F.avg_pool2d(to_nchw_view(x), 2))


class ResBlockDown(nn.Module):
    def __init__(self, in_ch, nfilters, resample, name, norm, conv_layer, is_first):
        super().__init__()
        assert resample in ('DOWN', 'SAME')
        self.resample, self.is_first = resample, is_first
        self.bn1 = norm(axis=-1, name=name + '.bn1', channels=in_ch)
        self.conv1 = conv_layer(in_ch, nfilters, (3, 3), name=name + '.conv1')
        self.bn2 = norm(axis=-1, name=name + '.bn2', channels=nfilters)
        self.conv2 = conv_layer(nfilters, nfilters, (3, 3), name=name + '.conv2')
        self.has_shortcut = (in_ch != nfilters) or resample == 'DOWN'
        if self.has_shortcut:
            self.shortcut = conv_layer(in_ch, nfilters, (1, 1), name=name + '.shortcut')

    def forward(self, x, cls):
        h = self.conv1(x) if self.is_first else self.conv1.forward_relu(self.bn1(x, cls))
        h = self.bn2(h, cls)
        s = x
        if self.resample == 'DOWN':
            from . import generator as _g
            if h.shape[1] * h.shape[2] >= 1024 or (_g.FAST_CONV and h.is_cuda):
                h = self.conv2.forward_pooled(h, relu_input=True)
            else:
                h = downsample2x(self.conv2.forward_relu(h))
            s = downsample2x(s)
        else:
            h = self.conv2.forward_relu(h)
        if self.has_shortcut:
            s = self.shortcut(s)
        return h + s


LEAKY_SLOPE = 0.3


class DCBlockDown(nn.Module):

    def __init__(self, in_ch, nfilters, resample, name, norm, conv_layer, is_first):
        super().__init__()
        assert resample in ('DOWN', 'SAME')
        self.resample, self.is_first = resample, is_first
        self.bn = norm(axis=-1, name=name + '.bn', channels=in_ch)
        if resample == 'DOWN':
            self.conv = conv_layer(in_ch, nfilters, (4, 4), name=name + '.conv', stride=2)
        else:
            self.conv = conv_layer(in_ch, nfilters, (3, 3), name=name + '.conv')

    def forward(self, x, cls):
        if self.is_first:
            return self.conv(x)
        return self.conv.forward_leaky(self.bn(x, cls), LEAKY_SLOPE)


class Discriminator(nn.Module):
    def __init__(self, in_ch, block_sizes, resamples, norm_layer, conv_layer, dense, emb, number_of_classes, type,
                 sum_pool, dropout, arch='res', input_hw=None):
        super().__init__()
        blocks = []
        ch = in_ch
        self.arch = arch
        block = ResBlockDown if arch == 'res' else DCBlockDown
        for i, (bs, rs) in enumerate(zip(block_sizes, resamples)):
            bs = int(bs)
            blocks.append(block(ch, bs, rs, 'Discriminator.' + str(i), norm_layer, conv_layer, is_first=(i == 0)))
            ch = bs
        self.blocks = nn.ModuleList(blocks)
        self.sum_pool, self.type = sum_pool, type
        self.dropout = nn.Dropout(dropout) if dropout else None
        emb_dim = ch
        if arch == 'dcgan':
            h, w = (int(v) for v in input_hw)
            for rs in resamples:
                if rs == 'DOWN':
                    if h % 2 or w % 2:
                        raise ValueError(f"arch='dcgan': a DOWN block halves a {h} x {w} grid")
                    h, w = h // 2, w // 2
            if type == 'PROJECTIVE' and h * w != 1:
                raise ValueError(f"arch='dcgan' with type='PROJECTIVE' needs a 1 x 1 final grid (the embedding has block_sizes[-1] = {ch} "
                                 f"dimensions, the flattened features {h} x {w} x {ch}); no shipped recipe combines them")
            ch = h * w * ch
        self.out = dense(ch, 1)
        if type == 'AC_GAN':
            self.cls_out = nn.Linear(ch, number_of_classes)
            nn.init.xavier_uniform_(self.cls_out.weight); nn.init.zeros_(self.cls_out.bias)
        elif type == 'PROJECTIVE':
            self.emb = emb(number_of_classes, emb_dim)

    def forward(self, x, cls=None):
        from .spectral import prepare_spectral
        prepare_spectral(self)
        y = x
        for blk in self.blocks:
            y = blk(y, cls)
        if self.arch == 'dcgan':
            y = F.leaky_relu(y, LEAKY_SLOPE).flatten(1)
        else:
            y = F.relu(y)
            y = y.sum(dim=(1, 2)) if self.sum_pool else y.mean(dim=(1, 2))
        if self.dropout is not None:
            y = self.dropout(y)
        out = self.out(y)
        if self.type == 'AC_GAN':
            return out, self.cls_out(y)
        if self.type == 'PROJECTIVE':
            out = out + (self.emb(cls.reshape(-1).long()) * y).sum(dim=1, keepdim=True)
        return out


def make_discriminator(input_image_shape=(32, 32, 3), input_cls_shape=(1,), block_sizes=(128, 128, 128, 128),
                       resamples=('DOWN', 'DOWN', 'SAME', 'SAME'), number_of_classes=10,
                       type='AC_GAN', norm='n', after_norm='n', spectral=False,
                       fully_diff_spectral=False, spectral_iterations=1, conv_singular=True,
                       sum_pool=False, dropout=False, arch='res', filters_emb=10):
    assert arch in ('res', 'dcgan')
    assert type in [None, 'AC_GAN', 'PROJECTIVE']
    if spectral and conv_singular:
        import warnings
        warnings.warn("conv_singular=True is not built: spectral normalisation uses the reshaped-kernel singular value",
                      stacklevel=2)
    sn_kw = dict(spectral_iterations=spectral_iterations, fully_diff_spectral=fully_diff_spectral)
    conv_layer = partial(Conv2D, spectral=bool(spectral), conv_singular=conv_singular, **sn_kw)

    def dense(i, o):
        if spectral:
            from .spectral import SNLinear
            lin = SNLinear(i, o, **sn_kw)
            with torch.no_grad():
                nn.init.xavier_uniform_(lin.weight); nn.init.zeros_(lin.bias)
                lin._sn_init(**sn_kw)
            return lin
        lin = nn.Linear(i, o)
        nn.init.xavier_uniform_(lin.weight); nn.init.zeros_(lin.bias)
        return lin

    def emb(k, d):
        if spectral:
            from .spectral import SNEmbedding
            return SNEmbedding(k, d, **sn_kw)
        return nn.Embedding(k, d)

    norm_layer = create_norm(norm, after_norm, number_of_classes=number_of_classes, filters_emb=filters_emb)
    return Discriminator(int(input_image_shape[-1]), block_sizes, resamples, norm_layer, conv_layer, dense, emb,
                         number_of_classes, type, sum_pool, dropout, arch=arch, input_hw=input_image_shape[:2])
```

Baseline: 3719 images/sec.

## Fuse discriminator residual blocks into a single custom autograd function

Adds a critic-block autograd function that runs conv1, conv2 and the shortcut of non-first discriminator residual blocks together. The residual add goes into the conv2 epilogue. In backward, the relu mask, the avg-pool backward and the gradient sum are folded into one block-dx kernel, and bias column sums are computed inside the masked split kernel. The aim is to cut elementwise kernel launches and extra fp32 tensor passes per block, at the cost of much custom code and narrower applicability checks.

```diff
diff --git a/include/wc_hip.h b/include/wc_hip.h
--- a/include/wc_hip.h
+++ b/include/wc_hip.h
@@ -297,6 +297,13 @@
                   const float* bias, const void* zero_line, const wc_conv_geom* g, int relu, float* y,
                   void* ws, size_t ws_bytes, wc_stream_t stream);
 
+int wc_conv_res_supported(const wc_conv_geom* g);
+int wc_conv_res_f16x3(const void* xhi, const void* xlo, const float* xscale, const void* wimage, const float* wscale,
+                      const float* bias, const float* res, const void* zero_line, const wc_conv_geom* g, float* y,
+                      void* ws, size_t ws_bytes, wc_stream_t stream);
+int wc_conv_block_dx_f32(const float* dx1, const float* x, const float* other, int64_t N, int64_t H, int64_t W, int C, int down,
+                         float* out, wc_stream_t stream);
+
 size_t wc_conv_wrw_workspace_bytes(const wc_conv_geom* g);
 int wc_conv_wrw_f16x3(const void* xhi, const void* xlo, const float* xscale, const void* ghi, const void* glo,
                       const float* gscale, const void* zero_line, const wc_conv_geom* g, float* dw, int64_t stride_k,
@@ -393,9 +400,9 @@
 
 
 int wc_conv_split_masked_f32(const float* t, const float* a, int64_t n, float slope, void* hi, void* lo, float* scale, void* amax_scratch,
-                             wc_stream_t stream);
-int wc_conv_split_hist_masked_f32(const float* t, const float* a, int64_t n, float slope, void* hi, void* lo, float* scale, float* hist,
-                                  int bootstrap, wc_stream_t stream);
+                             float* colsum_partials , int C, wc_stream_t stream);
+int wc_conv_split_hist_masked_f32(const float* t, const float* a, int64_t n, float slope, void* hi, void* lo, float* scale,
+                                  float* colsum_partials , int C, float* hist, int bootstrap, wc_stream_t stream);
 
 int wc_gp_interp_f32(const float* real, const float* fake, const float* eps, int64_t N, int64_t L, float* x_hat, wc_stream_t stream);
 
diff --git a/wc_gan_amd/_lib.py b/wc_gan_amd/_lib.py
--- a/wc_gan_amd/_lib.py
+++ b/wc_gan_amd/_lib.py
@@ -186,8 +186,13 @@
     "wc_bwd_factor_renorm_f64": (c_int, [c_void_p, c_void_p, c_void_p, c_void_p, c_void_p, c_void_p, c_void_p, c_int, c_int, c_int64,
                                          c_double, c_int, c_int, c_void_p, c_void_p, c_void_p, c_void_p,
                                          c_void_p, c_size_t, c_void_p]),
-    "wc_conv_split_masked_f32": (c_int, [c_void_p, c_void_p, c_int64, c_float, c_void_p, c_void_p, c_void_p, c_void_p, c_void_p]),
-    "wc_conv_split_hist_masked_f32": (c_int, [c_void_p, c_void_p, c_int64, c_float, c_void_p, c_void_p, c_void_p, c_void_p, c_int, c_void_p]),
+    "wc_conv_split_masked_f32": (c_int, [c_void_p, c_void_p, c_int64, c_float, c_void_p, c_void_p, c_void_p, c_void_p, c_void_p, c_int, c_void_p]),
+    "wc_conv_split_hist_masked_f32": (c_int, [c_void_p, c_void_p, c_int64, c_float, c_void_p, c_void_p, c_void_p, c_void_p, c_int, c_void_p, c_int,
+                                              c_void_p]),
+    "wc_conv_res_supported": (c_int, [c_void_p]),
+    "wc_conv_res_f16x3": (c_int, [c_void_p, c_void_p, c_void_p, c_void_p, c_void_p, c_void_p, c_void_p, c_void_p, c_void_p,
+                                  c_void_p, c_void_p, c_size_t, c_void_p]),
+    "wc_conv_block_dx_f32": (c_int, [c_void_p, c_void_p, c_void_p, c_int64, c_int64, c_int64, c_int, c_int, c_void_p, c_void_p]),
     "wc_gp_interp_f32": (c_int, [c_void_p, c_void_p, c_void_p, c_int64, c_int64, c_void_p, c_void_p]),
     "wc_gp_rows_workspace_bytes": (c_size_t, [c_int64]),
     "wc_gp_rows_f32": (c_int, [c_void_p, c_int64, c_int64, c_double, c_double, c_void_p, c_void_p, c_void_p, c_void_p, c_size_t, c_void_p]),
diff --git a/wc_gan_amd/conv.py b/wc_gan_amd/conv.py
--- a/wc_gan_amd/conv.py
+++ b/wc_gan_amd/conv.py
@@ -88,7 +88,7 @@
 
 
 class _Plan:
-    __slots__ = ('ok', 'fwd', 'bwd', 'fwd_ws', 'bwd_ws', 'wrw_ws', 'fwd_ptr', 'bwd_ptr', 'pair')
+    __slots__ = ('ok', 'fwd', 'bwd', 'fwd_ws', 'bwd_ws', 'wrw_ws', 'fwd_ptr', 'bwd_ptr', 'pair', 'res')
 
     def __init__(self, kind, N, H, W, wshape):
         class _W:
@@ -102,6 +102,7 @@
         self.bwd_ws = lib.wc_conv_workspace_bytes(self.bwd_ptr) if self.ok else 0
         self.wrw_ws = lib.wc_conv_wrw_workspace_bytes(self.fwd_ptr) if self.ok else 0
         self.pair = self.ok and bool(lib.wc_conv_bwd_pair_supported(self.bwd_ptr, self.fwd_ptr))
+        self.res = self.ok and bool(lib.wc_conv_res_supported(self.fwd_ptr))
 
 
 _plans = {}
@@ -201,23 +202,38 @@
     return (hi, lo, scale, part) if colsum else (hi, lo, scale)
 
 
-def split_planes_masked(t, a, slope=0.0, site=None, role='t'):
+def split_planes_masked(t, a, slope=0.0, site=None, role='t', colsum=False):
     if not (t.is_contiguous() and a.is_contiguous() and t.shape == a.shape and t.dtype == a.dtype == torch.float32):
         raise ValueError("split_planes_masked: dense fp32 tensors of one shape")
     lib = _lib.load()
     both = torch.empty((2,) + tuple(t.shape), dtype=torch.float16, device=t.device)
     hi, lo = both[0], both[1]
     scale = torch.empty(1 + 512, dtype=torch.float32, device=t.device)
+    C = t.shape[-1]
+    part = torch.empty((512, C), dtype=torch.float32, device=t.device) if colsum else None
     h = _site_hist(site, role, t.device) if (SPLIT_HIST and site is not None) else None
     if h is not None:
-        _lib.check(lib.wc_conv_split_hist_masked_f32(_ptr(t), _ptr(a), t.numel(), float(slope), _ptr(hi), _ptr(lo), _ptr(scale), _ptr(h[0]),
+        _lib.check(lib.wc_conv_split_hist_masked_f32(_ptr(t), _ptr(a), t.numel(), float(slope), _ptr(hi), _ptr(lo), _ptr(scale),
+                                                     _ptr(part), C if colsum else 0, _ptr(h[0]),
                                                      (0 if h[1] else 1) | (0 if _guarded(role) else 2), _stream()),
                    "wc_conv_split_hist_masked_f32")
         h[1] = True
     else:
         _lib.check(lib.wc_conv_split_masked_f32(_ptr(t), _ptr(a), t.numel(), float(slope), _ptr(hi), _ptr(lo), _ptr(scale),
-                                                scale.data_ptr() + 4, _stream()), "wc_conv_split_masked_f32")
-    return hi, lo, scale
+                                                scale.data_ptr() + 4, _ptr(part), C if colsum else 0, _stream()), "wc_conv_split_masked_f32")
+    return (hi, lo, scale, part) if colsum else (hi, lo, scale)
+
+
+def block_input_gradient(dx1, x, other, down):
+    N, H, W, C = dx1.shape
+    want = (N, H // 2, W // 2, C) if down else (N, H, W, C)
+    if not (dx1.is_contiguous() and x.is_contiguous() and other.is_contiguous() and x.shape == dx1.shape and tuple(other.shape) == want
+            and dx1.dtype == x.dtype == other.dtype == torch.float32):
+        raise ValueError("block_input_gradient: dense fp32 NHWC tensors, `other` of dx1's shape (at half resolution when down)")
+    out = torch.empty_like(dx1)
+    _lib.check(_lib.load().wc_conv_block_dx_f32(_ptr(dx1), _ptr(x), _ptr(other), N, H, W, C, 1 if down else 0, _ptr(out), _stream()),
+               "wc_conv_block_dx_f32")
+    return out
 
 
 def leaky_backward_(dx, x, slope):
@@ -269,7 +285,7 @@
     return weight_image(w, geom, k_axis, n_axis)
 
 
-def run(planes, image, geom, bias=None, relu=False, nbytes=None):
+def run(planes, image, geom, bias=None, relu=False, nbytes=None, res=None):
     hi, lo, xs = planes
     img, ws = image
     lib = _lib.load()
@@ -277,6 +293,13 @@
     if nbytes is None:
         nbytes = lib.wc_conv_workspace_bytes(ctypes.addressof(geom))
     work = torch.empty(nbytes, dtype=torch.uint8, device=hi.device) if nbytes else None
+    if res is not None:
+        if relu or not (res.is_contiguous() and res.shape == y.shape and res.dtype == torch.float32 and res.device == y.device):
+            raise ValueError("run: the residual is a dense fp32 tensor of the output's shape (and there is no ReLU behind it)")
+        _lib.check(lib.wc_conv_res_f16x3(_ptr(hi), _ptr(lo), _ptr(xs), _ptr(img), _ptr(ws), _ptr(bias) if bias is not None else None,
+                                         _ptr(res), _ptr(_zero_line(hi.device)), ctypes.addressof(geom), _ptr(y),
+                                         _ptr(work), nbytes, _stream()), "wc_conv_res_f16x3")
+        return y
     _lib.check(lib.wc_conv_f16x3(_ptr(hi), _ptr(lo), _ptr(xs), _ptr(img), _ptr(ws), _ptr(bias) if bias is not None else None,
                                  _ptr(_zero_line(hi.device)), ctypes.addressof(geom), 1 if relu else 0, _ptr(y),
                                  _ptr(work), nbytes, _stream()), "wc_conv_f16x3")
@@ -359,7 +382,7 @@
 
 class _FastConv(torch.autograd.Function):
     @staticmethod
-    def forward(ctx, x, w, bias, kind, plan, relu_input=False, handed=None, site=None, leaky=None):
+    def forward(ctx, x, w, bias, kind, plan, relu_input=False, handed=None, site=None, leaky=None, residual=None):
         gf, kf, nf = plan.fwd
         planes = handed if handed is not None else split_planes(x, relu=relu_input, site=site, role='x', leaky=leaky)
         ctx.site, ctx.leaky = site, leaky
@@ -367,7 +390,12 @@
             img, ctx.bwd_image = weight_image_pair(w, plan.fwd, plan.bwd)
         else:
             img, ctx.bwd_image = weight_image(w, gf, kf, nf), None
-        y = run(planes, img, gf, bias, nbytes=plan.fwd_ws)
+        if residual is not None and plan.res and FUSED_RESIDUAL:
+            y = run(planes, img, gf, bias, nbytes=plan.fwd_ws, res=residual.contiguous())
+        else:
+            y = run(planes, img, gf, bias, nbytes=plan.fwd_ws)
+            if residual is not None:
+                y = y + residual
         ctx.save_for_backward(w, *planes, *((x,) if (relu_input or leaky is not None) else ()))
         ctx.kind, ctx.has_bias, ctx.plan, ctx.relu_input = kind, bias is not None, plan, relu_input
         return y
@@ -403,7 +431,8 @@
                 dw = weight_gradient((xh, xl, xs), g_planes, gf, w, kf, nf, nbytes=plan.wrw_ws)
         if want_db and not fused_db:
             db = gy.sum((0, 1, 2))
-        return dx, dw, db, None, None, None, None, None, None
+        need = ctx.needs_input_grad
+        return dx, dw, db, None, None, None, None, None, None, (gy if len(need) > 9 and need[9] else None)
 
 
 _ones = {}
@@ -607,7 +636,159 @@
     return bool(_lib.load().wc_conv_wrw_narrow_supported(N, H, W, w.shape[0], C, k))
 
 
-def fast_conv(x, w, bias=None, kind='same'):
+def fast_conv(x, w, bias=None, kind='same', residual=None):
     if not supported(x, w, kind):
         raise _lib.WcHipError(f"fast_conv: unsupported call {tuple(x.shape)} x {tuple(w.shape)} ({kind})")
-    return _FastConv.apply(x, w, bias, kind, _plan(kind, x, w))
+    if residual is None:
+        return _FastConv.apply(x, w, bias, kind, _plan(kind, x, w))
+    return _FastConv.apply(x, w, bias, kind, _plan(kind, x, w), False, None, None, None, residual)
+
+
+FUSED_BLOCK = True
+FUSED_MASKED_SPLIT = True
+FUSED_RESIDUAL = True
+FUSED_BLOCK_DX = True
+
+
+class _Shape:
+    def __init__(self, shape):
+        self.shape = tuple(shape)
+
+
+def critic_block_plans(xshape, w1shape, w2shape, wsshape, down):
+    if len(xshape) != 4 or len(w1shape) != 4 or len(w2shape) != 4:
+        return None
+    N, H, W, C = xshape
+    F1, F2 = w1shape[0], w2shape[0]
+    if tuple(w1shape[1:]) != (C, 3, 3) or tuple(w2shape[1:]) != (F1, 3, 3):
+        return None
+    if down and (H % 2 or W % 2):
+        return None
+    if wsshape is None:
+        if down or F2 != C:
+            return None
+    elif tuple(wsshape) != (F2, C, 1, 1):
+        return None
+    if not (_colsum_ok(F1) and _colsum_ok(F2)):
+        return None
+    out = (N, H // 2, W // 2) if down else (N, H, W)
+    p1 = _plan('same', _Shape(xshape), _Shape(w1shape))
+    p2 = _plan('down3' if down else 'same', _Shape((N, H, W, F1)), _Shape(w2shape))
+    ps = _plan('same', _Shape(out + (C,)), _Shape(wsshape)) if wsshape is not None else None
+    if not (p1 and p1.ok and p2 and p2.ok and (wsshape is None or (ps and ps.ok))):
+        return None
+    return p1, p2, ps
+
+
+def _images(w, plan, both):
+    if both:
+        return weight_image_pair(w, plan.fwd, plan.bwd)
+    gf, kf, nf = plan.fwd
+    return weight_image(w, gf, kf, nf), None
+
+
+def _layer_gradients(g_planes, fused_db, x_planes, w, plan, bwd_image, need_dx, need_dw):
+    cs = g_planes[3] if fused_db else None
+    if need_dx and need_dw and bwd_image is not None and plan.pair:
+        return backward_pair(g_planes, bwd_image, x_planes, plan, w, colsum=cs)
+    dx = dw = db = None
+    if need_dx:
+        gb, kb, nb = plan.bwd
+        image = bwd_image if bwd_image is not None else weight_image(w, gb, kb, nb)
+        dx = run(g_planes[:3], image, gb, nbytes=plan.bwd_ws)
+    if need_dw:
+        gf, kf, nf = plan.fwd
+        if fused_db:
+            dw, db = weight_gradient(x_planes, g_planes, gf, w, kf, nf, nbytes=plan.wrw_ws, colsum=cs)
+        else:
+            dw = weight_gradient(x_planes, g_planes, gf, w, kf, nf, nbytes=plan.wrw_ws)
+    return dx, dw, db
+
+
+def _pool2(x):
+    return F.avg_pool2d(x.permute(0, 3, 1, 2), 2).permute(0, 2, 3, 1).contiguous()
+
+
+class _CriticBlock(torch.autograd.Function):
+    @staticmethod
+    def forward(ctx, x, w1, b1, w2, b2, ws, bs, sites, plans, down):
+        conv1, conv2, shortcut = sites
+        p1, p2, ps = plans
+        need = ctx.needs_input_grad
+        need_h = need[0] or need[1] or need[2]
+        x_pl = split_planes(x, relu=True, site=conv1, role='x')
+        img1, bimg1 = _images(w1, p1, need[0])
+        h = run(x_pl, img1, p1.fwd[0], b1, nbytes=p1.fwd_ws)
+        h_pl = split_planes(h, relu=True, site=conv2, role='x')
+        img2, bimg2 = _images(w2, p2, need_h)
+        s, s_pl, bimgs = x, (), None
+        if ws is not None:
+            s_pl = split_planes(_pool2(x) if down else x, site=shortcut, role='x')
+            imgs, bimgs = _images(ws, ps, need[0])
+            s = run(s_pl, imgs, ps.fwd[0], bs, nbytes=ps.fwd_ws)
+        if p2.res and FUSED_RESIDUAL:
+            y = run(h_pl, img2, p2.fwd[0], b2, nbytes=p2.fwd_ws, res=s)
+        else:
+            y = run(h_pl, img2, p2.fwd[0], b2, nbytes=p2.fwd_ws) + s
+        ctx.save_for_backward(x, h, w1, w2, *x_pl, *h_pl, *s_pl, *((ws,) if ws is not None else ()))
+        ctx.sites, ctx.plans, ctx.down = sites, plans, down
+        ctx.images = (bimg1, bimg2, bimgs)
+        ctx.has_bias = (b1 is not None, b2 is not None, bs is not None)
+        ctx.mark_non_differentiable(h)
+        ctx.set_materialize_grads(False)
+        return y, h
+
+    @staticmethod
+    def backward(ctx, g, _gh):
+        saved = ctx.saved_tensors
+        x, h, w1, w2 = saved[:4]
+        x_pl, h_pl = saved[4:7], saved[7:10]
+        conv1, conv2, shortcut = ctx.sites
+        p1, p2, ps = ctx.plans
+        bimg1, bimg2, bimgs = ctx.images
+        need = ctx.needs_input_grad
+        need_h = need[0] or need[1] or need[2]
+        if g is None:
+            return (None,) * 10
+        g = g.contiguous()
+        dx = dw1 = db1 = dw2 = db2 = dws = dbs = dx1 = None
+
+        def bias_rides(has, need_b, need_w, C):
+            return has and need_b and need_w and _colsum_ok(C)
+
+        fused2 = bias_rides(ctx.has_bias[1], need[4], need[3], g.shape[-1])
+        g2 = split_planes(g, colsum=fused2, site=conv2, role='g')
+        dh, dw2, db2 = _layer_gradients(g2, fused2, h_pl, w2, p2, bimg2, need_h, need[3])
+        if ctx.has_bias[1] and need[4] and not fused2:
+            db2 = g.sum((0, 1, 2))
+        if need_h:
+            fused1 = bias_rides(ctx.has_bias[0], need[2], need[1], h.shape[-1])
+            if FUSED_MASKED_SPLIT:
+                g1 = split_planes_masked(dh, h, site=conv1, role='g', colsum=fused1)
+            else:
+                g1 = split_planes(torch.ops.aten.threshold_backward(dh, h, 0), colsum=fused1, site=conv1, role='g')
+            dx1, dw1, db1 = _layer_gradients(g1, fused1, x_pl, w1, p1, bimg1, need[0], need[1])
+            if ctx.has_bias[0] and need[2] and not fused1:
+                db1 = torch.ops.aten.threshold_backward(dh, h, 0).sum((0, 1, 2))
+        other = g
+        if ps is not None:
+            ws = saved[13]
+            fuseds = bias_rides(ctx.has_bias[2], need[6], need[5], g.shape[-1])
+            gs = split_planes(g, colsum=fuseds, site=shortcut, role='g')
+            other, dws, dbs = _layer_gradients(gs, fuseds, saved[10:13], ws, ps, bimgs, need[0], need[5])
+            if ctx.has_bias[2] and need[6] and not fuseds:
+                dbs = g.sum((0, 1, 2))
+        if need[0]:
+            if FUSED_BLOCK_DX:
+                dx = block_input_gradient(dx1, x, other, ctx.down)
+            else:
+                dx = torch.ops.aten.threshold_backward(dx1, x, 0)
+                if ctx.down:
+                    other = torch.ops.aten.avg_pool2d_backward(other.permute(0, 3, 1, 2), x.permute(0, 3, 1, 2), [2, 2], [2, 2], [0, 0],
+                                                               False, True, None).permute(0, 2, 3, 1)
+                dx = dx + other
+        return dx, dw1, db1, dw2, db2, dws, dbs, None, None, None
+
+
+def critic_block(x, w1, b1, w2, b2, ws, bs, sites, plans, down):
+    return _CriticBlock.apply(x, w1, b1, w2, b2, ws, bs, sites, plans, down)
diff --git a/wc_gan_amd/csrc/wc_conv.hip b/wc_gan_amd/csrc/wc_conv.hip
--- a/wc_gan_amd/csrc/wc_conv.hip
+++ b/wc_gan_amd/csrc/wc_conv.hip
@@ -216,7 +216,7 @@
 __device__ __forceinline__ void conv_ksplit_reduce_body(const float* __restrict__ partial, int ksplit, int64_t n4, int cout,
                                                         const float* __restrict__ xscale, const float* __restrict__ wscale,
                                                         const float* __restrict__ bias, int relu, float* __restrict__ y,
-                                                        const unsigned bid, const unsigned nblocks)
+                                                        const unsigned bid, const unsigned nblocks, const float* __restrict__ res = nullptr)
 {
     const float inv = 1.0f / (xscale[0] * wscale[0]);
     for (int64_t i = (int64_t)bid * 256 + threadIdx.x; i < n4; i += (int64_t)nblocks * 256) {
@@ -233,6 +233,11 @@
         v = v * inv;
         if (bias) v += *reinterpret_cast<const f32x4*>(bias + (4 * i) % cout);
         if (relu) { v[0] = fmaxf(v[0], 0.f); v[1] = fmaxf(v[1], 0.f); v[2] = fmaxf(v[2], 0.f); v[3] = fmaxf(v[3], 0.f); }
+        if (res) {
+            const f32x4 r = *reinterpret_cast<const f32x4*>(res + 4 * i);
+            #pragma unroll
+            for (int j = 0; j < 4; ++j) v[j] = __fadd_rn(v[j], r[j]);
+        }
         *reinterpret_cast<f32x4*>(y + 4 * i) = v;
     }
 }
@@ -242,6 +247,14 @@
                                                                  const float* __restrict__ bias, int relu, float* __restrict__ y)
 {
     conv_ksplit_reduce_body(partial, ksplit, n4, cout, xscale, wscale, bias, relu, y, blockIdx.x, gridDim.x);
+}
+
+__global__ __launch_bounds__(256) void conv_ksplit_reduce_res_kernel(const float* __restrict__ partial, int ksplit, int64_t n4, int cout,
+                                                                     const float* __restrict__ xscale, const float* __restrict__ wscale,
+                                                                     const float* __restrict__ bias, const float* __restrict__ res,
+                                                                     float* __restrict__ y)
+{
+    conv_ksplit_reduce_body(partial, ksplit, n4, cout, xscale, wscale, bias, 0, y, blockIdx.x, gridDim.x, res);
 }
 
 __device__ __forceinline__ f32x4 split_act(f32x4 v, int relu, float slope)
@@ -304,6 +317,35 @@
         #pragma unroll
         for (int j = 0; j < 4; ++j) g[j] = v[j] > 0.f ? g[j] : slope * g[j];
         *reinterpret_cast<f32x4*>(dx + 4 * i) = g;
+    }
+}
+
+template <bool DOWN>
+__global__ __launch_bounds__(256) void conv_block_dx_kernel(const float* __restrict__ dx1, const float* __restrict__ x,
+                                                            const float* __restrict__ other, int64_t n4, int c4, int W, int H,
+                                                            float* __restrict__ out)
+{
+    for (int64_t i = (int64_t)blockIdx.x * 256 + threadIdx.x; i < n4; i += (int64_t)gridDim.x * 256) {
+        const f32x4 d = *reinterpret_cast<const f32x4*>(dx1 + 4 * i);
+        const f32x4 a = *reinterpret_cast<const f32x4*>(x + 4 * i);
+        int64_t j = i;
+        if (DOWN) {
+            const int64_t pix = i / c4;
+            const int c = (int)(i - pix * c4);
+            const int64_t row = pix / W;
+            const int xx = (int)(pix - row * W);
+            const int64_t n = row / H;
+            const int yy = (int)(row - n * H);
+            j = ((n * (H >> 1) + (yy >> 1)) * (W >> 1) + (xx >> 1)) * c4 + c;
+        }
+        const f32x4 o = *reinterpret_cast<const f32x4*>(other + 4 * j);
+        f32x4 r;
+        #pragma unroll
+        for (int k = 0; k < 4; ++k) {
+            const float m = a[k] <= 0.f ? 0.f : d[k];
+            r[k] = __fadd_rn(m, DOWN ? __fadd_rn(0.f, __fmul_rn(0.25f, o[k])) : o[k]);
+        }
+        *reinterpret_cast<f32x4*>(out + 4 * i) = r;
     }
 }
 
@@ -1280,6 +1322,42 @@
         hipLaunchKernelGGL(conv_ksplit_reduce_kernel, dim3(grid_for(n4)), dim3(256), 0, st, (const float*)ws, a.ksplit, n4, g->Cout,
                            xscale, wscale, bias, relu, y);
     }
+    return (int)hipGetLastError();
+}
+
+int wc_conv_res_supported(const wc_conv_geom* g)
+{
+    return g && wc_conv_supported(g) && (g->Cout % 128) == 0 && conv_ksplit(g) > 1;
+}
+
+int wc_conv_res_f16x3(const void* xhi, const void* xlo, const float* xscale, const void* wimage, const float* wscale,
+                      const float* bias, const float* res, const void* zero_line, const wc_conv_geom* g, float* y,
+                      void* ws, size_t ws_bytes, wc_stream_t stream)
+{
+    hipStream_t st = (hipStream_t)stream;
+    if (!res) return WC_ERR_ARG;
+    ConvArgs a;
+    const int rc = conv_prepare(a, xhi, xlo, xscale, wimage, wscale, bias, zero_line, g, 0, y, ws, ws_bytes);
+    if (rc != WC_OK) return rc;
+    if (!wc_conv_res_supported(g)) return WC_ERR_SHAPE;
+    const hipError_t e = (g->Cout % 256) == 0 ? launch_conv<2, 4, true>(a, st) : launch_conv<2, 2, true>(a, st);
+    if (e != hipSuccess) return (int)e;
+    const int64_t n4 = (int64_t)g->N * g->Hout * g->Wout * g->Cout / 4;
+    hipLaunchKernelGGL(conv_ksplit_reduce_res_kernel, dim3(grid_for(n4)), dim3(256), 0, st, (const float*)ws, a.ksplit, n4, g->Cout,
+                       xscale, wscale, bias, res, y);
+    return (int)hipGetLastError();
+}
+
+int wc_conv_block_dx_f32(const float* dx1, const float* x, const float* other, int64_t N, int64_t H, int64_t W, int C, int down,
+                         float* out, wc_stream_t stream)
+{
+    if (!dx1 || !x || !other || !out) return WC_ERR_NULL;
+    if (N <= 0 || H <= 0 || W <= 0 || C <= 0 || (C & 3) || H > 0x7fffffff || W > 0x7fffffff) return WC_ERR_SHAPE;
+    if (down && ((H & 1) || (W & 1))) return WC_ERR_SHAPE;
+    const int64_t n4 = N * H * W * (C >> 2);
+    hipStream_t st = (hipStream_t)stream;
+    if (down) hipLaunchKernelGGL(conv_block_dx_kernel<true>, dim3(grid_for(n4)), dim3(256), 0, st, dx1, x, other, n4, C >> 2, (int)W, (int)H, out);
+    else      hipLaunchKernelGGL(conv_block_dx_kernel<false>, dim3(grid_for(n4)), dim3(256), 0, st, dx1, x, other, n4, C >> 2, (int)W, (int)H, out);
     return (int)hipGetLastError();
 }
 
diff --git a/wc_gan_amd/csrc/wc_gp.hip b/wc_gan_amd/csrc/wc_gp.hip
--- a/wc_gan_amd/csrc/wc_gp.hip
+++ b/wc_gan_amd/csrc/wc_gp.hip
@@ -47,16 +47,40 @@
     return m;
 }
 
+__device__ __forceinline__ f32x4 colsum_add(f32x4 cs, f32x4 v)
+{
+    #pragma unroll
+    for (int j = 0; j < 4; ++j) cs[j] = __fadd_rn(cs[j], v[j]);
+    return cs;
+}
+
+__device__ __forceinline__ void colsum_fold(f32x4* red4, float* __restrict__ colsum, int c4n)
+{
+    if (colsum && (int)threadIdx.x < c4n) {
+        f32x4 s = red4[threadIdx.x];
+        for (int p = threadIdx.x + c4n; p < 256; p += c4n) s += red4[p];
+        *reinterpret_cast<f32x4*>(colsum + (int64_t)blockIdx.x * 4 * c4n + 4 * threadIdx.x) = s;
+    }
+}
+
 __global__ __launch_bounds__(256) void gp_absmax_kernel(const float* __restrict__ t, const float* __restrict__ a, int64_t n4, float slope,
-                                                        float* __restrict__ partial)
+                                                        float* __restrict__ partial, float* __restrict__ colsum = nullptr, int c4n = 0)
 {
     __shared__ float red[4];
+    __shared__ f32x4 red4[256];
     float m = 0.f;
-    for (int64_t i = blockIdx.x * 256 + threadIdx.x; i < n4; i += (int64_t)gridDim.x * 256) m = absmax4(m, masked_load(t, a, i, slope));
+    f32x4 cs = {0.f, 0.f, 0.f, 0.f};
+    for (int64_t i = blockIdx.x * 256 + threadIdx.x; i < n4; i += (int64_t)gridDim.x * 256) {
+        const f32x4 v = masked_load(t, a, i, slope);
+        m = absmax4(m, v);
+        cs = colsum_add(cs, v);
+    }
     m = wave_max(m);
     if ((threadIdx.x & 63) == 0) red[threadIdx.x >> 6] = m;
+    if (colsum) red4[threadIdx.x] = cs;
     __syncthreads();
     if (threadIdx.x == 0) partial[blockIdx.x] = fmaxf(fmaxf(red[0], red[1]), fmaxf(red[2], red[3]));
+    colsum_fold(red4, colsum, c4n);
 }
 
 __global__ __launch_bounds__(256) void gp_split_kernel(const float* __restrict__ t, const float* __restrict__ a, int64_t n4, float slope,
@@ -93,9 +117,10 @@
 
 __global__ __launch_bounds__(256) void gp_split_hist_kernel(const float* __restrict__ t, const float* __restrict__ a, int64_t n4, float slope,
                                                             _Float16* __restrict__ hi, _Float16* __restrict__ lo, float* __restrict__ scale_out,
-                                                            float* __restrict__ hist)
+                                                            float* __restrict__ hist, float* __restrict__ colsum, int c4n)
 {
     __shared__ float red[4];
+    __shared__ f32x4 red4[256];
     float mx[2] = {0.f, 0.f};
     int tlo[2] = {0x7fffffff, 0x7fffffff}, thi[2] = {0, 0};
     #pragma unroll
@@ -123,18 +148,22 @@
     const float s = scale_for(assumed * kHistMargin);
     if (blockIdx.x == 0 && threadIdx.x == 0) { scale_out[0] = s; hist[2 * kHistArray + 2 + (1 - src)] = assumed; }
     float m = 0.f;
+    f32x4 cs = {0.f, 0.f, 0.f, 0.f};
     for (int64_t i = blockIdx.x * 256 + threadIdx.x; i < n4; i += (int64_t)gridDim.x * 256) {
         const f32x4 v = masked_load(t, a, i, slope);
+        cs = colsum_add(cs, v);
         m = absmax4(m, v);
         store_split(v, s, hi, lo, i);
     }
     m = wave_max(m);
     if ((threadIdx.x & 63) == 0) red[threadIdx.x >> 6] = m;
+    if (colsum) red4[threadIdx.x] = cs;
     __syncthreads();
     if (threadIdx.x == 0) {
         const f32x2h p = {fmaxf(fmaxf(red[0], red[1]), fmaxf(red[2], red[3])), __builtin_bit_cast(float, tag)};
         *reinterpret_cast<f32x2h*>(hist + (1 - src) * kHistArray + 2 * blockIdx.x) = p;
     }
+    colsum_fold(red4, colsum, c4n);
 }
 
 __global__ __launch_bounds__(256) void gp_split_redo_kernel(const float* __restrict__ t, const float* __restrict__ a, int64_t n4, float slope,
@@ -217,32 +246,42 @@
 
 extern "C" {
 
+static bool colsum_args_ok(const float* colsum_partials, int C, int64_t n)
+{
+    return !colsum_partials || (C > 0 && !(C & 3) && 256 % (C >> 2) == 0 && n % C == 0);
+}
+
 int wc_conv_split_masked_f32(const float* t, const float* a, int64_t n, float slope, void* hi, void* lo, float* scale, void* amax_scratch,
-                             wc_stream_t stream)
+                             float* colsum_partials, int C, wc_stream_t stream)
 {
     if (!t || !a || !hi || !lo || !scale || !amax_scratch || n <= 0 || (n & 3)) return WC_ERR_ARG;
     if (!(slope >= 0.f && slope <= 1.f)) return WC_ERR_ARG;
+    if (!colsum_args_ok(colsum_partials, C, n)) return WC_ERR_SHAPE;
     hipStream_t st = (hipStream_t)stream;
-    hipLaunchKernelGGL(gp_absmax_kernel, dim3(kAmaxBlocks), dim3(256), 0, st, t, a, n / 4, slope, (float*)amax_scratch);
+    hipLaunchKernelGGL(gp_absmax_kernel, dim3(kAmaxBlocks), dim3(256), 0, st, t, a, n / 4, slope, (float*)amax_scratch,
+                       colsum_partials, colsum_partials ? C >> 2 : 0);
     hipLaunchKernelGGL(gp_split_kernel, dim3(grid_for(n / 4)), dim3(256), 0, st, t, a, n / 4, slope, (const float*)amax_scratch,
                        (_Float16*)hi, (_Float16*)lo, scale);
     return (int)hipGetLastError();
 }
 
-int wc_conv_split_hist_masked_f32(const float* t, const float* a, int64_t n, float slope, void* hi, void* lo, float* scale, float* hist,
-                                  int bootstrap, wc_stream_t stream)
+int wc_conv_split_hist_masked_f32(const float* t, const float* a, int64_t n, float slope, void* hi, void* lo, float* scale,
+                                  float* colsum_partials, int C, float* hist, int bootstrap, wc_stream_t stream)
 {
     if (!t || !a || !hi || !lo || !scale || !hist || n <= 0 || (n & 3)) return WC_ERR_ARG;
     if (!(slope >= 0.f && slope <= 1.f)) return WC_ERR_ARG;
+    if (!colsum_args_ok(colsum_partials, C, n)) return WC_ERR_SHAPE;
     hipStream_t st = (hipStream_t)stream;
+    const int c4n = colsum_partials ? C >> 2 : 0;
     if (bootstrap & 1) {
-        hipLaunchKernelGGL(gp_absmax_kernel, dim3(kAmaxBlocks), dim3(256), 0, st, t, a, n / 4, slope, hist);
+        hipLaunchKernelGGL(gp_absmax_kernel, dim3(kAmaxBlocks), dim3(256), 0, st, t, a, n / 4, slope, hist, colsum_partials, c4n);
         hipLaunchKernelGGL(gp_split_kernel, dim3(grid_for(n / 4)), dim3(256), 0, st, t, a, n / 4, slope, (const float*)hist, (_Float16*)hi,
                            (_Float16*)lo, scale);
         hipLaunchKernelGGL(gp_hist_seed_kernel, dim3(1), dim3(kAmaxBlocks), 0, st, hist);
         return (int)hipGetLastError();
     }
-    hipLaunchKernelGGL(gp_split_hist_kernel, dim3(kAmaxBlocks), dim3(256), 0, st, t, a, n / 4, slope, (_Float16*)hi, (_Float16*)lo, scale, hist);
+    hipLaunchKernelGGL(gp_split_hist_kernel, dim3(kAmaxBlocks), dim3(256), 0, st, t, a, n / 4, slope, (_Float16*)hi, (_Float16*)lo, scale, hist,
+                       colsum_partials, c4n);
     if (!(bootstrap & 2)) {
         const unsigned g2 = grid_for(n / 4) < 64 ? grid_for(n / 4) : 64u;
         hipLaunchKernelGGL(gp_split_redo_kernel, dim3(g2), dim3(256), 0, st, t, a, n / 4, slope, (_Float16*)hi, (_Float16*)lo, scale, hist);
diff --git a/wc_gan_amd/discriminator.py b/wc_gan_amd/discriminator.py
--- a/wc_gan_amd/discriminator.py
+++ b/wc_gan_amd/discriminator.py
@@ -26,7 +26,36 @@
         if self.has_shortcut:
             self.shortcut = conv_layer(in_ch, nfilters, (1, 1), name=name + '.shortcut')
 
+    def _fusable(self):
+        from . import conv as fc, generator as _g
+        if self.is_first or not (fc.FUSED_BLOCK and _g.FAST_CONV):
+            return False
+        if not all(isinstance(bn, _g._UnfusedStack) and bn.norm_layer is None and len(bn.branches) == 0 for bn in (self.bn1, self.bn2)):
+            return False
+        convs = [self.conv1, self.conv2] + ([self.shortcut] if self.has_shortcut else [])
+        return all(isinstance(c, Conv2D) and c.kind == 'same' and c.conv.weight.dtype == torch.float32 for c in convs)
+
+    def _fused_plans(self, x):
+        from . import conv as fc, generator as _g
+        if not self._fusable():
+            return None
+        if not (torch.is_tensor(x) and x.is_cuda and x.dtype == torch.float32 and x.dim() == 4 and x.is_contiguous()
+                and getattr(x, '_wc_planes', None) is None and _g.split_of(x) is None):
+            return None
+        return fc.critic_block_plans(tuple(x.shape), tuple(self.conv1.conv.weight.shape), tuple(self.conv2.conv.weight.shape),
+                                     tuple(self.shortcut.conv.weight.shape) if self.has_shortcut else None, self.resample == 'DOWN')
+
     def forward(self, x, cls):
+        plans = self._fused_plans(x)
+        if plans is not None:
+            from . import conv as fc
+            w1, w2 = self.conv1._weight(), self.conv2._weight()
+            ws = self.shortcut._weight() if self.has_shortcut else None
+            x = self.bn1(x, cls)
+            y, h = fc.critic_block(x, w1, self.conv1.conv.bias, w2, self.conv2.conv.bias, ws, self.shortcut.conv.bias if self.has_shortcut else None,
+                                   (self.conv1, self.conv2, self.shortcut if self.has_shortcut else None), plans, self.resample == 'DOWN')
+            self.bn2(h, cls)
+            return y
         h = self.conv1(x) if self.is_first else self.conv1.forward_relu(self.bn1(x, cls))
         h = self.bn2(h, cls)
         s = x
```

Measured after the change: 3804 images/sec (median of 6 runs). 1.02x the previous value.
